# someone-in-somewhere/multimodal_rag

Measured on AMD Instinct MI355X. Metric: chunks embedded/sec + queries/sec top_k=5 over 1M×768 at 1/2/4/8 GPUs, higher is better.
Workload: dtype f16

## Files before the change

include/mmrag.h:

```cpp
#ifndef MMRAG_H
#define MMRAG_H

#include <stddef.h>
#include <stdint.h>

#ifdef __cplusplus
extern "C" {
#endif

#define MMRAG_OK 0
#define MMRAG_EINVAL 1
#define MMRAG_EWORKSPACE 2
#define MMRAG_EHIP 3
#define MMRAG_EUNSUPPORTED 4

#define MMRAG_F32 0
#define MMRAG_F16 1
#define MMRAG_BF16 2
#define MMRAG_F8E4M3 3

#define MMRAG_MAX_K 20

int mmrag_abi_version(void);
const char *mmrag_last_error(void);

int64_t mmrag_padded_dim(int d, int dtype);

size_t mmrag_cosine_topk_workspace_bytes(int B, int64_t n, int k);

int mmrag_cosine_topk(const void *q, const void *corpus, int B, int64_t n, int d, int64_t ld,
                      int dtype, int k, int64_t row_offset, const uint32_t *alive_bits,
                      float *out_scores, int64_t *out_rows, void *workspace,
                      size_t workspace_bytes, void *stream);

int mmrag_cosine_topk_lists(const void *q, const void *corpus, int B, int64_t n, int d, int64_t ld,
                            int dtype, int k, const uint32_t *alive_bits, void *workspace,
                            size_t workspace_bytes, void *stream);
int mmrag_cosine_topk_select(int B, int64_t n, int k, int64_t row_offset, const void *workspace,
                             float *out_scores, int64_t *out_rows, void *stream);

#define MMRAG_MAX_K_DEEP 4096
size_t mmrag_cosine_topk_deep_workspace_bytes(int B, int64_t n, int k);
int mmrag_cosine_topk_deep(const void *q, const void *corpus, int B, int64_t n, int d, int64_t ld,
                           int dtype, int k, int64_t row_offset, const uint32_t *alive_bits,
                           float *out_scores, int64_t *out_rows, void *workspace,
                           size_t workspace_bytes, void *stream);

#define MMRAG_MAX_RESCORE_CANDIDATES 4096
int mmrag_rescore_topk(const void *q, const void *plane, int64_t ld, int dtype, int d, const int64_t *cand_rows,
                       int B, int C, int k, float *out_scores, int64_t *out_rows, void *stream);

int mmrag_merge_topk(const float *scores, const int64_t *rows, int G, int B, int k_in, int k,
                     float *out_scores, int64_t *out_rows, void *stream);
int mmrag_merge_topk_host(const float *scores, const int64_t *rows, int G, int B, int k_in,
                          int k, float *out_scores, int64_t *out_rows);
int mmrag_merge_topk_host_packed(const void *blocks, int G, int B, int k_in, int k,
                                 float *out_scores, int64_t *out_rows);

int mmrag_append_rows(void *corpus, int64_t capacity, int64_t ld, int dtype, int64_t n_used,
                      const float *new_rows, int64_t m, int d, void *stream);

int mmrag_gather_rows(void *dst, const void *src, int64_t ld, int dtype,
                      const int64_t *keep_rows, int64_t m, void *stream);

int mmrag_fetch_rows_f32(const void *corpus, int64_t ld, int dtype, const int64_t *rows,
                         int64_t m, int d, float *out, void *stream);

int mmrag_copy_to_host_async(void *dst_host, const void *src_dev, size_t bytes, void *stream);


#define MMRAG_ACT_NONE 0
#define MMRAG_ACT_GELU 1
#define MMRAG_ACT_QUICK_GELU 2

#define MMRAG_ARCH_BERT 0
#define MMRAG_ARCH_PRELN 1

#define MMRAG_POOL_MEAN 0
#define MMRAG_POOL_FIRST 1
#define MMRAG_POOL_SELECT 2

typedef struct mmrag_encoder_desc {
    int32_t arch;
    int32_t n_layers, hidden, n_heads, intermediate, vocab, max_pos;
    int32_t pool, act, causal, normalize;
    int32_t out_dim;
    float ln_eps;
    int32_t image, patch;
} mmrag_encoder_desc;

size_t mmrag_encoder_workspace_bytes(const mmrag_encoder_desc *desc, int64_t T, int B);
int mmrag_encoder_forward(const mmrag_encoder_desc *desc, const void *const *w, const int32_t *ids,
                          const int32_t *pos_ids, const int32_t *cu_seqlens, const int32_t *sel,
                          int64_t T, int B, int max_len, float *out, void *workspace,
                          size_t workspace_bytes, void *stream);

size_t mmrag_encoder_f32_workspace_bytes(const mmrag_encoder_desc *desc, int64_t T, int B);
int mmrag_encoder_forward_f32(const mmrag_encoder_desc *desc, const void *const *w, const int32_t *ids,
                              const int32_t *pos_ids, const int32_t *cu_seqlens, const int32_t *sel, int64_t T, int B,
                              int max_len, float *out, void *workspace, size_t workspace_bytes, void *stream);
int mmrag_linear_f32(const float *x, int64_t M, int K, const float *wt, int N, const float *bias, int act,
                     const float *resid, float *out, void *stream);

size_t mmrag_cross_encoder_workspace_bytes(const mmrag_encoder_desc *desc, int64_t T, int B);
int mmrag_cross_encoder_forward(const mmrag_encoder_desc *desc, const void *const *w, int n_labels, const int32_t *ids,
                                const int32_t *type_ids, const int32_t *pos_ids, const int32_t *cu_seqlens, int64_t T,
                                int B, int max_len, float *out_logits, void *workspace, size_t workspace_bytes,
                                void *stream);
size_t mmrag_cross_encoder_f32_workspace_bytes(const mmrag_encoder_desc *desc, int64_t T, int B);
int mmrag_cross_encoder_forward_f32(const mmrag_encoder_desc *desc, const void *const *w, int n_labels,
                                    const int32_t *ids, const int32_t *type_ids, const int32_t *pos_ids,
                                    const int32_t *cu_seqlens, int64_t T, int B, int max_len, float *out_logits,
                                    void *workspace, size_t workspace_bytes, void *stream);

#define MMRAG_MAX_READER_TOKENS 512
#define MMRAG_MAX_ANSWER_TOKENS 64
#define MMRAG_MAX_READER_SPANS 8
int mmrag_span_select(const void *hidden, int ld, int hidden_dim, const float *qa_w, const float *qa_b,
                      const int32_t *cu_seqlens, const int32_t *ctx_start, const int32_t *ctx_len, int64_t T, int B,
                      int max_answer_tokens, int n_best, int32_t *out_span, float *out_score, float *out_null,
                      float *out_lse, float *out_logits, void *stream);
size_t mmrag_reader_workspace_bytes(const mmrag_encoder_desc *desc, int64_t T, int B);
int mmrag_reader_forward(const mmrag_encoder_desc *desc, const void *const *w, const int32_t *ids,
                         const int32_t *type_ids, const int32_t *pos_ids, const int32_t *cu_seqlens,
                         const int32_t *ctx_start, const int32_t *ctx_len, int64_t T, int B, int max_len,
                         int max_answer_tokens, int n_best, int32_t *out_span, float *out_score, float *out_null,
                         float *out_lse, float *out_logits, void *workspace, size_t workspace_bytes, void *stream);

#define MMRAG_PIXELS_F16_CHW 0
#define MMRAG_PIXELS_U8_HWC 1
int mmrag_vit_forward(const mmrag_encoder_desc *desc, const void *const *w, const void *pixels, int pixel_kind,
                      const int32_t *cu_seqlens, int B, float *out, void *workspace, size_t workspace_bytes,
                      void *stream);

void *mmrag_wordpiece_create(const uint32_t *cps, const int64_t *offsets, int n_tokens, int lower);
void mmrag_wordpiece_destroy(void *tokenizer);
int mmrag_wordpiece_encode_batch(const void *tokenizer, const uint32_t *cps, const int64_t *offsets, int n,
                                 int max_length, int32_t *ids, int32_t *lens, int n_threads);

int mmrag_wordpiece_encode_pairs(const void *tokenizer, const uint32_t *cps_a, const int64_t *offsets_a,
                                 const uint32_t *cps_b, const int64_t *offsets_b, int n, int max_length, int32_t *ids,
                                 int32_t *type_ids, int32_t *lens, int n_threads);

#define MMRAG_LEX_DOCUMENTS 0
#define MMRAG_LEX_QUERIES 1
void *mmrag_lexicon_create(void);
void mmrag_lexicon_destroy(void *lexicon);
int64_t mmrag_lexicon_size(const void *lexicon);
int mmrag_lexicon_analyze_batch(void *lexicon, const uint32_t *cps, const int64_t *offsets, int n, int mode,
                                int64_t *out_offsets, int32_t *term_ids, int32_t *tfs, int32_t *dl, int64_t capacity,
                                int n_threads);

int mmrag_lexical_df_update(const int64_t *fwd_off, const int32_t *fwd_term, const int64_t *rows, int64_t row0,
                            int64_t n_rows, int sign, int32_t *df, void *stream);
size_t mmrag_lexical_csr_build_workspace_bytes(int64_t n, int n_terms);
int mmrag_lexical_csr_build(const int64_t *fwd_off, const int32_t *fwd_term, const int32_t *fwd_tf, int64_t n,
                            int64_t n_postings, int n_terms, int64_t *term_off, int32_t *post_row, int32_t *post_tf,
                            void *workspace, size_t workspace_bytes, void *stream);
size_t mmrag_bm25_topk_workspace_bytes(int B, int64_t n, int k);
int mmrag_bm25_topk(const int64_t *term_off, const int32_t *post_row, const int32_t *post_tf, const int32_t *dl,
                    const int32_t *df, int n_terms, int64_t n, const int32_t *q_off, const int32_t *q_terms, int B,
                    int64_t n_live, int64_t sum_dl, float k1, float b, int k, const uint32_t *alive_bits,
                    float *out_scores, int64_t *out_rows, void *workspace, size_t workspace_bytes, void *stream);
int mmrag_rows_dot(const void *q, const void *corpus, int64_t ld, int dtype, int d, const int32_t *qi,
                   const int64_t *rows, int64_t m, float *out, void *stream);

#define MMRAG_MAX_MMR_CANDIDATES 1024
size_t mmrag_mmr_select_workspace_bytes(int B, int C, int d, int dtype);
int mmrag_mmr_select(const void *corpus, int64_t ld, int dtype, int d, const float *cand_scores,
                     const int64_t *cand_rows, int B, int C, int k, float lambda, float *out_scores, int64_t *out_rows,
                     int32_t *out_pos, float *out_mmr, void *workspace, size_t workspace_bytes, void *stream);

#define MMRAG_MAX_GROUP_CANDIDATES 4096
#define MMRAG_MAX_GROUPS 256
#define MMRAG_MAX_GROUP_SIZE 16
int mmrag_group_select(const float *scores, const int64_t *rows, int B, int C, const int32_t *group_of_row,
                       int64_t n_rows, int n_groups, int group_size, float *out_scores, int64_t *out_rows,
                       int32_t *out_pos, int32_t *out_group, int32_t *out_info, void *stream);

#define MMRAG_MAX_FUSE_LISTS 16
#define MMRAG_MAX_FUSE_CANDIDATES 256
#define MMRAG_MAX_FUSE_RESULTS 4096
#define MMRAG_FUSE_RRF 0
#define MMRAG_FUSE_MAX 1
int mmrag_fuse_select(const float *scores, const int64_t *rows, int L, int C, const int32_t *list_off, int G,
                      const float *weights, int method, int rrf_k, int n, float *out_fused, int64_t *out_rows,
                      float *out_best, int32_t *out_best_list, int32_t *out_count, int32_t *out_info, void *stream);

#define MMRAG_MAX_JOIN_PAIRS (1 << 26)
int mmrag_sim_join(const void *rows, int64_t n, int64_t ld, int dtype, int d, const uint32_t *alive, float threshold,
                   int64_t *out_pairs, float *out_scores, int64_t capacity, unsigned long long *count, void *stream);

#define MMRAG_MAX_CLUSTERS 4096
int mmrag_kmeans_assign(const void *rows, int64_t n, int64_t ld, int dtype, int d, const void *centroids, int k,
                        const uint32_t *alive, int32_t *out_assign, float *out_score, void *stream);
int mmrag_cluster_sums(const void *rows, int64_t ld, int dtype, int d, const int32_t *order, const int64_t *seg_off,
                       int k, float *out_sums, void *stream);

#define MMRAG_MAX_SCOPE_GROUPS 64
size_t mmrag_scoped_topk_workspace_bytes(int B, int64_t n, int k, int n_groups);
int mmrag_scoped_topk(const void *q, const void *rows, int B, int64_t n, int d, int64_t ld, int dtype, int k,
                      int64_t row_offset, const uint32_t *alive_bits, const int32_t *group_of_row, int n_groups,
                      const int32_t *scope_of_query, int S, const int32_t *scope_off, const int32_t *scope_groups,
                      int64_t max_candidates, float *out_scores, int64_t *out_rows, void *workspace,
                      size_t workspace_bytes, void *stream);

size_t mmrag_boosted_topk_workspace_bytes(int B, int64_t n, int k);
int mmrag_boosted_topk(const void *q, const void *rows, int B, int64_t n, int d, int64_t ld, int dtype, int k,
                       int64_t row_offset, const uint32_t *alive_bits, const float *prior, const float *weight,
                       float *out_scores, int64_t *out_rows, float *out_boost, void *workspace, size_t workspace_bytes,
                       void *stream);

#define MMRAG_MAX_RECOMMEND_EXAMPLES 16
size_t mmrag_recommend_topk_workspace_bytes(int R, int64_t n, int k);
int mmrag_recommend_topk(const void *examples, const int8_t *sign, const float *neg_weight, const void *rows, int R,
                         int64_t n, int d, int64_t ld, int dtype, int k, int64_t row_offset, const uint32_t *alive_bits,
                         float *out_scores, int64_t *out_rows, float *out_pos, float *out_neg, int32_t *out_pos_arg,
                         int32_t *out_neg_arg, void *workspace, size_t workspace_bytes, void *stream);

#define MMRAG_MAX_RELATED_ROWS 8192
#define MMRAG_MAX_RELATED_SETS 64
size_t mmrag_related_groups_workspace_bytes(int M, int S, int64_t n, int n_groups, int k);
int mmrag_related_groups(const void *set_rows, int M, const int32_t *set_off, int S, const void *rows, int64_t n, int d,
                         int64_t ld, int dtype, const uint32_t *alive_bits, const int32_t *group_of_row, int n_groups,
                         const int32_t *exclude_group, float threshold, int k, float *out_similarity, int32_t *out_group,
                         int32_t *out_covered, float *out_best, int64_t *out_best_row, void *workspace,
                         size_t workspace_bytes, void *stream);

#define MMRAG_MAX_FILTER_OPS 32
#define MMRAG_MAX_FILTER_SET 64
#define MMRAG_MAX_FILTER_COLUMNS 16
#define MMRAG_FILTER_NUMBER 0
#define MMRAG_FILTER_STRING 1
enum {
    MMRAG_FILTER_TRUE = 0, MMRAG_FILTER_FALSE, MMRAG_FILTER_AND, MMRAG_FILTER_OR, MMRAG_FILTER_EQ, MMRAG_FILTER_NE,
    MMRAG_FILTER_GT, MMRAG_FILTER_GE, MMRAG_FILTER_LT, MMRAG_FILTER_LE, MMRAG_FILTER_IN, MMRAG_FILTER_NIN
};
typedef struct {
    int32_t code, column, set_off, set_len;
    double value;
} mmrag_filter_op;
int64_t mmrag_filter_words(int64_t n);
int mmrag_filter_eval(const mmrag_filter_op *ops, int n_ops, const int32_t *prog_off, int F, const double *set_values,
                      int n_set, const void *const *columns, const int32_t *kinds, int n_columns, int64_t n,
                      const uint32_t *alive_bits, uint32_t *out_bits, void *stream);
size_t mmrag_filtered_topk_workspace_bytes(int B, int64_t n, int k);
int mmrag_filtered_topk(const void *q, const void *rows, int B, int64_t n, int d, int64_t ld, int dtype, int k,
                        int64_t row_offset, const int32_t *filter_of_query, int F, const uint32_t *vis_bits,
                        float *out_scores, int64_t *out_rows, void *workspace, size_t workspace_bytes, void *stream);

#define MMRAG_MAX_FACET_COLUMNS 4
size_t mmrag_range_scan_workspace_bytes(int B, int64_t n, int limit, int facet_slots);
int mmrag_range_scan(const void *q, const void *rows, int B, int64_t n, int d, int64_t ld, int dtype,
                     const float *threshold, int limit, int64_t row_offset, const int32_t *filter_of_query, int F,
                     const uint32_t *vis_bits, const int32_t *const *facet_cols, const int32_t *facet_sizes, int n_facets,
                     uint32_t *out_count, uint32_t *out_facets, float *out_scores, int64_t *out_rows, void *workspace,
                     size_t workspace_bytes, void *stream);

#define MMRAG_MAX_LATE_QUERY_TOKENS 128
#define MMRAG_MAX_LATE_DOC_TOKENS 512
size_t mmrag_encoder_tokens_workspace_bytes(const mmrag_encoder_desc *desc, int64_t T, int B, int out_dim);
int mmrag_encoder_forward_tokens(const mmrag_encoder_desc *desc, const void *const *w, const int32_t *ids,
                                 const int32_t *pos_ids, const int32_t *cu_seqlens, int64_t T, int B, int max_len,
                                 const void *proj, int out_dim, void *out_tokens, void *workspace,
                                 size_t workspace_bytes, void *stream);
int mmrag_maxsim_scores(const void *q_tok, int64_t q_rows, int64_t q_ld, const void *d_tok, int64_t d_rows,
                        int64_t d_ld, int dim, const int32_t *q_start, const int32_t *q_len, int n_q,
                        const int32_t *d_start, const int32_t *d_len, int n_d, const int32_t *pair_q,
                        const int32_t *pair_d, int P, float *out_sum, float *out_best_sim, int32_t *out_best_idx,
                        void *stream);

#define MMRAG_MAX_LATE_QUESTIONS 4096
size_t mmrag_maxsim_topk_workspace_bytes(int Q, int64_t n_items, int k);
int mmrag_maxsim_topk(const void *q_tok, int64_t q_rows, int64_t q_ld, const int32_t *q_start, const int32_t *q_len,
                      int Q, const void *tok, int64_t T, int64_t ld, const int32_t *item_off, int64_t n_items,
                      const uint32_t *alive_bits, int dim, int k, float *out_scores, int64_t *out_items,
                      void *workspace, size_t workspace_bytes, void *stream);

int mmrag_f8_encode_rows(const void *src, int src_dtype, int64_t m, int d, int64_t src_ld, void *dst, int64_t dst_ld,
                         void *stream);
int mmrag_maxsim_scores_f8(const void *q_codes, int64_t q_rows, int64_t q_ld, const void *d_codes, int64_t d_rows,
                           int64_t d_ld, int dim, const int32_t *q_start, const int32_t *q_len, int n_q,
                           const int32_t *d_start, const int32_t *d_len, int n_d, const int32_t *pair_q,
                           const int32_t *pair_d, int P, float *out_sum, float *out_best_sim, int32_t *out_best_idx,
                           void *stream);
size_t mmrag_maxsim_topk_f8_workspace_bytes(int Q, int64_t n_items, int k);
int mmrag_maxsim_topk_f8(const void *q_codes, int64_t q_rows, int64_t q_ld, const int32_t *q_start,
                         const int32_t *q_len, int Q, const void *codes, int64_t T, int64_t ld,
                         const int32_t *item_off, int64_t n_items, const uint32_t *alive_bits, int dim, int k,
                         float *out_scores, int64_t *out_items, void *workspace, size_t workspace_bytes, void *stream);

#define MMRAG_LATE_WINDOW_TOKENS 16
#define MMRAG_MAX_LATE_WINDOWS 32
int mmrag_maxsim_windows(const void *q_tok, int64_t q_rows, int64_t q_ld, const void *d_tok, int64_t d_rows,
                         int64_t d_ld, int dim, const int32_t *q_start, const int32_t *q_len, int n_q,
                         const int32_t *d_start, const int32_t *d_len, int n_d, const int32_t *pair_q,
                         const int32_t *pair_d, int P, int window_blocks, float *out_sum, float *out_win,
                         int32_t *out_best, void *stream);
int mmrag_maxsim_windows_f8(const void *q_codes, int64_t q_rows, int64_t q_ld, const void *d_codes, int64_t d_rows,
                            int64_t d_ld, int dim, const int32_t *q_start, const int32_t *q_len, int n_q,
                            const int32_t *d_start, const int32_t *d_len, int n_d, const int32_t *pair_q,
                            const int32_t *pair_d, int P, int window_blocks, float *out_sum, float *out_win,
                            int32_t *out_best, void *stream);

void *mmrag_clip_bpe_create(const uint32_t *vocab_cps, const int64_t *vocab_offsets, const int32_t *vocab_ids,
                            int n_vocab, const uint32_t *merge_cps, const int64_t *merge_offsets, int n_merges);
void mmrag_clip_bpe_destroy(void *tokenizer);
int mmrag_clip_bpe_encode_batch(const void *tokenizer, const uint32_t *cps, const int64_t *offsets, int n,
                                int max_length, int32_t *ids, int32_t *lens, int n_threads);

int mmrag_resample_ksize(int in_size, int out_size);
int mmrag_resample_coeffs(int in_size, int out_size, int first, int count, int32_t *bounds, int32_t *taps);
int mmrag_resize_crop_u8(const uint8_t *src, int H, int W, int64_t src_row_bytes, const int32_t *bx,
                         const int32_t *kx, int ksx, const int32_t *by, const int32_t *ky, int ksy, int out_h,
                         int out_w, int y_lo, int y_hi, uint8_t *tmp, uint8_t *dst, void *stream);

#define MMRAG_MAX_SPARSE_CHUNK_TOKENS 512
#define MMRAG_MAX_SPARSE_CHUNKS 65536
#define MMRAG_MAX_SPARSE_VOCAB 65536
#define MMRAG_MAX_SPARSE_TERMS 256
#define MMRAG_MAX_SPARSE_QUERY_TERMS 64
size_t mmrag_sparse_expand_forward_workspace_bytes(const mmrag_encoder_desc *desc, int64_t T, int B);
int mmrag_sparse_expand_forward(const mmrag_encoder_desc *desc, const void *const *w, const int32_t *ids,
                                const int32_t *pos_ids, const int32_t *cu_seqlens, int64_t T, int B, int max_len,
                                const void *head_w, const float *head_b, const float *head_ln_g,
                                const float *head_ln_b, void *out_tokens, void *workspace, size_t workspace_bytes,
                                void *stream);
size_t mmrag_sparse_pool_workspace_bytes(int64_t T, int n_chunks, int V);
int mmrag_sparse_pool(const void *tok, int64_t T, int64_t tok_ld, const int32_t *cu, int n_chunks, const void *E, int V,
                      int64_t e_ld, int dim, float *pooled, void *workspace, size_t workspace_bytes, void *stream);
int mmrag_sparse_select(const float *pooled, const float *bias, const uint32_t *skip_bits, int n_chunks, int V,
                        float scale, int m, int32_t *out_cnt, int32_t *out_terms, int32_t *out_imp, void *stream);
size_t mmrag_impact_topk_workspace_bytes(int B, int64_t n, int k);
int mmrag_impact_topk(const int64_t *term_off, const int32_t *post_row, const int32_t *post_imp, int n_terms, int64_t n,
                      const int32_t *q_off, const int32_t *q_terms, const int32_t *q_imp, int B, int k,
                      const uint32_t *alive_bits, float *out_scores, int64_t *out_rows, void *workspace,
                      size_t workspace_bytes, void *stream);

#define MMRAG_MAX_SUMMARY_SENTENCES 128
#define MMRAG_MAX_SUMMARY_ITERATIONS 64
int mmrag_summary_select(const void *rows, int64_t ld, int dtype, int d, int64_t n_rows, const int32_t *unit_start,
                         const int32_t *unit_len, int n_units, const int32_t *cost, const int32_t *budget,
                         const void *bias_rows, int64_t n_bias, const int32_t *unit_bias, float edge_threshold,
                         float alpha, int iterations, float lambda, int k, int32_t *out_pos, float *out_val,
                         float *out_rel, int32_t *out_used, void *stream);

int mmrag_device_info(int *n_cus, int *max_clock_mhz, int64_t *hbm_bytes);
int mmrag_bench_stream_copy(void *dst, const void *src, int64_t bytes, void *stream);
int mmrag_bench_stream_read(const void *src, int64_t bytes, float *out, void *stream);
int mmrag_bench_stream_write(void *dst, int64_t bytes, void *stream);
int mmrag_bench_mfma_f16(const void *seed, float *out, int iters, int64_t *flops, void *stream);
int mmrag_bench_mfma_f16_16x16x32(const void *seed, float *out, int iters, int64_t *flops, void *stream);

int mmrag_linear_f16(const void *x, int64_t M, int K, const void *wt, int N, const float *bias, int act,
                     const void *resid, void *out, void *stream);
int mmrag_layernorm_f16(const void *x, void *out, const float *gamma, const float *beta, int64_t T, int H,
                        float eps, void *stream);
int mmrag_embed_ln_f16(const int32_t *ids, const int32_t *pos_ids, const void *tok, const void *pos,
                       const void *type0, const float *gamma, const float *beta, void *out, int64_t T,
                       int H, int vocab, int max_pos, float eps, void *stream);
int mmrag_attention_f16(const void *qkv, const int32_t *cu_seqlens, void *ctx, int B, int max_len, int H,
                        int n_heads, int causal, void *stream);
int mmrag_pool_normalize_f16(const void *x, const int32_t *cu_seqlens, const int32_t *sel, float *out,
                             int B, int H, int pool, int normalize, void *stream);

#ifdef __cplusplus
}
#endif
#endif
```

multimodal_rag_amd/_native.py:

```python
from __future__ import annotations

import ctypes
import os
import threading
from ctypes import c_char_p, c_float, c_int, c_int32, c_int64, c_size_t, c_void_p
from typing import Optional, Tuple

import numpy as np
import torch

_PKG = os.path.dirname(os.path.abspath(__file__))
LIB_PATH = os.path.join(_PKG, "lib", "libmmrag.so")

F32, F16, BF16, F8E4M3 = 0, 1, 2, 3
MAX_K = 20
MAX_K_DEEP = 4096
MAX_MMR_CANDIDATES = 1024
MAX_RESCORE_CANDIDATES = 4096
MAX_GROUP_CANDIDATES, MAX_GROUPS, MAX_GROUP_SIZE = 4096, 256, 16
MAX_FUSE_LISTS, MAX_FUSE_CANDIDATES, MAX_FUSE_RESULTS = 16, 256, 4096
FUSE_METHODS = {"rrf": 0, "max": 1}
MAX_JOIN_PAIRS = 1 << 26
MAX_CLUSTERS = 4096
MAX_SCOPE_GROUPS = 64
MAX_FILTER_OPS, MAX_FILTER_SET, MAX_FILTER_COLUMNS = 32, 64, 16
MAX_FACET_COLUMNS = 4
MAX_RELATED_ROWS, MAX_RELATED_SETS = 8192, 64
MAX_RECOMMEND_EXAMPLES = 16
MAX_LATE_QUERY_TOKENS, MAX_LATE_DOC_TOKENS = 128, 512
MAX_LATE_PAIRS = 65535
MAX_LATE_QUESTIONS = 4096
LATE_WINDOW_TOKENS, MAX_LATE_WINDOWS = 16, 32
MAX_SUMMARY_SENTENCES, MAX_SUMMARY_ITERATIONS = 128, 64
MAX_READER_TOKENS, MAX_ANSWER_TOKENS, MAX_READER_SPANS = 512, 64, 8
_DT2TORCH = {F32: torch.float32, F16: torch.float16, BF16: torch.bfloat16, F8E4M3: torch.float8_e4m3fn}
_TORCH2DT = {v: k for k, v in _DT2TORCH.items()}

_lib = None
_lock = threading.Lock()


class MMRagNativeError(RuntimeError):
    pass


def _declare(lib):
    lib.mmrag_abi_version.restype = c_int
    lib.mmrag_last_error.restype = c_char_p
    lib.mmrag_padded_dim.restype = c_int64
    lib.mmrag_padded_dim.argtypes = [c_int, c_int]
    lib.mmrag_cosine_topk_workspace_bytes.restype = c_size_t
    lib.mmrag_cosine_topk_workspace_bytes.argtypes = [c_int, c_int64, c_int]
    lib.mmrag_cosine_topk.restype = c_int
    lib.mmrag_cosine_topk.argtypes = [c_void_p, c_void_p, c_int, c_int64, c_int, c_int64, c_int, c_int,
                                      c_int64, c_void_p, c_void_p, c_void_p, c_void_p, c_size_t, c_void_p]
    lib.mmrag_cosine_topk_lists.restype = c_int
    lib.mmrag_cosine_topk_lists.argtypes = [c_void_p, c_void_p, c_int, c_int64, c_int, c_int64, c_int, c_int,
                                            c_void_p, c_void_p, c_size_t, c_void_p]
    lib.mmrag_internal_search_uses_qs.restype = c_int
    lib.mmrag_internal_search_uses_qs.argtypes = [c_int, c_int64, c_int64, c_int, c_int]
    lib.mmrag_internal_cosine_topk_lists_ex.restype = c_int
    lib.mmrag_internal_cosine_topk_lists_ex.argtypes = [c_void_p, c_void_p, c_int, c_int64, c_int, c_int64, c_int,
                                                        c_int, c_void_p, c_void_p, c_size_t, c_void_p, ctypes.c_uint]
    lib.mmrag_cosine_topk_select.restype = c_int
    lib.mmrag_cosine_topk_select.argtypes = [c_int, c_int64, c_int, c_int64, c_void_p, c_void_p, c_void_p, c_void_p]
    lib.mmrag_cosine_topk_deep_workspace_bytes.restype = c_size_t
    lib.mmrag_cosine_topk_deep_workspace_bytes.argtypes = [c_int, c_int64, c_int]
    lib.mmrag_cosine_topk_deep.restype = c_int
    lib.mmrag_cosine_topk_deep.argtypes = lib.mmrag_cosine_topk.argtypes
    lib.mmrag_internal_cosine_topk_deep_ex.restype = c_int
    lib.mmrag_internal_cosine_topk_deep_ex.argtypes = lib.mmrag_cosine_topk.argtypes + [ctypes.c_uint, c_int64]
    lib.mmrag_rescore_topk.restype = c_int
    lib.mmrag_rescore_topk.argtypes = [c_void_p, c_void_p, c_int64, c_int, c_int, c_void_p, c_int, c_int, c_int,
                                       c_void_p, c_void_p, c_void_p]
    lib.mmrag_merge_topk.restype = c_int
    lib.mmrag_merge_topk.argtypes = [c_void_p, c_void_p, c_int, c_int, c_int, c_int, c_void_p, c_void_p, c_void_p]
    lib.mmrag_merge_topk_host.restype = c_int
    lib.mmrag_merge_topk_host.argtypes = [c_void_p, c_void_p, c_int, c_int, c_int, c_int, c_void_p, c_void_p]
    lib.mmrag_merge_topk_host_packed.restype = c_int
    lib.mmrag_merge_topk_host_packed.argtypes = [c_void_p, c_int, c_int, c_int, c_int, c_void_p, c_void_p]
    lib.mmrag_append_rows.restype = c_int
    lib.mmrag_append_rows.argtypes = [c_void_p, c_int64, c_int64, c_int, c_int64, c_void_p, c_int64, c_int, c_void_p]
    lib.mmrag_gather_rows.restype = c_int
    lib.mmrag_gather_rows.argtypes = [c_void_p, c_void_p, c_int64, c_int, c_void_p, c_int64, c_void_p]
    lib.mmrag_fetch_rows_f32.restype = c_int
    lib.mmrag_fetch_rows_f32.argtypes = [c_void_p, c_int64, c_int, c_void_p, c_int64, c_int, c_void_p, c_void_p]
    lib.mmrag_device_info.restype = c_int
    lib.mmrag_device_info.argtypes = [ctypes.POINTER(c_int), ctypes.POINTER(c_int), ctypes.POINTER(c_int64)]
    lib.mmrag_bench_stream_copy.restype = c_int
    lib.mmrag_bench_stream_copy.argtypes = [c_void_p, c_void_p, c_int64, c_void_p]
    lib.mmrag_bench_mfma_f16.restype = c_int
    lib.mmrag_bench_mfma_f16.argtypes = [c_void_p, c_void_p, c_int, ctypes.POINTER(c_int64), c_void_p]
    lib.mmrag_bench_mfma_f16_16x16x32.restype = c_int
    lib.mmrag_bench_mfma_f16_16x16x32.argtypes = [c_void_p, c_void_p, c_int, ctypes.POINTER(c_int64), c_void_p]
    lib.mmrag_bench_stream_read.restype = c_int
    lib.mmrag_bench_stream_read.argtypes = [c_void_p, c_int64, c_void_p, c_void_p]
    lib.mmrag_bench_stream_write.restype = c_int
    lib.mmrag_bench_stream_write.argtypes = [c_void_p, c_int64, c_void_p]
    lib.mmrag_copy_to_host_async.restype = c_int
    lib.mmrag_copy_to_host_async.argtypes = [c_void_p, c_void_p, c_size_t, c_void_p]
    lib.mmrag_encoder_workspace_bytes.restype = c_size_t
    lib.mmrag_encoder_workspace_bytes.argtypes = [c_void_p, c_int64, c_int]
    lib.mmrag_encoder_forward.restype = c_int
    lib.mmrag_encoder_forward.argtypes = [c_void_p, c_void_p, c_void_p, c_void_p, c_void_p, c_void_p, c_int64, c_int,
                                          c_int, c_void_p, c_void_p, c_size_t, c_void_p]
    lib.mmrag_encoder_f32_workspace_bytes.restype = c_size_t
    lib.mmrag_encoder_f32_workspace_bytes.argtypes = [c_void_p, c_int64, c_int]
    lib.mmrag_encoder_forward_f32.restype = c_int
    lib.mmrag_encoder_forward_f32.argtypes = lib.mmrag_encoder_forward.argtypes
    lib.mmrag_linear_f32.restype = c_int
    lib.mmrag_linear_f32.argtypes = [c_void_p, c_int64, c_int, c_void_p, c_int, c_void_p, c_int, c_void_p, c_void_p, c_void_p]
    lib.mmrag_vit_forward.restype = c_int
    lib.mmrag_vit_forward.argtypes = [c_void_p, c_void_p, c_void_p, c_int, c_void_p, c_int, c_void_p, c_void_p, c_size_t,
                                      c_void_p]
    lib.mmrag_wordpiece_create.restype = c_void_p
    lib.mmrag_wordpiece_create.argtypes = [c_void_p, c_void_p, c_int, c_int]
    lib.mmrag_wordpiece_destroy.restype = None
    lib.mmrag_wordpiece_destroy.argtypes = [c_void_p]
    lib.mmrag_wordpiece_encode_batch.restype = c_int
    lib.mmrag_wordpiece_encode_batch.argtypes = [c_void_p, c_void_p, c_void_p, c_int, c_int, c_void_p, c_void_p, c_int]
    lib.mmrag_clip_bpe_create.restype = c_void_p
    lib.mmrag_clip_bpe_create.argtypes = [c_void_p, c_void_p, c_void_p, c_int, c_void_p, c_void_p, c_int]
    lib.mmrag_clip_bpe_destroy.restype = None
    lib.mmrag_clip_bpe_destroy.argtypes = [c_void_p]
    lib.mmrag_clip_bpe_encode_batch.restype = c_int
    lib.mmrag_clip_bpe_encode_batch.argtypes = [c_void_p, c_void_p, c_void_p, c_int, c_int, c_void_p, c_void_p, c_int]
    lib.mmrag_resample_ksize.restype = c_int
    lib.mmrag_resample_ksize.argtypes = [c_int, c_int]
    lib.mmrag_resample_coeffs.restype = c_int
    lib.mmrag_resample_coeffs.argtypes = [c_int, c_int, c_int, c_int, c_void_p, c_void_p]
    lib.mmrag_resize_crop_u8.restype = c_int
    lib.mmrag_resize_crop_u8.argtypes = [c_void_p, c_int, c_int, c_int64, c_void_p, c_void_p, c_int, c_void_p, c_void_p,
                                         c_int, c_int, c_int, c_int, c_int, c_void_p, c_void_p, c_void_p]
    lib.mmrag_linear_f16.restype = c_int
    lib.mmrag_linear_f16.argtypes = [c_void_p, c_int64, c_int, c_void_p, c_int, c_void_p, c_int, c_void_p, c_void_p,
                                     c_void_p]
    lib.mmrag_layernorm_f16.restype = c_int
    lib.mmrag_layernorm_f16.argtypes = [c_void_p, c_void_p, c_void_p, c_void_p, c_int64, c_int, c_float, c_void_p]
    lib.mmrag_embed_ln_f16.restype = c_int
    lib.mmrag_embed_ln_f16.argtypes = [c_void_p, c_void_p, c_void_p, c_void_p, c_void_p, c_void_p, c_void_p, c_void_p,
                                       c_int64, c_int, c_int, c_int, c_float, c_void_p]
    lib.mmrag_attention_f16.restype = c_int
    lib.mmrag_attention_f16.argtypes = [c_void_p, c_void_p, c_void_p, c_int, c_int, c_int, c_int, c_int, c_void_p]
    lib.mmrag_pool_normalize_f16.restype = c_int
    lib.mmrag_pool_normalize_f16.argtypes = [c_void_p, c_void_p, c_void_p, c_void_p, c_int, c_int, c_int, c_int,
                                             c_void_p]
    lib.mmrag_internal_linear_f16_norms.restype = c_int
    lib.mmrag_internal_linear_f16_norms.argtypes = [c_void_p, c_int64, c_int, c_void_p, c_int, c_void_p, c_int, c_void_p,
                                                    c_void_p, c_void_p, c_void_p, c_float, c_void_p, c_void_p, c_void_p,
                                                    c_void_p, c_void_p]
    lib.mmrag_internal_attention_f32.restype = c_int
    lib.mmrag_internal_attention_f32.argtypes = [c_void_p, c_void_p, c_void_p, c_int, c_int, c_int, c_int, c_void_p]
    lib.mmrag_internal_layernorm_f32.restype = c_int
    lib.mmrag_internal_layernorm_f32.argtypes = [c_void_p, c_void_p, c_void_p, c_void_p, c_int64, c_int, c_float, c_void_p]
    lib.mmrag_internal_pool_norm_f32.restype = c_int
    lib.mmrag_internal_pool_norm_f32.argtypes = [c_void_p, c_void_p, c_void_p, c_void_p, c_int, c_int, c_int, c_int,
                                                 c_void_p]
    lib.mmrag_internal_patchify.restype = c_int
    lib.mmrag_internal_patchify.argtypes = [c_void_p, c_int, c_void_p, c_int, c_int, c_int, c_void_p]
    lib.mmrag_internal_vit_assemble_ln.restype = c_int
    lib.mmrag_internal_vit_assemble_ln.argtypes = [c_void_p] * 6 + [c_int, c_int, c_int, c_float, c_void_p]
    lib.mmrag_internal_normalize_rows.restype = c_int
    lib.mmrag_internal_normalize_rows.argtypes = [c_void_p, c_void_p, c_int, c_int, c_void_p]
    lib.mmrag_internal_pool_f16.restype = c_int
    lib.mmrag_internal_pool_f16.argtypes = [c_void_p, c_void_p, c_void_p, c_void_p, c_int, c_int, c_int, c_void_p]
    lib.mmrag_cross_encoder_workspace_bytes.restype = c_size_t
    lib.mmrag_cross_encoder_workspace_bytes.argtypes = [c_void_p, c_int64, c_int]
    lib.mmrag_cross_encoder_f32_workspace_bytes.restype = c_size_t
    lib.mmrag_cross_encoder_f32_workspace_bytes.argtypes = [c_void_p, c_int64, c_int]
    lib.mmrag_cross_encoder_forward.restype = c_int
    lib.mmrag_cross_encoder_forward.argtypes = [c_void_p, c_void_p, c_int, c_void_p, c_void_p, c_void_p, c_void_p,
                                                c_int64, c_int, c_int, c_void_p, c_void_p, c_size_t, c_void_p]
    lib.mmrag_cross_encoder_forward_f32.restype = c_int
    lib.mmrag_cross_encoder_forward_f32.argtypes = lib.mmrag_cross_encoder_forward.argtypes
    lib.mmrag_span_select.restype = c_int
    lib.mmrag_span_select.argtypes = [c_void_p, c_int, c_int, c_void_p, c_void_p, c_void_p, c_void_p, c_void_p, c_int64,
                                      c_int, c_int, c_int, c_void_p, c_void_p, c_void_p, c_void_p, c_void_p, c_void_p]
    lib.mmrag_reader_workspace_bytes.restype = c_size_t
    lib.mmrag_reader_workspace_bytes.argtypes = [c_void_p, c_int64, c_int]
    lib.mmrag_reader_forward.restype = c_int
    lib.mmrag_reader_forward.argtypes = [c_void_p] * 8 + [c_int64, c_int, c_int, c_int, c_int] + [c_void_p] * 6 + \
        [c_size_t, c_void_p]
    lib.mmrag_wordpiece_encode_pairs.restype = c_int
    lib.mmrag_wordpiece_encode_pairs.argtypes = [c_void_p, c_void_p, c_void_p, c_void_p, c_void_p, c_int, c_int, c_void_p,
                                                 c_void_p, c_void_p, c_int]
    lib.mmrag_internal_embed_types_ln_f16.restype = c_int
    lib.mmrag_internal_embed_types_ln_f16.argtypes = [c_void_p] * 9 + [c_int64, c_int, c_int, c_int, c_int, c_float,
                                                                       c_void_p]
    lib.mmrag_internal_embed_types_ln_f32.restype = c_int
    lib.mmrag_internal_embed_types_ln_f32.argtypes = lib.mmrag_internal_embed_types_ln_f16.argtypes
    lib.mmrag_internal_cls_head_f32.restype = c_int
    lib.mmrag_internal_cls_head_f32.argtypes = [c_void_p] * 6 + [c_int, c_int, c_int, c_void_p, c_size_t, c_void_p]
    lib.mmrag_internal_cls_head_workspace_bytes.restype = c_size_t
    lib.mmrag_internal_cls_head_workspace_bytes.argtypes = [c_int, c_int, c_int]
    lib.mmrag_mmr_select_workspace_bytes.restype = c_size_t
    lib.mmrag_mmr_select_workspace_bytes.argtypes = [c_int, c_int, c_int, c_int]
    lib.mmrag_mmr_select.restype = c_int
    lib.mmrag_mmr_select.argtypes = [c_void_p, c_int64, c_int, c_int, c_void_p, c_void_p, c_int, c_int, c_int, c_float,
                                     c_void_p, c_void_p, c_void_p, c_void_p, c_void_p, c_size_t, c_void_p]
    lib.mmrag_internal_mmr_select_ex.restype = c_int
    lib.mmrag_internal_mmr_select_ex.argtypes = lib.mmrag_mmr_select.argtypes + [ctypes.c_uint]
    lib.mmrag_group_select.restype = c_int
    lib.mmrag_group_select.argtypes = [c_void_p, c_void_p, c_int, c_int, c_void_p, c_int64, c_int, c_int, c_void_p,
                                       c_void_p, c_void_p, c_void_p, c_void_p, c_void_p]
    lib.mmrag_fuse_select.restype = c_int
    lib.mmrag_fuse_select.argtypes = [c_void_p, c_void_p, c_int, c_int, c_void_p, c_int, c_void_p, c_int, c_int, c_int,
                                      c_void_p, c_void_p, c_void_p, c_void_p, c_void_p, c_void_p, c_void_p]
    lib.mmrag_sim_join.restype = c_int
    lib.mmrag_sim_join.argtypes = [c_void_p, c_int64, c_int64, c_int, c_int, c_void_p, c_float, c_void_p, c_void_p,
                                   c_int64, c_void_p, c_void_p]
    for name in ("mmrag_internal_join_tile", "mmrag_internal_join_slot_tile"):
        getattr(lib, name).restype = c_int
        getattr(lib, name).argtypes = [c_int64, c_int64, ctypes.POINTER(c_int64), ctypes.POINTER(c_int64)]
    lib.mmrag_kmeans_assign.restype = c_int
    lib.mmrag_kmeans_assign.argtypes = [c_void_p, c_int64, c_int64, c_int, c_int, c_void_p, c_int, c_void_p, c_void_p,
                                        c_void_p, c_void_p]
    lib.mmrag_cluster_sums.restype = c_int
    lib.mmrag_cluster_sums.argtypes = [c_void_p, c_int64, c_int, c_int, c_void_p, c_void_p, c_int, c_void_p, c_void_p]
    lib.mmrag_scoped_topk_workspace_bytes.restype = c_size_t
    lib.mmrag_scoped_topk_workspace_bytes.argtypes = [c_int, c_int64, c_int, c_int]
    lib.mmrag_scoped_topk.restype = c_int
    lib.mmrag_scoped_topk.argtypes = [c_void_p, c_void_p, c_int, c_int64, c_int, c_int64, c_int, c_int, c_int64,
                                      c_void_p, c_void_p, c_int, c_void_p, c_int, c_void_p, c_void_p, c_int64,
                                      c_void_p, c_void_p, c_void_p, c_size_t, c_void_p]
    lib.mmrag_internal_scoped_topk_ex.restype = c_int
    lib.mmrag_internal_scoped_topk_ex.argtypes = lib.mmrag_scoped_topk.argtypes + [c_int64]
    lib.mmrag_filter_words.restype = c_int64
    lib.mmrag_filter_words.argtypes = [c_int64]
    lib.mmrag_filter_eval.restype = c_int
    lib.mmrag_filter_eval.argtypes = [c_void_p, c_int, c_void_p, c_int, c_void_p, c_int, c_void_p, c_void_p, c_int,
                                      c_int64, c_void_p, c_void_p, c_void_p]
    lib.mmrag_filtered_topk_workspace_bytes.restype = c_size_t
    lib.mmrag_filtered_topk_workspace_bytes.argtypes = [c_int, c_int64, c_int]
    lib.mmrag_filtered_topk.restype = c_int
    lib.mmrag_filtered_topk.argtypes = [c_void_p, c_void_p, c_int, c_int64, c_int, c_int64, c_int, c_int, c_int64,
                                        c_void_p, c_int, c_void_p, c_void_p, c_void_p, c_void_p, c_size_t, c_void_p]
    lib.mmrag_internal_filtered_topk_ex.restype = c_int
    lib.mmrag_internal_filtered_topk_ex.argtypes = lib.mmrag_filtered_topk.argtypes + [c_int64, ctypes.c_uint, c_void_p]
    lib.mmrag_range_scan_workspace_bytes.restype = c_size_t
    lib.mmrag_range_scan_workspace_bytes.argtypes = [c_int, c_int64, c_int, c_int]
    lib.mmrag_range_scan.restype = c_int
    lib.mmrag_range_scan.argtypes = [c_void_p, c_void_p, c_int, c_int64, c_int, c_int64, c_int, c_void_p, c_int, c_int64,
                                     c_void_p, c_int, c_void_p, c_void_p, c_void_p, c_int, c_void_p, c_void_p, c_void_p,
                                     c_void_p, c_void_p, c_size_t, c_void_p]
    lib.mmrag_internal_range_scan_ex.restype = c_int
    lib.mmrag_internal_range_scan_ex.argtypes = lib.mmrag_range_scan.argtypes + [c_int64, ctypes.c_uint]
    lib.mmrag_related_groups_workspace_bytes.restype = c_size_t
    lib.mmrag_related_groups_workspace_bytes.argtypes = [c_int, c_int, c_int64, c_int, c_int]
    lib.mmrag_related_groups.restype = c_int
    lib.mmrag_related_groups.argtypes = [c_void_p, c_int, c_void_p, c_int, c_void_p, c_int64, c_int, c_int64, c_int,
                                         c_void_p, c_void_p, c_int, c_void_p, c_float, c_int, c_void_p, c_void_p,
                                         c_void_p, c_void_p, c_void_p, c_void_p, c_size_t, c_void_p]
    lib.mmrag_internal_related_groups_ex.restype = c_int
    lib.mmrag_internal_related_groups_ex.argtypes = lib.mmrag_related_groups.argtypes + [c_int64]
    lib.mmrag_internal_candidate_capacity.restype = c_int64
    lib.mmrag_internal_candidate_capacity.argtypes = [c_int]
    lib.mmrag_internal_bound_plan.restype = c_int
    lib.mmrag_internal_bound_plan.argtypes = [c_int64, c_int, c_int64, ctypes.c_uint, c_void_p, c_void_p]
    lib.mmrag_boosted_topk_workspace_bytes.restype = c_size_t
    lib.mmrag_boosted_topk_workspace_bytes.argtypes = [c_int, c_int64, c_int]
    lib.mmrag_boosted_topk.restype = c_int
    lib.mmrag_boosted_topk.argtypes = [c_void_p, c_void_p, c_int, c_int64, c_int, c_int64, c_int, c_int, c_int64,
                                       c_void_p, c_void_p, c_void_p, c_void_p, c_void_p, c_void_p, c_void_p, c_size_t,
                                       c_void_p]
    lib.mmrag_internal_boosted_topk_ex.restype = c_int
    lib.mmrag_internal_boosted_topk_ex.argtypes = lib.mmrag_boosted_topk.argtypes + [c_int64, ctypes.c_uint]
    lib.mmrag_recommend_topk_workspace_bytes.restype = c_size_t
    lib.mmrag_recommend_topk_workspace_bytes.argtypes = [c_int, c_int64, c_int]
    lib.mmrag_recommend_topk.restype = c_int
    lib.mmrag_recommend_topk.argtypes = [c_void_p, c_void_p, c_void_p, c_void_p, c_int, c_int64, c_int, c_int64, c_int,
                                         c_int, c_int64, c_void_p, c_void_p, c_void_p, c_void_p, c_void_p, c_void_p,
                                         c_void_p, c_void_p, c_size_t, c_void_p]
    lib.mmrag_internal_recommend_topk_ex.restype = c_int
    lib.mmrag_internal_recommend_topk_ex.argtypes = lib.mmrag_recommend_topk.argtypes + [c_int64, ctypes.c_uint]
    lib.mmrag_encoder_tokens_workspace_bytes.restype = c_size_t
    lib.mmrag_encoder_tokens_workspace_bytes.argtypes = [c_void_p, c_int64, c_int, c_int]
    lib.mmrag_encoder_forward_tokens.restype = c_int
    lib.mmrag_encoder_forward_tokens.argtypes = [c_void_p, c_void_p, c_void_p, c_void_p, c_void_p, c_int64, c_int, c_int,
                                                 c_void_p, c_int, c_void_p, c_void_p, c_size_t, c_void_p]
    lib.mmrag_maxsim_scores.restype = c_int
    lib.mmrag_maxsim_scores.argtypes = [c_void_p, c_int64, c_int64, c_void_p, c_int64, c_int64, c_int, c_void_p, c_void_p,
                                        c_int, c_void_p, c_void_p, c_int, c_void_p, c_void_p, c_int, c_void_p, c_void_p,
                                        c_void_p, c_void_p]
    lib.mmrag_maxsim_topk_workspace_bytes.restype = c_size_t
    lib.mmrag_maxsim_topk_workspace_bytes.argtypes = [c_int, c_int64, c_int]
    lib.mmrag_maxsim_topk.restype = c_int
    lib.mmrag_maxsim_topk.argtypes = [c_void_p, c_int64, c_int64, c_void_p, c_void_p, c_int, c_void_p, c_int64, c_int64,
                                      c_void_p, c_int64, c_void_p, c_int, c_int, c_void_p, c_void_p, c_void_p, c_size_t,
                                      c_void_p]
    lib.mmrag_internal_maxsim_topk_ex.restype = c_int
    lib.mmrag_internal_maxsim_topk_ex.argtypes = lib.mmrag_maxsim_topk.argtypes + [c_int, c_int64, ctypes.c_uint, c_int]
    lib.mmrag_internal_maxsim_topk_workspace_bytes_ex.restype = c_size_t
    lib.mmrag_internal_maxsim_topk_workspace_bytes_ex.argtypes = [c_int, c_int64, c_int, c_int, c_int]
    lib.mmrag_f8_encode_rows.restype = c_int
    lib.mmrag_f8_encode_rows.argtypes = [c_void_p, c_int, c_int64, c_int, c_int64, c_void_p, c_int64, c_void_p]
    lib.mmrag_maxsim_scores_f8.restype = c_int
    lib.mmrag_maxsim_scores_f8.argtypes = lib.mmrag_maxsim_scores.argtypes
    lib.mmrag_maxsim_topk_f8_workspace_bytes.restype = c_size_t
    lib.mmrag_maxsim_topk_f8_workspace_bytes.argtypes = [c_int, c_int64, c_int]
    lib.mmrag_maxsim_topk_f8.restype = c_int
    lib.mmrag_maxsim_topk_f8.argtypes = lib.mmrag_maxsim_topk.argtypes
    lib.mmrag_internal_maxsim_topk_f8_ex.restype = c_int
    lib.mmrag_internal_maxsim_topk_f8_ex.argtypes = lib.mmrag_internal_maxsim_topk_ex.argtypes
    lib.mmrag_internal_maxsim_topk_f8_workspace_bytes_ex.restype = c_size_t
    lib.mmrag_internal_maxsim_topk_f8_workspace_bytes_ex.argtypes = [c_int, c_int64, c_int, c_int, c_int]
    lib.mmrag_maxsim_windows.restype = c_int
    lib.mmrag_maxsim_windows.argtypes = lib.mmrag_maxsim_scores.argtypes[:16] + [c_int, c_void_p, c_void_p, c_void_p,
                                                                                 c_void_p]
    lib.mmrag_maxsim_windows_f8.restype = c_int
    lib.mmrag_maxsim_windows_f8.argtypes = lib.mmrag_maxsim_windows.argtypes
    lib.mmrag_sparse_expand_forward_workspace_bytes.restype = c_size_t
    lib.mmrag_sparse_expand_forward_workspace_bytes.argtypes = [c_void_p, c_int64, c_int]
    lib.mmrag_sparse_expand_forward.restype = c_int
    lib.mmrag_sparse_expand_forward.argtypes = [c_void_p, c_void_p, c_void_p, c_void_p, c_void_p, c_int64, c_int, c_int,
                                                c_void_p, c_void_p, c_void_p, c_void_p, c_void_p, c_void_p, c_size_t,
                                                c_void_p]
    lib.mmrag_sparse_pool_workspace_bytes.restype = c_size_t
    lib.mmrag_sparse_pool_workspace_bytes.argtypes = [c_int64, c_int, c_int]
    lib.mmrag_sparse_pool.restype = c_int
    lib.mmrag_sparse_pool.argtypes = [c_void_p, c_int64, c_int64, c_void_p, c_int, c_void_p, c_int, c_int64, c_int,
                                      c_void_p, c_void_p, c_size_t, c_void_p]
    lib.mmrag_internal_sparse_pool_ex.restype = c_int
    lib.mmrag_internal_sparse_pool_ex.argtypes = [c_void_p, c_int64, c_int64, c_void_p, c_int, c_void_p, c_int, c_int64,
                                                  c_int, c_void_p, c_void_p, c_int]
    lib.mmrag_sparse_select.restype = c_int
    lib.mmrag_sparse_select.argtypes = [c_void_p, c_void_p, c_void_p, c_int, c_int, c_float, c_int, c_void_p, c_void_p,
                                        c_void_p, c_void_p]
    lib.mmrag_impact_topk_workspace_bytes.restype = c_size_t
    lib.mmrag_impact_topk_workspace_bytes.argtypes = [c_int, c_int64, c_int]
    lib.mmrag_impact_topk.restype = c_int
    lib.mmrag_impact_topk.argtypes = [c_void_p, c_void_p, c_void_p, c_int, c_int64, c_void_p, c_void_p, c_void_p, c_int,
                                      c_int, c_void_p, c_void_p, c_void_p, c_void_p, c_size_t, c_void_p]
    lib.mmrag_internal_impact_topk_ex.restype = c_int
    lib.mmrag_internal_impact_topk_ex.argtypes = lib.mmrag_impact_topk.argtypes + [c_int64, ctypes.c_uint]
    lib.mmrag_internal_sparse_limits.restype = c_int
    lib.mmrag_internal_sparse_limits.argtypes = [c_void_p] * 5
    lib.mmrag_summary_select.restype = c_int
    lib.mmrag_summary_select.argtypes = [c_void_p, c_int64, c_int, c_int, c_int64, c_void_p, c_void_p, c_int, c_void_p,
                                         c_void_p, c_void_p, c_int64, c_void_p, c_float, c_float, c_int, c_float, c_int,
                                         c_void_p, c_void_p, c_void_p, c_void_p, c_void_p]
    from .lexical import declare as declare_lexical

    declare_lexical(lib)


def lib():
    global _lib
    if _lib is None:
        with _lock:
            if _lib is None:
                if not os.path.exists(LIB_PATH):
                    raise MMRagNativeError(
                        f"{LIB_PATH} is missing: build it with `python -m multimodal_rag_amd.build` "
                        "(hipcc, gfx950).  There is no CPU fallback.")
                handle = ctypes.CDLL(LIB_PATH, mode=ctypes.RTLD_GLOBAL)
                _declare(handle)
                _lib = handle
    return _lib


def _check(status: int, what: str):
    if status != 0:
        msg = lib().mmrag_last_error().decode("utf-8", "replace")
        raise MMRagNativeError(f"{what} failed (status {status}): {msg}")


def _stream_ptr(device) -> int:
    return torch.cuda.current_stream(device).cuda_stream


def _dev_check(*tensors):
    for t in tensors:
        if t is not None and not t.is_cuda:
            raise MMRagNativeError("libmmrag entry points take device (HIP) tensors only; got a CPU tensor")


def _nbytes(t: torch.Tensor) -> int:
    return t.numel() * t.element_size()


def _check_q_rows(who: str, q: torch.Tensor, rows: torch.Tensor, n: Optional[int] = None, other: str = "corpus"):
    if q.dim() != 2 or rows.dim() != 2 or not q.is_contiguous() or not rows.is_contiguous():
        raise MMRagNativeError(f"{who}: q and {other} must be contiguous 2-D tensors")
    if q.dtype != rows.dtype or q.shape[1] != rows.shape[1]:
        raise MMRagNativeError(f"{who}: q and {other} must share dtype and padded width")
    if n is not None and n > rows.shape[0]:
        raise MMRagNativeError(f"{who}: n={n} exceeds corpus capacity {rows.shape[0]}")


def _topk_out(B: int, k: int, device, packed: bool = False) -> Tuple[torch.Tensor, torch.Tensor]:
    if not packed:
        return (torch.empty((B, k), dtype=torch.float32, device=device),
                torch.empty((B, k), dtype=torch.int64, device=device))
    buf = torch.empty(B * k * 12, dtype=torch.uint8, device=device)
    return buf[B * k * 8:].view(torch.float32).view(B, k), buf[: B * k * 8].view(torch.int64).view(B, k)


def search_uses_query_stationary(B: int, n: int, d: int, k: int, dtype: torch.dtype) -> bool:
    return bool(lib().mmrag_internal_search_uses_qs(B, n, padded_dim(d, dtype), _TORCH2DT[dtype], k))


def search_kernel_name(B: int, n: int, d: int, k: int, dtype: torch.dtype) -> str:
    v = lib().mmrag_internal_search_uses_qs(B, n, padded_dim(d, dtype), _TORCH2DT[dtype], k)
    return {0: "cosine_topk_kernel (slab-ring)", 1: "cosine_topk_qs_kernel", 2: "cosine_topk_walk_kernel"}[v]


def padded_dim(d: int, dtype: torch.dtype) -> int:
    v = lib().mmrag_padded_dim(int(d), _TORCH2DT[dtype])
    if v < 0:
        raise MMRagNativeError(f"padded_dim: bad arguments d={d} dtype={dtype}")
    return int(v)


DBG_NO_PREPASS, DBG_8_WAVES, DBG_NO_QS, DBG_FORCE_QS = 1, 2, 4, 8
DBG_OLD_QS, DBG_MFMA32, DBG_MFMA16, DBG_NO_DYN, DBG_NO_SEED = 0x10000, 0x20000, 0x40000, 0x80000, 0x100000


def cosine_topk(q: torch.Tensor, corpus: torch.Tensor, n: int, d: int, k: int, row_offset: int = 0,
                alive_bits: Optional[torch.Tensor] = None,
                workspace: Optional[torch.Tensor] = None, dbg: int = 0,
                packed_out: bool = False) -> Tuple[torch.Tensor, torch.Tensor]:
    _dev_check(q, corpus, alive_bits)
    _check_q_rows("cosine_topk", q, corpus, n)
    B, ld = q.shape
    L = lib()
    need = L.mmrag_cosine_topk_workspace_bytes(B, n, k)
    if workspace is None or _nbytes(workspace) < need:
        workspace = torch.empty(max(need, 16), dtype=torch.uint8, device=q.device)
    out_s, out_r = _topk_out(B, k, q.device, packed_out)
    if dbg:
        cosine_topk_lists(q, corpus, n, d, k, workspace, alive_bits=alive_bits, dbg=dbg)
        return cosine_topk_select(B, n, k, row_offset, workspace, out_s, out_r)
    with torch.cuda.device(q.device):
        st = L.mmrag_cosine_topk(q.data_ptr(), corpus.data_ptr(), B, n, d, ld, _TORCH2DT[q.dtype], k, row_offset,
                                 alive_bits.data_ptr() if alive_bits is not None else None,
                                 out_s.data_ptr(), out_r.data_ptr(), workspace.data_ptr(), _nbytes(workspace),
                                 _stream_ptr(q.device))
    _check(st, "mmrag_cosine_topk")
    return out_s, out_r


DEEP_DBG_NO_BOUND = 1


def cosine_topk_deep(q: torch.Tensor, corpus: torch.Tensor, n: int, d: int, k: int, row_offset: int = 0,
                     alive_bits: Optional[torch.Tensor] = None, workspace: Optional[torch.Tensor] = None,
                     dbg: int = 0, cap: int = 0) -> Tuple[torch.Tensor, torch.Tensor]:
    _dev_check(q, corpus, alive_bits)
    _check_q_rows("cosine_topk_deep", q, corpus, n)
    B, ld = q.shape
    L = lib()
    need = cosine_topk_deep_workspace_bytes(B, n, k)
    if workspace is None or _nbytes(workspace) < need:
        workspace = torch.empty(max(need, 16), dtype=torch.uint8, device=q.device)
    out_s, out_r = _topk_out(B, k, q.device)
    with torch.cuda.device(q.device):
        st = L.mmrag_internal_cosine_topk_deep_ex(
            q.data_ptr(), corpus.data_ptr(), B, n, d, ld, _TORCH2DT[q.dtype], k, row_offset,
            alive_bits.data_ptr() if alive_bits is not None else None, out_s.data_ptr(), out_r.data_ptr(),
            workspace.data_ptr(), _nbytes(workspace), _stream_ptr(q.device), dbg, cap)
    _check(st, "mmrag_cosine_topk_deep")
    return out_s, out_r


def cosine_topk_deep_workspace_bytes(B: int, n: int, k: int) -> int:
    return int(lib().mmrag_cosine_topk_deep_workspace_bytes(B, n, k))


def rescore_topk(q: torch.Tensor, plane: torch.Tensor, d: int, cand_rows: torch.Tensor, k: int,
                 packed_out: bool = False) -> Tuple[torch.Tensor, torch.Tensor]:
    _dev_check(q, plane, cand_rows)
    _check_q_rows("rescore_topk", q, plane, other="plane")
    if cand_rows.dim() != 2 or cand_rows.dtype != torch.int64 or not cand_rows.is_contiguous() \
            or cand_rows.shape[0] != q.shape[0]:
        raise MMRagNativeError("rescore_topk: cand_rows must be a contiguous [B, C] int64 tensor")
    B, C = cand_rows.shape
    out_s, out_r = _topk_out(B, k, q.device, packed_out)
    with torch.cuda.device(q.device):
        st = lib().mmrag_rescore_topk(q.data_ptr(), plane.data_ptr(), plane.shape[1], _TORCH2DT[plane.dtype], d,
                                      cand_rows.data_ptr(), B, C, k, out_s.data_ptr(), out_r.data_ptr(),
                                      _stream_ptr(q.device))
    _check(st, "mmrag_rescore_topk")
    return out_s, out_r


MMR_DBG_STREAM = 1


def mmr_select_workspace_bytes(B: int, C: int, d: int, dtype: torch.dtype) -> int:
    return int(lib().mmrag_mmr_select_workspace_bytes(B, C, d, _TORCH2DT[dtype]))


def mmr_select(corpus: torch.Tensor, d: int, cand_scores: torch.Tensor, cand_rows: torch.Tensor, k: int,
               lambda_mult: float, dbg: int = 0):
    _dev_check(corpus, cand_scores, cand_rows)
    if corpus.dim() != 2 or not corpus.is_contiguous() or corpus.dtype not in _TORCH2DT:
        raise MMRagNativeError("mmr_select: corpus must be a contiguous 2-D tensor of a storage dtype")
    if (cand_scores.dim() != 2 or cand_scores.shape != cand_rows.shape or cand_scores.dtype != torch.float32
            or cand_rows.dtype != torch.int64 or not cand_scores.is_contiguous() or not cand_rows.is_contiguous()):
        raise MMRagNativeError("mmr_select: cand_scores [B, C] float32 and cand_rows [B, C] int64 must be contiguous "
                               "and of one shape")
    if cand_scores.device != corpus.device or cand_rows.device != corpus.device:
        raise MMRagNativeError("mmr_select: candidates and corpus must be on one device")
    B, C = cand_scores.shape
    dev = corpus.device
    out_s = torch.empty((B, k), dtype=torch.float32, device=dev)
    out_r = torch.empty((B, k), dtype=torch.int64, device=dev)
    out_p = torch.empty((B, k), dtype=torch.int32, device=dev)
    out_v = torch.empty((B, k), dtype=torch.float32, device=dev)
    with torch.cuda.device(dev):
        st = lib().mmrag_internal_mmr_select_ex(corpus.data_ptr(), corpus.shape[1], _TORCH2DT[corpus.dtype], d,
                                                cand_scores.data_ptr(), cand_rows.data_ptr(), B, C, k,
                                                float(lambda_mult), out_s.data_ptr(), out_r.data_ptr(),
                                                out_p.data_ptr(), out_v.data_ptr(), None, 0, _stream_ptr(dev), int(dbg))
    _check(st, "mmrag_mmr_select")
    return out_s, out_r, out_p, out_v


def group_select(scores: torch.Tensor, rows: torch.Tensor, group_of_row: torch.Tensor, n_rows: int, n_groups: int,
                 group_size: int):
    _dev_check(scores, rows, group_of_row)
    if (scores.dim() != 2 or scores.shape != rows.shape or scores.dtype != torch.float32 or rows.dtype != torch.int64
            or not scores.is_contiguous() or not rows.is_contiguous()):
        raise MMRagNativeError("group_select: scores [B, C] float32 and rows [B, C] int64 must be contiguous and of "
                               "one shape")
    if group_of_row.dim() != 1 or group_of_row.dtype != torch.int32 or not group_of_row.is_contiguous():
        raise MMRagNativeError("group_select: group_of_row must be a contiguous 1-D int32 tensor")
    if rows.device != scores.device or group_of_row.device != scores.device:
        raise MMRagNativeError("group_select: candidates and group_of_row must be on one device")
    n_rows, G, S = int(n_rows), int(n_groups), int(group_size)
    if n_rows > group_of_row.numel():
        raise MMRagNativeError(f"group_select: n_rows={n_rows} but group_of_row holds {group_of_row.numel()} entries")
    B, C = scores.shape
    dev = scores.device
    shape = (B, max(G, 0), max(S, 0))
    out_s = torch.empty(shape, dtype=torch.float32, device=dev)
    out_r = torch.empty(shape, dtype=torch.int64, device=dev)
    out_p = torch.empty(shape, dtype=torch.int32, device=dev)
    out_g = torch.empty(shape[:2], dtype=torch.int32, device=dev)
    out_i = torch.empty((B, 2), dtype=torch.int32, device=dev)
    with torch.cuda.device(dev):
        st = lib().mmrag_group_select(scores.data_ptr(), rows.data_ptr(), B, C, group_of_row.data_ptr(), n_rows, G, S,
                                      out_s.data_ptr(), out_r.data_ptr(), out_p.data_ptr(), out_g.data_ptr(),
                                      out_i.data_ptr(), _stream_ptr(dev))
    _check(st, "mmrag_group_select")
    return out_s, out_r, out_p, out_g, out_i


def _pinned_to_device(host: torch.Tensor, device) -> torch.Tensor:
    return host.contiguous().pin_memory().to(device, non_blocking=True)


def fuse_offsets(list_off, L: int, device) -> torch.Tensor:
    host = torch.as_tensor(list_off).to(torch.int64).reshape(-1)
    steps = host[1:] - host[:-1]
    if host.numel() < 2 or int(host[0]) != 0 or int(host[-1]) != L or bool((steps < 0).any()):
        raise MMRagNativeError(f"fuse_select: list_off must ascend from 0 to L={L} over at least one group")
    if int(steps.max()) > MAX_FUSE_LISTS:
        raise MMRagNativeError(f"fuse_select: a group owns {int(steps.max())} lists, at most {MAX_FUSE_LISTS} "
                               "are fused")
    return _pinned_to_device(host.to(torch.int32), device)


def fuse_select(scores: torch.Tensor, rows: torch.Tensor, list_off, n: int, weights: Optional[torch.Tensor] = None,
                method: str = "rrf", rrf_k: int = 60):
    _dev_check(scores, rows, weights)
    if (scores.dim() != 2 or scores.shape != rows.shape or scores.dtype != torch.float32 or rows.dtype != torch.int64
            or not scores.is_contiguous() or not rows.is_contiguous()):
        raise MMRagNativeError("fuse_select: scores [L, C] float32 and rows [L, C] int64 must be contiguous and of "
                               "one shape")
    L, C = scores.shape
    dev = scores.device
    if rows.device != dev:
        raise MMRagNativeError("fuse_select: scores and rows must be on one device")
    if weights is not None and (weights.dim() != 1 or weights.numel() != L or weights.dtype != torch.float32
                                or not weights.is_contiguous() or weights.device != dev):
        raise MMRagNativeError("fuse_select: weights must be a contiguous float32 tensor [L] on the lists' device")
    if method not in FUSE_METHODS:
        raise MMRagNativeError(f"fuse_select: unknown method {method!r} (one of {sorted(FUSE_METHODS)})")
    if isinstance(list_off, torch.Tensor) and list_off.is_cuda:
        if list_off.dim() != 1 or list_off.dtype != torch.int32 or not list_off.is_contiguous() or list_off.device != dev:
            raise MMRagNativeError("fuse_select: list_off must be a contiguous 1-D int32 tensor on the lists' device")
        off_dev = list_off
    else:
        off_dev = fuse_offsets(list_off, L, dev)
    G, n = off_dev.numel() - 1, int(n)
    shape = (max(G, 0), max(n, 0))
    out_f = torch.empty(shape, dtype=torch.float32, device=dev)
    out_r = torch.empty(shape, dtype=torch.int64, device=dev)
    out_b = torch.empty(shape, dtype=torch.float32, device=dev)
    out_l = torch.empty(shape, dtype=torch.int32, device=dev)
    out_c = torch.empty(shape, dtype=torch.int32, device=dev)
    out_i = torch.empty((shape[0], 2), dtype=torch.int32, device=dev)
    with torch.cuda.device(dev):
        st = lib().mmrag_fuse_select(scores.data_ptr(), rows.data_ptr(), L, C, off_dev.data_ptr(), G,
                                     weights.data_ptr() if weights is not None else None, FUSE_METHODS[method],
                                     int(rrf_k), n, out_f.data_ptr(), out_r.data_ptr(), out_b.data_ptr(),
                                     out_l.data_ptr(), out_c.data_ptr(), out_i.data_ptr(), _stream_ptr(dev))
    _check(st, "mmrag_fuse_select")
    return out_f, out_r, out_b, out_l, out_c, out_i


def _check_stored_rows(who: str, rows: torch.Tensor):
    if rows.dim() != 2 or not rows.is_contiguous() or rows.dtype not in _TORCH2DT:
        raise MMRagNativeError(f"{who}: rows must be a contiguous 2-D tensor of a storage dtype")


def _check_alive(who: str, alive: Optional[torch.Tensor], n: int, rows: torch.Tensor):
    if n > rows.shape[0]:
        raise MMRagNativeError(f"{who}: n={n} exceeds the {rows.shape[0]} rows given")
    if alive is not None and (alive.dim() != 1 or alive.dtype != torch.int32 or not alive.is_contiguous()
                              or alive.numel() * 32 < n or alive.device != rows.device):
        raise MMRagNativeError(f"{who}: alive must be a contiguous int32 bitmap of at least n bits on the rows' device")


def sim_join(rows: torch.Tensor, n: int, d: int, threshold: float, alive: Optional[torch.Tensor] = None,
             capacity: int = 1 << 20) -> Tuple[torch.Tensor, torch.Tensor, int]:
    _dev_check(rows, alive)
    _check_stored_rows("sim_join", rows)
    n, cap = int(n), int(capacity)
    _check_alive("sim_join", alive, n, rows)
    dev = rows.device
    pairs = torch.empty((max(cap, 1), 2), dtype=torch.int64, device=dev)
    scores = torch.empty(max(cap, 1), dtype=torch.float32, device=dev)
    count = torch.empty(1, dtype=torch.int64, device=dev)
    with torch.cuda.device(dev):
        st = lib().mmrag_sim_join(rows.data_ptr(), n, rows.shape[1], _TORCH2DT[rows.dtype], int(d),
                                  alive.data_ptr() if alive is not None else None, float(threshold), pairs.data_ptr(),
                                  scores.data_ptr(), cap, count.data_ptr(), _stream_ptr(dev))
    _check(st, "mmrag_sim_join")
    total = int(count.item())
    m = min(total, cap)
    pairs, scores = pairs[:m], scores[:m]
    if m > 1:
        order = torch.argsort(pairs[:, 0] * max(n, 1) + pairs[:, 1])
        pairs, scores = pairs[order], scores[order]
    return pairs, scores, total


def kmeans_assign(rows: torch.Tensor, n: int, d: int, centroids: torch.Tensor,
                  alive: Optional[torch.Tensor] = None) -> Tuple[torch.Tensor, torch.Tensor]:
    _dev_check(rows, centroids, alive)
    _check_stored_rows("kmeans_assign", rows)
    if (centroids.dim() != 2 or not centroids.is_contiguous() or centroids.dtype != rows.dtype
            or centroids.shape[1] != rows.shape[1] or centroids.device != rows.device):
        raise MMRagNativeError("kmeans_assign: centroids must be a contiguous [k, ld] tensor of the rows' dtype, padded "
                               "width and device")
    n = int(n)
    _check_alive("kmeans_assign", alive, n, rows)
    dev = rows.device
    assign = torch.empty(max(n, 1), dtype=torch.int32, device=dev)
    score = torch.empty(max(n, 1), dtype=torch.float32, device=dev)
    with torch.cuda.device(dev):
        st = lib().mmrag_kmeans_assign(rows.data_ptr(), n, rows.shape[1], _TORCH2DT[rows.dtype], int(d),
                                       centroids.data_ptr(), centroids.shape[0],
                                       alive.data_ptr() if alive is not None else None,
                                       assign.data_ptr(), score.data_ptr(), _stream_ptr(dev))
    _check(st, "mmrag_kmeans_assign")
    return assign[: max(n, 0)], score[: max(n, 0)]


def cluster_sums(rows: torch.Tensor, d: int, order: torch.Tensor, seg_off: torch.Tensor, k: int) -> torch.Tensor:
    _dev_check(rows, order, seg_off)
    _check_stored_rows("cluster_sums", rows)
    k = int(k)
    if order.dim() != 1 or order.dtype != torch.int32 or not order.is_contiguous() or order.device != rows.device:
        raise MMRagNativeError("cluster_sums: order must be a contiguous 1-D int32 tensor on the rows' device")
    if (seg_off.dim() != 1 or seg_off.dtype != torch.int64 or not seg_off.is_contiguous()
            or seg_off.numel() != k + 1 or seg_off.device != rows.device):
        raise MMRagNativeError("cluster_sums: seg_off must be a contiguous int64 tensor of k + 1 offsets on the rows' "
                               "device")
    dev = rows.device
    sums = torch.empty((max(k, 1), max(int(d), 1)), dtype=torch.float32, device=dev)
    order_ptr = order.data_ptr() if order.numel() else seg_off.data_ptr()
    with torch.cuda.device(dev):
        st = lib().mmrag_cluster_sums(rows.data_ptr(), rows.shape[1], _TORCH2DT[rows.dtype], int(d),
                                      order_ptr, seg_off.data_ptr(), k, sums.data_ptr(), _stream_ptr(dev))
    _check(st, "mmrag_cluster_sums")
    return sums


def scoped_topk_workspace_bytes(B: int, n: int, k: int, n_groups: int) -> int:
    return int(lib().mmrag_scoped_topk_workspace_bytes(int(B), int(n), int(k), int(n_groups)))


def candidate_capacity(k: int) -> int:
    return int(lib().mmrag_internal_candidate_capacity(int(k)))


def bound_plan(n: int, k: int, cap: int = 0, dbg: int = 0) -> Tuple[int, list]:
    slots = ctypes.c_int64(0)
    stages = (ctypes.c_int64 * 8)()
    m = int(lib().mmrag_internal_bound_plan(int(n), int(k), int(cap), int(dbg), ctypes.byref(slots), stages))
    if m < 0:
        raise MMRagNativeError(f"bound_plan: n={n}, k={k} outside the range of the scans")
    return int(slots.value), [int(stages[i]) for i in range(m)]


def check_scopes(B: int, n_groups: int, scope_of_query, scope_off, scope_groups) -> int:
    soq = [int(v) for v in scope_of_query]
    off = [int(v) for v in scope_off]
    grp = [int(v) for v in scope_groups]
    S = len(off) - 1
    if len(soq) != B:
        raise MMRagNativeError(f"scoped_topk: scope_of_query holds {len(soq)} entries for {B} queries")
    if S < 1 or off[0] != 0 or off[-1] != len(grp) or any(b < a for a, b in zip(off, off[1:])):
        raise MMRagNativeError("scoped_topk: scope_off must hold S + 1 >= 2 ascending offsets from 0 to "
                               "len(scope_groups)")
    for s in range(S):
        mine = grp[off[s]: off[s + 1]]
        if len(mine) > MAX_SCOPE_GROUPS:
            raise MMRagNativeError(f"scoped_topk: scope {s} holds {len(mine)} groups, at most {MAX_SCOPE_GROUPS}")
        if any(b <= a for a, b in zip(mine, mine[1:])) or (mine and (mine[0] < 0 or mine[-1] >= n_groups)):
            raise MMRagNativeError(f"scoped_topk: scope {s} must hold ascending ordinals in 0..{n_groups - 1}")
    bad = [v for v in soq if not 0 <= v < S]
    if bad:
        raise MMRagNativeError(f"scoped_topk: scope_of_query {bad[0]} outside 0..{S - 1}")
    return S


def scoped_topk(q: torch.Tensor, rows: torch.Tensor, n: int, d: int, k: int, group_col: torch.Tensor, n_groups: int,
                scope_of_query, scope_off, scope_groups, max_candidates: int,
                alive_bits: Optional[torch.Tensor] = None, workspace: Optional[torch.Tensor] = None,
                row_offset: int = 0, cap: int = 0) -> Tuple[torch.Tensor, torch.Tensor]:
    _dev_check(q, rows, alive_bits, group_col)
    _check_q_rows("scoped_topk", q, rows, n, other="rows")
    _check_stored_rows("scoped_topk", rows)
    B, ld = q.shape
    n, k, n_groups = int(n), int(k), int(n_groups)
    _check_alive("scoped_topk", alive_bits, n, rows)
    dev = q.device
    if (group_col.dim() != 1 or group_col.dtype != torch.int32 or not group_col.is_contiguous()
            or group_col.numel() < n or group_col.device != dev):
        raise MMRagNativeError("scoped_topk: group_col must be a contiguous int32 tensor of at least n ordinals on the "
                               "rows' device")
    tables = [torch.as_tensor(t, dtype=torch.int32).reshape(-1).cpu()
              for t in (scope_of_query, scope_off, scope_groups)]
    S = check_scopes(B, n_groups, *(t.tolist() for t in tables))
    at = [0, B, B + S + 1]
    packed = _pinned_to_device(torch.cat(tables + [torch.zeros(1, dtype=torch.int32)]), dev)
    soq, off, grp = (packed[lo:] for lo in at)
    need = scoped_topk_workspace_bytes(B, n, k, n_groups)
    if workspace is None or _nbytes(workspace) < need:
        workspace = torch.empty(max(need, 16), dtype=torch.uint8, device=dev)
    out_s, out_r = _topk_out(B, k, dev)
    with torch.cuda.device(dev):
        st = lib().mmrag_internal_scoped_topk_ex(
            q.data_ptr(), rows.data_ptr(), B, n, int(d), ld, _TORCH2DT[q.dtype], k, int(row_offset),
            alive_bits.data_ptr() if alive_bits is not None else None, group_col.data_ptr(), n_groups,
            soq.data_ptr(), S, off.data_ptr(), grp.data_ptr(), int(max_candidates), out_s.data_ptr(), out_r.data_ptr(),
            workspace.data_ptr(), _nbytes(workspace), _stream_ptr(dev), int(cap))
    _check(st, "mmrag_scoped_topk")
    return out_s, out_r


def filter_words(n: int) -> int:
    return int(lib().mmrag_filter_words(int(n)))


def filtered_topk_workspace_bytes(B: int, n: int, k: int) -> int:
    return int(lib().mmrag_filtered_topk_workspace_bytes(int(B), int(n), int(k)))


def check_filter_programs(ops: np.ndarray, prog_off, set_values, n_columns: int) -> int:
    off = [int(v) for v in np.asarray(prog_off).reshape(-1)]
    F, n_ops, n_set = len(off) - 1, len(ops), len(set_values)
    if F < 1 or off[0] != 0 or off[-1] != n_ops or any(b < a for a, b in zip(off, off[1:])):
        raise MMRagNativeError("filter_eval: prog_off must hold F + 1 >= 2 ascending offsets from 0 to len(ops)")
    if n_set and not np.isfinite(np.asarray(set_values, dtype=np.float64)).all():
        raise MMRagNativeError("filter_eval: set_values must be finite")
    for f in range(F):
        lo, hi = off[f], off[f + 1]
        if not 1 <= hi - lo <= MAX_FILTER_OPS:
            raise MMRagNativeError(f"filter_eval: program {f} holds {hi - lo} instructions, 1..{MAX_FILTER_OPS}")
        depth = 0
        for i in range(lo, hi):
            code, column, set_off, set_len, value = (ops[i][name].item() for name in
                                                     ("code", "column", "set_off", "set_len", "value"))
            if not 0 <= code <= 11:
                raise MMRagNativeError(f"filter_eval: instruction {i} has the unknown code {code}")
            if code in (2, 3):
                depth -= 1
                if depth < 1:
                    raise MMRagNativeError(f"filter_eval: program {f} pops an empty stack")
                continue
            depth += 1
            if code >= 4 and not 0 <= column < n_columns:
                raise MMRagNativeError(f"filter_eval: instruction {i} reads column {column} outside 0..{n_columns - 1}")
            if code >= 10 and not (0 <= set_len <= MAX_FILTER_SET and 0 <= set_off <= n_set - set_len):
                raise MMRagNativeError(f"filter_eval: instruction {i} reads a set outside set_values "
                                       f"(offset {set_off}, length {set_len}, at most {MAX_FILTER_SET})")
            if 4 <= code <= 9 and not np.isfinite(value):
                raise MMRagNativeError(f"filter_eval: instruction {i} compares with {value}")
        if depth != 1:
            raise MMRagNativeError(f"filter_eval: program {f} leaves {depth} values on the stack")
    return F


def filter_eval(ops: np.ndarray, prog_off, set_values, columns, n: int, alive_bits: Optional[torch.Tensor] = None,
                device=None, out: Optional[torch.Tensor] = None) -> torch.Tensor:
    columns = list(columns)
    n = int(n)
    if len(columns) > MAX_FILTER_COLUMNS:
        raise MMRagNativeError(f"filter_eval: {len(columns)} columns, at most {MAX_FILTER_COLUMNS}")
    _dev_check(alive_bits, *columns)
    dev = columns[0].device if columns else (alive_bits.device if alive_bits is not None else torch.device(device))
    for c in columns:
        if (c.dim() != 1 or c.dtype not in (torch.float64, torch.int32) or not c.is_contiguous() or c.numel() < n
                or c.device != dev):
            raise MMRagNativeError("filter_eval: a column must be a contiguous float64 or int32 tensor of at least n "
                                   "values on one device")
    if alive_bits is not None and (alive_bits.dim() != 1 or alive_bits.dtype != torch.int32
                                   or not alive_bits.is_contiguous() or alive_bits.numel() * 32 < n
                                   or alive_bits.device != dev):
        raise MMRagNativeError("filter_eval: alive must be a contiguous int32 bitmap of at least n bits on the columns' "
                               "device")
    ops = np.ascontiguousarray(ops)
    if ops.dtype.itemsize != 24:
        raise MMRagNativeError("filter_eval: ops must be an array of filters.OP_DTYPE (24-byte instructions)")
    off = np.ascontiguousarray(prog_off, dtype=np.int32).reshape(-1)
    sets = np.ascontiguousarray(set_values, dtype=np.float64).reshape(-1)
    F = check_filter_programs(ops, off, sets, len(columns))
    W = filter_words(n)
    if n < 0 or (W == 0 and n != 0):
        raise MMRagNativeError(f"filter_eval: n={n} outside 0..2^31-1")
    blob = np.concatenate([ops.view(np.uint8).reshape(-1), np.append(sets, 0.0).view(np.uint8), off.view(np.uint8)])
    packed = _pinned_to_device(torch.from_numpy(blob), dev)
    at_sets = ops.nbytes
    at_off = at_sets + (sets.size + 1) * 8
    if out is None:
        out = torch.empty((F, W), dtype=torch.int32, device=dev)
    elif (not out.is_cuda or out.dtype != torch.int32 or not out.is_contiguous() or tuple(out.shape) != (F, W)
          or out.device != dev):
        raise MMRagNativeError(f"filter_eval: out must be a contiguous int32 [{F}, {W}] tensor on the columns' device")
    if W == 0:
        return out
    ptrs = (c_void_p * MAX_FILTER_COLUMNS)(*[c.data_ptr() for c in columns])
    kinds = (c_int32 * MAX_FILTER_COLUMNS)(*[0 if c.dtype == torch.float64 else 1 for c in columns])
    with torch.cuda.device(dev):
        st = lib().mmrag_filter_eval(packed.data_ptr(), len(ops), packed.data_ptr() + at_off, F,
                                     packed.data_ptr() + at_sets, sets.size, ptrs, kinds, len(columns), n,
                                     alive_bits.data_ptr() if alive_bits is not None else None, out.data_ptr(),
                                     _stream_ptr(dev))
    _check(st, "mmrag_filter_eval")
    return out


def filtered_topk(q: torch.Tensor, rows: torch.Tensor, n: int, d: int, k: int, filter_of_query, vis_bits: torch.Tensor,
                  workspace: Optional[torch.Tensor] = None, row_offset: int = 0, cap: int = 0, dbg: int = 0,
                  count_items: bool = False):
    _dev_check(q, rows, vis_bits)
    _check_q_rows("filtered_topk", q, rows, n, other="rows")
    _check_stored_rows("filtered_topk", rows)
    B, ld = q.shape
    n, k = int(n), int(k)
    if not 1 <= k <= MAX_K_DEEP:
        raise ValueError(f"filtered_topk: k={k} outside 1..{MAX_K_DEEP}")
    dev = q.device
    W = filter_words(n)
    if (vis_bits.dim() != 2 or vis_bits.dtype != torch.int32 or not vis_bits.is_contiguous() or vis_bits.shape[0] < 1
            or vis_bits.shape[1] != W or vis_bits.device != dev):
        raise MMRagNativeError(f"filtered_topk: vis_bits must be a contiguous int32 [F, {W}] tensor on the rows' device")
    F = vis_bits.shape[0]
    foq = torch.as_tensor(filter_of_query, dtype=torch.int32).reshape(-1).cpu()
    if foq.numel() != B:
        raise MMRagNativeError(f"filtered_topk: filter_of_query holds {foq.numel()} entries for {B} queries")
    if B and (int(foq.min()) < 0 or int(foq.max()) >= F):
        raise MMRagNativeError(f"filtered_topk: filter_of_query outside 0..{F - 1}")
    foq_dev = _pinned_to_device(foq, dev)
    need = filtered_topk_workspace_bytes(B, n, k)
    if workspace is None or _nbytes(workspace) < need:
        workspace = torch.empty(max(need, 16), dtype=torch.uint8, device=dev)
    out_s, out_r = _topk_out(B, k, dev)
    items = torch.zeros(1, dtype=torch.int64, device=dev) if count_items else None
    with torch.cuda.device(dev):
        st = lib().mmrag_internal_filtered_topk_ex(
            q.data_ptr(), rows.data_ptr(), B, n, int(d), ld, _TORCH2DT[q.dtype], k, int(row_offset), foq_dev.data_ptr(),
            F, vis_bits.data_ptr() if vis_bits.numel() else None, out_s.data_ptr(), out_r.data_ptr(),
            workspace.data_ptr(), _nbytes(workspace), _stream_ptr(dev), int(cap), int(dbg),
            items.data_ptr() if items is not None else None)
    _check(st, "mmrag_filtered_topk")
    return (out_s, out_r, items) if count_items else (out_s, out_r)


def range_scan_workspace_bytes(B: int, n: int, limit: int, facet_slots: int = 0) -> int:
    return int(lib().mmrag_range_scan_workspace_bytes(int(B), int(n), int(limit), int(facet_slots)))


def range_scan(q: torch.Tensor, rows: torch.Tensor, n: int, d: int, threshold, limit: int, facet_cols=(),
               facet_sizes=(), filter_of_query=None, vis_bits: Optional[torch.Tensor] = None,
               workspace: Optional[torch.Tensor] = None, row_offset: int = 0, cap: int = 0, dbg: int = 0):
    n, limit = int(n), int(limit)
    facet_cols, facet_sizes = list(facet_cols), [int(g) for g in facet_sizes]
    if not 0 <= limit <= MAX_K_DEEP:
        raise ValueError(f"range_scan: limit={limit} outside 0..{MAX_K_DEEP}")
    if len(facet_cols) > MAX_FACET_COLUMNS:
        raise MMRagNativeError(f"range_scan: {len(facet_cols)} facet columns, at most {MAX_FACET_COLUMNS}")
    if len(facet_sizes) != len(facet_cols) or any(g < 0 for g in facet_sizes):
        raise MMRagNativeError("range_scan: facet_sizes must hold one G >= 0 per facet column")
    _dev_check(q, rows, vis_bits, *facet_cols)
    _check_q_rows("range_scan", q, rows, n, other="rows")
    _check_stored_rows("range_scan", rows)
    B, ld = q.shape
    dev = q.device
    for c in facet_cols:
        if c.dim() != 1 or c.dtype != torch.int32 or not c.is_contiguous() or c.numel() < n or c.device != dev:
            raise MMRagNativeError("range_scan: a facet column must be a contiguous int32 tensor of at least n codes on "
                                   "the rows' device")
    if isinstance(threshold, torch.Tensor) and threshold.is_cuda:
        thr = threshold
        if thr.dtype != torch.float32 or thr.dim() != 1 or thr.numel() != B or not thr.is_contiguous() or thr.device != dev:
            raise MMRagNativeError(f"range_scan: a device threshold must be a contiguous float32 [{B}] tensor")
    else:
        host = torch.as_tensor(threshold, dtype=torch.float32).reshape(-1)
        if host.numel() == 1:
            host = host.expand(B)
        if host.numel() != B:
            raise MMRagNativeError(f"range_scan: threshold holds {host.numel()} entries for {B} queries")
        if not bool(torch.isfinite(host).all()):
            raise ValueError("range_scan: thresholds must be finite")
        thr = _pinned_to_device(host, dev)
    foq_dev, F = None, 0
    if vis_bits is not None:
        W = filter_words(n)
        if (vis_bits.dim() != 2 or vis_bits.dtype != torch.int32 or not vis_bits.is_contiguous()
                or vis_bits.shape[0] < 1 or vis_bits.shape[1] != W or vis_bits.device != dev):
            raise MMRagNativeError(f"range_scan: vis_bits must be a contiguous int32 [F, {W}] tensor on the rows' device")
        F = vis_bits.shape[0]
        if filter_of_query is None:
            raise MMRagNativeError("range_scan: vis_bits needs filter_of_query")
        foq = torch.as_tensor(filter_of_query, dtype=torch.int32).reshape(-1).cpu()
        if foq.numel() != B:
            raise MMRagNativeError(f"range_scan: filter_of_query holds {foq.numel()} entries for {B} queries")
        foq_dev = _pinned_to_device(foq, dev)
    slots = sum(g + 1 for g in facet_sizes)
    need = range_scan_workspace_bytes(B, n, limit, slots)
    if workspace is None or _nbytes(workspace) < need:
        workspace = torch.empty(max(need, 16), dtype=torch.uint8, device=dev)
    counts = torch.empty(B, dtype=torch.int32, device=dev)
    facets = torch.empty((B, slots), dtype=torch.int32, device=dev) if facet_cols else None
    out_s, out_r = _topk_out(B, limit, dev) if limit else (None, None)
    ptrs = (c_void_p * MAX_FACET_COLUMNS)(*[c.data_ptr() for c in facet_cols])
    sizes = (c_int32 * MAX_FACET_COLUMNS)(*facet_sizes)
    with torch.cuda.device(dev):
        st = lib().mmrag_internal_range_scan_ex(
            q.data_ptr(), rows.data_ptr(), B, n, int(d), ld, _TORCH2DT[q.dtype], thr.data_ptr(), limit, int(row_offset),
            foq_dev.data_ptr() if foq_dev is not None else None, F,
            vis_bits.data_ptr() if vis_bits is not None and vis_bits.numel() else None, ptrs, sizes, len(facet_cols),
            counts.data_ptr(), facets.data_ptr() if facets is not None else None,
            out_s.data_ptr() if limit else None, out_r.data_ptr() if limit else None, workspace.data_ptr(),
            _nbytes(workspace), _stream_ptr(dev), int(cap), int(dbg))
    _check(st, "mmrag_range_scan")
    return counts, facets, out_s, out_r


def related_groups_workspace_bytes(M: int, S: int, n: int, n_groups: int, k: int) -> int:
    return int(lib().mmrag_related_groups_workspace_bytes(int(M), int(S), int(n), int(n_groups), int(k)))


def related_groups(sets: torch.Tensor, set_off, rows: torch.Tensor, n: int, d: int, k: int, group_col: torch.Tensor,
                   n_groups: int, threshold: float, exclude=None, alive_bits: Optional[torch.Tensor] = None,
                   table_bytes: Optional[int] = None, grid: int = 0):
    _dev_check(sets, rows, alive_bits, group_col)
    _check_q_rows("related_groups", sets, rows, n, other="rows")
    _check_stored_rows("related_groups", rows)
    M, ld = sets.shape
    n, k, n_groups = int(n), int(k), int(n_groups)
    _check_alive("related_groups", alive_bits, n, rows)
    dev = rows.device
    if (group_col.dim() != 1 or group_col.dtype != torch.int32 or not group_col.is_contiguous()
            or group_col.numel() < n or group_col.device != dev):
        raise MMRagNativeError("related_groups: group_col must be a contiguous int32 tensor of at least n ordinals on "
                               "the rows' device")
    off = [int(v) for v in set_off]
    S = len(off) - 1
    if S < 1 or off[0] != 0 or off[-1] != M or any(b < a for a, b in zip(off, off[1:])):
        raise ValueError(f"related_groups: set_off must hold S + 1 >= 2 ascending offsets from 0 to M={M}")
    if S > MAX_RELATED_SETS or M > MAX_RELATED_ROWS:
        raise ValueError(f"related_groups: at most {MAX_RELATED_SETS} sets and {MAX_RELATED_ROWS} vectors per call "
                         f"(S={S}, M={M})")
    if not 1 <= k <= MAX_K_DEEP:
        raise ValueError(f"related_groups: k={k} outside 1..{MAX_K_DEEP}")
    excl = [-1] * S if exclude is None else [-1 if v is None else int(v) for v in exclude]
    if len(excl) != S:
        raise ValueError(f"related_groups: exclude holds {len(excl)} entries for {S} sets")
    if table_bytes is None:
        from .config import settings

        table_bytes = int(settings.MMRAG_RELATED_TABLE_BYTES)
    cell = 8 * max(n_groups, 0)
    parts, s0 = [], 0
    for s in range(S):
        if (off[s + 1] - off[s]) * cell > table_bytes:
            raise ValueError(f"related_groups: set {s} alone needs a table of {(off[s + 1] - off[s]) * cell} bytes, "
                             f"above MMRAG_RELATED_TABLE_BYTES={table_bytes}")
        if (off[s + 1] - off[s0]) * cell > table_bytes:
            parts.append((s0, s))
            s0 = s
    parts.append((s0, S))
    host = []
    for a, b in parts:
        host += [v - off[a] for v in off[a: b + 1]] + excl[a:b]
    packed = _pinned_to_device(torch.tensor(host, dtype=torch.int32), dev)
    out_sim = torch.empty((S, k), dtype=torch.float32, device=dev)
    out_grp = torch.empty((S, k), dtype=torch.int32, device=dev)
    out_cov = torch.empty((S, k), dtype=torch.int32, device=dev)
    out_best = torch.empty((M + 1, k), dtype=torch.float32, device=dev)
    out_row = torch.empty((M + 1, k), dtype=torch.int64, device=dev)
    need = max(related_groups_workspace_bytes(off[b] - off[a], b - a, n, n_groups, k) for a, b in parts)
    workspace = torch.empty(max(need, 16), dtype=torch.uint8, device=dev)
    sets_ptr = sets.data_ptr() if M else workspace.data_ptr()
    at = 0
    with torch.cuda.device(dev):
        for a, b in parts:
            Sp, c0, Mp = b - a, off[a], off[b] - off[a]
            st = lib().mmrag_internal_related_groups_ex(
                sets_ptr + c0 * ld * sets.element_size(), Mp, packed[at:].data_ptr(), Sp, rows.data_ptr(), n, int(d),
                ld, _TORCH2DT[rows.dtype], alive_bits.data_ptr() if alive_bits is not None else None,
                group_col.data_ptr(), n_groups, packed[at + Sp + 1:].data_ptr(), float(threshold), k,
                out_sim[a:].data_ptr(), out_grp[a:].data_ptr(), out_cov[a:].data_ptr(), out_best[c0:].data_ptr(),
                out_row[c0:].data_ptr(), workspace.data_ptr(), _nbytes(workspace), _stream_ptr(dev), int(grid))
            _check(st, "mmrag_related_groups")
            at += 2 * Sp + 1
    return out_sim, out_grp, out_cov, out_best[:M], out_row[:M]


def boosted_topk_workspace_bytes(B: int, n: int, k: int) -> int:
    return int(lib().mmrag_boosted_topk_workspace_bytes(int(B), int(n), int(k)))


def _boost_operand(who: str, what: str, t, count: int, exact: bool, device) -> torch.Tensor:
    if isinstance(t, torch.Tensor) and t.is_cuda:
        if (t.dim() != 1 or t.dtype != torch.float32 or not t.is_contiguous() or t.device != device
                or (t.numel() != count if exact else t.numel() < count)):
            raise ValueError(f"{who}: {what} must be a contiguous float32 tensor of {count} entries on the rows' device")
        return t
    host = torch.as_tensor(t, dtype=torch.float64).reshape(-1).to(torch.float32)
    if host.numel() != count:
        raise ValueError(f"{who}: {what} holds {host.numel()} entries, expected {count}")
    if not bool(torch.isfinite(host).all()):
        raise ValueError(f"{who}: {what} must be finite")
    if host.numel() == 0:
        host = torch.zeros(1, dtype=torch.float32)
    return _pinned_to_device(host, device)


def boosted_topk(q: torch.Tensor, rows: torch.Tensor, n: int, d: int, k: int, prior, weight,
                 alive_bits: Optional[torch.Tensor] = None, workspace: Optional[torch.Tensor] = None,
                 row_offset: int = 0, cap: int = 0, dbg: int = 0,
                 want_boost: bool = True) -> Tuple[torch.Tensor, torch.Tensor, Optional[torch.Tensor]]:
    _dev_check(q, rows, alive_bits)
    _check_q_rows("boosted_topk", q, rows, n, other="rows")
    _check_stored_rows("boosted_topk", rows)
    B, ld = q.shape
    n, k = int(n), int(k)
    if not 1 <= k <= MAX_K_DEEP:
        raise ValueError(f"boosted_topk: k={k} outside 1..{MAX_K_DEEP}")
    _check_alive("boosted_topk", alive_bits, n, rows)
    dev = q.device
    if not isinstance(weight, torch.Tensor) and not hasattr(weight, "__len__"):
        weight = [float(weight)] * B
    prior_dev = _boost_operand("boosted_topk", "prior", prior, n, False, dev)
    weight_dev = _boost_operand("boosted_topk", "weight", weight, B, True, dev)
    need = boosted_topk_workspace_bytes(B, n, k)
    if workspace is None or _nbytes(workspace) < need:
        workspace = torch.empty(max(need, 16), dtype=torch.uint8, device=dev)
    out_s, out_r = _topk_out(B, k, dev)
    out_b = torch.empty((B, k), dtype=torch.float32, device=dev) if want_boost else None
    with torch.cuda.device(dev):
        st = lib().mmrag_internal_boosted_topk_ex(
            q.data_ptr(), rows.data_ptr(), B, n, int(d), ld, _TORCH2DT[q.dtype], k, int(row_offset),
            alive_bits.data_ptr() if alive_bits is not None else None, prior_dev.data_ptr(), weight_dev.data_ptr(),
            out_s.data_ptr(), out_r.data_ptr(), out_b.data_ptr() if out_b is not None else None,
            workspace.data_ptr(), _nbytes(workspace), _stream_ptr(dev), int(cap), int(dbg))
    _check(st, "mmrag_boosted_topk")
    return out_s, out_r, out_b


def recommend_topk_workspace_bytes(R: int, n: int, k: int) -> int:
    return int(lib().mmrag_recommend_topk_workspace_bytes(int(R), int(n), int(k)))


def pack_examples(positives, negatives, dim: int, dtype: torch.dtype, device,
                  rows: Optional[torch.Tensor] = None) -> Tuple[torch.Tensor, torch.Tensor]:
    E = MAX_RECOMMEND_EXAMPLES
    positives = list(positives)
    R = len(positives)
    if R == 0:
        raise ValueError("pack_examples: no request")
    negatives = [None] * R if negatives is None else list(negatives)
    if len(negatives) != R:
        raise ValueError(f"pack_examples: {len(negatives)} negative lists for {R} requests")
    ld = int(rows.shape[1]) if rows is not None else padded_dim(dim, dtype)
    host = np.zeros((E * R, dim), dtype=np.float32)
    sign = np.zeros(E * R, dtype=np.int8)
    slots, gathered = [], []
    for g in range(R):
        pos = list(positives[g]) if positives[g] is not None else []
        neg = list(negatives[g]) if negatives[g] is not None else []
        if not pos:
            raise ValueError(f"pack_examples: request {g} has no positive example")
        if len(pos) + len(neg) > E:
            raise ValueError(f"pack_examples: request {g} has {len(pos) + len(neg)} examples, at most {E}")
        for j, e in enumerate(pos + neg):
            at = E * g + j
            sign[at] = 1 if j < len(pos) else -1
            if rows is not None and isinstance(e, (int, np.integer)) and not isinstance(e, bool):
                if not 0 <= int(e) < rows.shape[0]:
                    raise ValueError(f"pack_examples: request {g}: stored row {int(e)} out of range")
                slots.append(at)
                gathered.append(int(e))
                continue
            v = np.asarray(e.detach().cpu() if isinstance(e, torch.Tensor) else e, dtype=np.float32).reshape(-1)
            if v.size != dim:
                raise ValueError(f"pack_examples: request {g}: an example holds {v.size} numbers, expected {dim}")
            nrm = float(np.sqrt(np.dot(v.astype(np.float64), v.astype(np.float64))))
            if not abs(nrm - 1.0) <= 1e-2:
                raise ValueError(f"pack_examples: request {g}: example {j} has norm {nrm:.4f}; examples are unit "
                                 f"vectors, as queries are -- L2-normalise them first")
            host[at] = v
    packed = torch.zeros((E * R, ld), dtype=dtype)
    packed[:, :dim] = torch.from_numpy(host).to(dtype)
    dev = torch.device(device)
    if dev.type == "cpu":
        if gathered:
            packed[slots] = rows[gathered].to(dtype)
        return packed, torch.from_numpy(sign)
    examples = _pinned_to_device(packed, dev)
    if gathered:
        examples[_pinned_to_device(torch.tensor(slots, dtype=torch.int64), dev)] = \
            rows[_pinned_to_device(torch.tensor(gathered, dtype=torch.int64), dev)]
    return examples, _pinned_to_device(torch.from_numpy(sign), dev)


def check_recommend_request(who: str, sign, neg_weight, R: int):
    E = MAX_RECOMMEND_EXAMPLES
    s = w = None
    if sign is not None:
        s = np.asarray(sign.cpu() if isinstance(sign, torch.Tensor) else sign).reshape(-1)
        if s.size != E * R:
            raise ValueError(f"{who}: sign holds {s.size} entries, expected {E} per request = {E * R}")
        if not np.isin(s, (-1, 0, 1)).all():
            raise ValueError(f"{who}: a sign must be -1, 0 or 1")
        s = s.astype(np.int8)
        lacking = np.nonzero(~(s.reshape(R, E) > 0).any(axis=1))[0]
        if lacking.size:
            raise ValueError(f"{who}: request {int(lacking[0])} has no positive example")
    if neg_weight is not None:
        w = np.asarray(neg_weight.cpu() if isinstance(neg_weight, torch.Tensor) else neg_weight,
                       dtype=np.float64).reshape(-1)
        if np.ndim(neg_weight) == 0:
            w = np.full(R, w[0])
        if w.size != R:
            raise ValueError(f"{who}: neg_weight holds {w.size} entries, expected {R}")
        if not (np.isfinite(w).all() and (w >= 0).all()):
            raise ValueError(f"{who}: neg_weight must be finite and >= 0")
        w = w.astype(np.float32)
    return s, w


def recommend_topk(examples: torch.Tensor, sign, neg_weight, rows: torch.Tensor, n: int, d: int, k: int,
                   alive_bits: Optional[torch.Tensor] = None, workspace: Optional[torch.Tensor] = None,
                   row_offset: int = 0, cap: int = 0, dbg: int = 0, want_explain: bool = True, checked: bool = False):
    E = MAX_RECOMMEND_EXAMPLES
    _dev_check(examples, rows, alive_bits)
    _check_q_rows("recommend_topk", examples, rows, n, other="rows")
    _check_stored_rows("recommend_topk", rows)
    n, k = int(n), int(k)
    if examples.shape[0] == 0 or examples.shape[0] % E:
        raise ValueError(f"recommend_topk: examples hold {examples.shape[0]} rows, expected {E} per request")
    R, ld = examples.shape[0] // E, examples.shape[1]
    if not 1 <= k <= MAX_K_DEEP:
        raise ValueError(f"recommend_topk: k={k} outside 1..{MAX_K_DEEP}")
    _check_alive("recommend_topk", alive_bits, n, rows)
    dev = examples.device
    sign_dev = sign if isinstance(sign, torch.Tensor) and sign.is_cuda else None
    w_dev = neg_weight if isinstance(neg_weight, torch.Tensor) and neg_weight.is_cuda else None
    if sign_dev is not None and (sign_dev.dtype != torch.int8 or sign_dev.numel() != E * R
                                 or not sign_dev.is_contiguous() or sign_dev.device != dev):
        raise ValueError(f"recommend_topk: sign must be a contiguous int8 tensor of {E * R} entries on the rows' device")
    if w_dev is not None and (w_dev.dtype != torch.float32 or w_dev.numel() != R or not w_dev.is_contiguous()
                              or w_dev.device != dev):
        raise ValueError(f"recommend_topk: neg_weight must be a contiguous float32 tensor of {R} entries on the rows' "
                         f"device")
    s_host, w_host = check_recommend_request("recommend_topk", None if checked and sign_dev is not None else sign,
                                             None if checked and w_dev is not None else neg_weight, R)
    if sign_dev is None:
        sign_dev = _pinned_to_device(torch.from_numpy(s_host), dev)
    if w_dev is None:
        w_dev = _pinned_to_device(torch.from_numpy(w_host), dev)
    need = recommend_topk_workspace_bytes(R, n, k)
    if workspace is None or _nbytes(workspace) < need:
        workspace = torch.empty(max(need, 16), dtype=torch.uint8, device=dev)
    out_s, out_r = _topk_out(R, k, dev)
    expl = [None] * 4
    if want_explain:
        expl = [torch.empty((R, k), dtype=t, device=dev)
                for t in (torch.float32, torch.float32, torch.int32, torch.int32)]
    with torch.cuda.device(dev):
        st = lib().mmrag_internal_recommend_topk_ex(
            examples.data_ptr(), sign_dev.data_ptr(), w_dev.data_ptr(), rows.data_ptr(), R, n, int(d), ld,
            _TORCH2DT[examples.dtype], k, int(row_offset), alive_bits.data_ptr() if alive_bits is not None else None,
            out_s.data_ptr(), out_r.data_ptr(), *[t.data_ptr() if t is not None else None for t in expl],
            workspace.data_ptr(), _nbytes(workspace), _stream_ptr(dev), int(cap), int(dbg))
    _check(st, "mmrag_recommend_topk")
    return (out_s, out_r, *expl)


_DT_NAME = {torch.float16: "float16", torch.uint8: "uint8"}


def check_late_tables(q_rows: int, d_rows: int, q_start, q_len, d_start, d_len, pair_q, pair_d) -> Tuple[int, int, int]:
    qs, ql, ds, dl = ([int(v) for v in t] for t in (q_start, q_len, d_start, d_len))
    pq, pd = [int(v) for v in pair_q], [int(v) for v in pair_d]
    if len(qs) != len(ql) or len(ds) != len(dl) or not qs or not ds:
        raise MMRagNativeError("maxsim_scores: start and len tables must have one entry per sequence, at least one "
                               "sequence on each side")
    if len(pq) != len(pd) or not 1 <= len(pq) <= MAX_LATE_PAIRS:
        raise MMRagNativeError(f"maxsim_scores: pair_q and pair_d must hold the same 1..{MAX_LATE_PAIRS} pairs "
                               f"(got {len(pq)} and {len(pd)})")
    for side, starts, lens, rows, most in (("query", qs, ql, int(q_rows), MAX_LATE_QUERY_TOKENS),
                                           ("passage", ds, dl, int(d_rows), MAX_LATE_DOC_TOKENS)):
        for s, (a, n) in enumerate(zip(starts, lens)):
            if not 1 <= n <= most:
                raise MMRagNativeError(f"maxsim_scores: {side} {s} has {n} tokens, outside 1..{most}")
            if a < 0 or a + n > rows:
                raise MMRagNativeError(f"maxsim_scores: {side} {s} (rows {a}..{a + n}) is outside the {rows} rows given")
    for name, idx, n in (("pair_q", pq, len(qs)), ("pair_d", pd, len(ds))):
        bad = [v for v in idx if not 0 <= v < n]
        if bad:
            raise MMRagNativeError(f"maxsim_scores: {name} {bad[0]} outside 0..{n - 1}")
    return len(qs), len(ds), len(pq)


def maxsim_scores(q_tok: torch.Tensor, d_tok: torch.Tensor, dim: int, q_start, q_len, d_start, d_len, pair_q, pair_d,
                  want_best: bool = True, _f8: bool = False):
    who, row_dtype = ("maxsim_scores_f8", torch.uint8) if _f8 else ("maxsim_scores", torch.float16)
    _dev_check(q_tok, d_tok)
    for name, t in (("q_tok", q_tok), ("d_tok", d_tok)):
        if t.dim() != 2 or not t.is_contiguous() or t.dtype != row_dtype:
            raise MMRagNativeError(f"{who}: {name} must be a contiguous 2-D {_DT_NAME[row_dtype]} tensor")
    if q_tok.device != d_tok.device:
        raise MMRagNativeError(f"{who}: q_tok and d_tok must be on one device")
    tables = [torch.as_tensor(t, dtype=torch.int32).reshape(-1).cpu()
              for t in (q_start, q_len, d_start, d_len, pair_q, pair_d)]
    n_q, n_d, P = check_late_tables(q_tok.shape[0], d_tok.shape[0], *(t.tolist() for t in tables))
    dev = q_tok.device
    packed = _pinned_to_device(torch.cat(tables), dev)
    at = [0, n_q, 2 * n_q, 2 * n_q + n_d, 2 * n_q + 2 * n_d, 2 * n_q + 2 * n_d + P]
    qs, ql, ds, dl, pq, pd = (packed[lo:] for lo in at)
    sums = torch.empty(P, dtype=torch.float32, device=dev)
    best_sim = torch.empty((P, MAX_LATE_QUERY_TOKENS), dtype=torch.float32, device=dev) if want_best else None
    best_idx = torch.empty((P, MAX_LATE_QUERY_TOKENS), dtype=torch.int32, device=dev) if want_best else None
    with torch.cuda.device(dev):
        fn = lib().mmrag_maxsim_scores_f8 if _f8 else lib().mmrag_maxsim_scores
        st = fn(q_tok.data_ptr(), q_tok.shape[0], q_tok.shape[1], d_tok.data_ptr(), d_tok.shape[0], d_tok.shape[1],
                int(dim), qs.data_ptr(), ql.data_ptr(), n_q, ds.data_ptr(), dl.data_ptr(), n_d, pq.data_ptr(),
                pd.data_ptr(), P, sums.data_ptr(), _ptr(best_sim), _ptr(best_idx), _stream_ptr(dev))
    _check(st, "mmrag_" + who)
    return sums, best_sim, best_idx


def maxsim_scores_f8(q_codes: torch.Tensor, d_codes: torch.Tensor, dim: int, q_start, q_len, d_start, d_len, pair_q,
                     pair_d, want_best: bool = True):
    return maxsim_scores(q_codes, d_codes, dim, q_start, q_len, d_start, d_len, pair_q, pair_d, want_best, _f8=True)


def maxsim_windows(q_tok: torch.Tensor, d_tok: torch.Tensor, dim: int, q_start, q_len, d_start, d_len, pair_q, pair_d,
                   window_blocks: int, _f8: bool = False):
    who, row_dtype = ("maxsim_windows_f8", torch.uint8) if _f8 else ("maxsim_windows", torch.float16)
    _dev_check(q_tok, d_tok)
    for name, t in (("q_tok", q_tok), ("d_tok", d_tok)):
        if t.dim() != 2 or not t.is_contiguous() or t.dtype != row_dtype:
            raise MMRagNativeError(f"{who}: {name} must be a contiguous 2-D {_DT_NAME[row_dtype]} tensor")
    if q_tok.device != d_tok.device:
        raise MMRagNativeError(f"{who}: q_tok and d_tok must be on one device")
    if not 1 <= int(window_blocks) <= MAX_LATE_WINDOWS:
        raise MMRagNativeError(f"{who}: window_blocks={window_blocks} outside 1..{MAX_LATE_WINDOWS}")
    tables = [torch.as_tensor(t, dtype=torch.int32).reshape(-1).cpu()
              for t in (q_start, q_len, d_start, d_len, pair_q, pair_d)]
    n_q, n_d, P = check_late_tables(q_tok.shape[0], d_tok.shape[0], *(t.tolist() for t in tables))
    dev = q_tok.device
    packed = _pinned_to_device(torch.cat(tables), dev)
    at = [0, n_q, 2 * n_q, 2 * n_q + n_d, 2 * n_q + 2 * n_d, 2 * n_q + 2 * n_d + P]
    qs, ql, ds, dl, pq, pd = (packed[lo:] for lo in at)
    sums = torch.empty(P, dtype=torch.float32, device=dev)
    win = torch.empty((P, MAX_LATE_WINDOWS), dtype=torch.float32, device=dev)
    best = torch.empty((P, 3), dtype=torch.int32, device=dev)
    with torch.cuda.device(dev):
        fn = lib().mmrag_maxsim_windows_f8 if _f8 else lib().mmrag_maxsim_windows
        st = fn(q_tok.data_ptr(), q_tok.shape[0], q_tok.shape[1], d_tok.data_ptr(), d_tok.shape[0], d_tok.shape[1],
                int(dim), qs.data_ptr(), ql.data_ptr(), n_q, ds.data_ptr(), dl.data_ptr(), n_d, pq.data_ptr(),
                pd.data_ptr(), P, int(window_blocks), sums.data_ptr(), win.data_ptr(), best.data_ptr(),
                _stream_ptr(dev))
    _check(st, "mmrag_" + who)
    return sums, win, best


def maxsim_windows_f8(q_codes: torch.Tensor, d_codes: torch.Tensor, dim: int, q_start, q_len, d_start, d_len, pair_q,
                      pair_d, window_blocks: int):
    return maxsim_windows(q_codes, d_codes, dim, q_start, q_len, d_start, d_len, pair_q, pair_d, window_blocks,
                          _f8=True)


def summary_select(rows: torch.Tensor, d: int, unit_start: torch.Tensor, unit_len: torch.Tensor, cost: torch.Tensor,
                   budget: torch.Tensor, k: int, edge_threshold: float, alpha: float, iterations: int, lam: float,
                   bias_rows: Optional[torch.Tensor] = None, unit_bias: Optional[torch.Tensor] = None,
                   want_rel: bool = True, out=None):
    who = "summary_select"
    tables = (unit_start, unit_len, cost, budget)
    _dev_check(rows, bias_rows, unit_bias, *tables)
    _check_stored_rows(who, rows)
    for t in tables + ((unit_bias,) if unit_bias is not None else ()):
        if t.dtype != torch.int32 or t.dim() != 1 or not t.is_contiguous() or t.device != rows.device:
            raise MMRagNativeError(f"{who}: the tables must be contiguous 1-D int32 tensors on the rows' device")
    n_rows, n_units = int(rows.shape[0]), int(unit_start.shape[0])
    if unit_len.shape[0] != n_units or budget.shape[0] != n_units or cost.shape[0] != n_rows:
        raise MMRagNativeError(f"{who}: unit_start, unit_len and budget need one entry per unit, cost one per row")
    if (bias_rows is None) != (unit_bias is None):
        raise MMRagNativeError(f"{who}: bias_rows and unit_bias go together")
    if bias_rows is not None:
        _check_q_rows(who, bias_rows, rows, other="rows")
        if unit_bias.shape[0] != n_units or bias_rows.device != rows.device:
            raise MMRagNativeError(f"{who}: unit_bias needs one entry per unit, bias_rows the rows' device")
    dev = rows.device
    if out is None:
        k_alloc = max(int(k), 1)
        out = (torch.empty((n_units, k_alloc), dtype=torch.int32, device=dev),
               torch.empty((n_units, k_alloc), dtype=torch.float32, device=dev),
               torch.empty(n_rows, dtype=torch.float32, device=dev) if want_rel else None,
               torch.empty(n_units, dtype=torch.int32, device=dev))
    pos, val, rel, used = out
    with torch.cuda.device(dev):
        st = lib().mmrag_summary_select(rows.data_ptr(), rows.shape[1], _TORCH2DT[rows.dtype], int(d), n_rows,
                                        unit_start.data_ptr(), unit_len.data_ptr(), n_units, cost.data_ptr(),
                                        budget.data_ptr(), _ptr(bias_rows),
                                        int(bias_rows.shape[0]) if bias_rows is not None else 0, _ptr(unit_bias),
                                        float(edge_threshold), float(alpha), int(iterations), float(lam), int(k),
                                        pos.data_ptr(), val.data_ptr(), _ptr(rel), used.data_ptr(), _stream_ptr(dev))
    _check(st, "mmrag_summary_select")
    return pos, val, rel, used


def f8_encode_rows(src: torch.Tensor, d: Optional[int] = None, out: Optional[torch.Tensor] = None) -> torch.Tensor:
    _dev_check(src)
    if (src.dim() != 2 or src.dtype not in (torch.float16, torch.float32) or src.stride(1) != 1
            or (src.shape[0] > 1 and src.stride(0) < src.shape[1])):
        raise MMRagNativeError("f8_encode_rows: src must be a 2-D float16 or float32 tensor with contiguous rows")
    m, d = int(src.shape[0]), int(src.shape[1] if d is None else d)
    if not 0 < d <= src.shape[1]:
        raise MMRagNativeError(f"f8_encode_rows: d={d} outside 1..{src.shape[1]}")
    ld = padded_dim(d, torch.float8_e4m3fn)
    if out is None:
        out = torch.empty((m, ld), dtype=torch.uint8, device=src.device)
    elif (out.dim() != 2 or out.dtype != torch.uint8 or not out.is_contiguous() or out.shape[0] < m
          or out.shape[1] < ld or out.device != src.device):
        raise MMRagNativeError(f"f8_encode_rows: out must be a contiguous uint8 tensor of at least [{m}, {ld}] on "
                               f"src's device")
    src_ld = int(src.stride(0)) if m > 1 else int(src.shape[1])
    with torch.cuda.device(src.device):
        st = lib().mmrag_f8_encode_rows(src.data_ptr(), _TORCH2DT[src.dtype], m, d, src_ld, out.data_ptr(),
                                        out.shape[1], _stream_ptr(src.device))
    _check(st, "mmrag_f8_encode_rows")
    return out[:m]


def maxsim_topk_workspace_bytes(Q: int, n_items: int, k: int, dim: int = 0, max_tiles: int = 0,
                                dtype: torch.dtype = torch.float16) -> int:
    if dtype not in (torch.float16, torch.float8_e4m3fn):
        raise ValueError(f"maxsim_topk_workspace_bytes: dtype must be float16 or float8_e4m3fn (got {dtype})")
    L, f8 = lib(), dtype == torch.float8_e4m3fn
    if not dim:
        fn = L.mmrag_maxsim_topk_f8_workspace_bytes if f8 else L.mmrag_maxsim_topk_workspace_bytes
        return int(fn(int(Q), int(n_items), int(k)))
    fn = L.mmrag_internal_maxsim_topk_f8_workspace_bytes_ex if f8 else L.mmrag_internal_maxsim_topk_workspace_bytes_ex
    return int(fn(int(Q), int(n_items), int(k), int(dim), int(max_tiles)))


def late_question_tiles(q_start, q_len, q_rows: int) -> int:
    tiles, used = 0, MAX_LATE_QUERY_TOKENS + 1
    for a, n in zip(q_start, q_len):
        if not 1 <= n <= MAX_LATE_QUERY_TOKENS or a < 0 or a + n > q_rows:
            continue
        if used + n > MAX_LATE_QUERY_TOKENS:
            tiles, used = tiles + 1, 0
        used += n
    return max(tiles, 1)


def maxsim_topk(q_tok: torch.Tensor, q_start, q_len, tok: torch.Tensor, n_rows: int, item_off: torch.Tensor,
                n_items: int, dim: int, k: int, alive_bits: Optional[torch.Tensor] = None,
                workspace: Optional[torch.Tensor] = None, chunk_rows: int = 0, cap: int = 0, dbg: int = 0,
                check_tables: bool = True, _f8: bool = False):
    who, row_dtype = ("maxsim_topk_f8", torch.uint8) if _f8 else ("maxsim_topk", torch.float16)
    _dev_check(q_tok, tok, item_off)
    for name, t in (("q_tok", q_tok), ("tok", tok)):
        if t.dim() != 2 or not t.is_contiguous() or t.dtype != row_dtype:
            raise MMRagNativeError(f"{who}: {name} must be a contiguous 2-D {_DT_NAME[row_dtype]} tensor")
    dev = q_tok.device
    n_rows, n_items, k = int(n_rows), int(n_items), int(k)
    if not 1 <= k <= MAX_K_DEEP:
        raise ValueError(f"{who}: k={k} outside 1..{MAX_K_DEEP}")
    if tok.device != dev or item_off.device != dev or (alive_bits is not None and alive_bits.device != dev):
        raise MMRagNativeError(f"{who}: q_tok, tok, item_off and alive_bits must be on one device")
    if not 0 <= n_rows <= tok.shape[0]:
        raise MMRagNativeError(f"{who}: n_rows={n_rows} outside the {tok.shape[0]} rows of tok")
    if (item_off.dim() != 1 or item_off.dtype != torch.int32 or not item_off.is_contiguous() or n_items < 0
            or item_off.numel() < n_items + 1):
        raise MMRagNativeError(f"{who}: item_off must be a contiguous int32 tensor of at least n_items + 1 = "
                               f"{n_items + 1} offsets")
    if alive_bits is not None and (alive_bits.dtype != torch.int32 or not alive_bits.is_contiguous()
                                   or alive_bits.numel() * 32 < n_items):
        raise MMRagNativeError(f"{who}: alive_bits must be a contiguous int32 bitmap over {n_items} items")
    tables = [torch.as_tensor(t, dtype=torch.int32).reshape(-1).cpu() for t in (q_start, q_len)]
    Q = tables[0].numel()
    if tables[1].numel() != Q or not 1 <= Q <= MAX_LATE_QUESTIONS:
        raise MMRagNativeError(f"{who}: q_start and q_len must hold the same 1..{MAX_LATE_QUESTIONS} questions "
                               f"(got {Q} and {tables[1].numel()})")
    if check_tables:
        for s, (a, n) in enumerate(zip(tables[0].tolist(), tables[1].tolist())):
            if not 1 <= n <= MAX_LATE_QUERY_TOKENS:
                raise MMRagNativeError(f"{who}: question {s} has {n} tokens, outside 1..{MAX_LATE_QUERY_TOKENS}")
            if a < 0 or a + n > q_tok.shape[0]:
                raise MMRagNativeError(f"{who}: question {s} (rows {a}..{a + n}) is outside the "
                                       f"{q_tok.shape[0]} rows given")
    packed = _pinned_to_device(torch.cat(tables), dev)
    tiles = late_question_tiles(tables[0].tolist(), tables[1].tolist(), q_tok.shape[0])
    need = maxsim_topk_workspace_bytes(Q, n_items, k, int(dim), tiles, torch.float8_e4m3fn if _f8 else torch.float16)
    if need == 0:
        raise MMRagNativeError(f"{who}: dim must be a multiple of 64, at most 1024 (dim={dim})")
    if workspace is None or _nbytes(workspace) < need:
        workspace = torch.empty(max(need, 16), dtype=torch.uint8, device=dev)
    out_s, out_r = _topk_out(Q, k, dev)
    with torch.cuda.device(dev):
        fn = lib().mmrag_internal_maxsim_topk_f8_ex if _f8 else lib().mmrag_internal_maxsim_topk_ex
        st = fn(
            q_tok.data_ptr(), q_tok.shape[0], q_tok.shape[1], packed.data_ptr(), packed[Q:].data_ptr(), Q,
            tok.data_ptr(), n_rows, tok.shape[1], item_off.data_ptr(), n_items, _ptr(alive_bits), int(dim), k,
            out_s.data_ptr(), out_r.data_ptr(), workspace.data_ptr(), _nbytes(workspace), _stream_ptr(dev),
            int(chunk_rows), int(cap), int(dbg), tiles)
    _check(st, "mmrag_" + who)
    return out_s, out_r


def maxsim_topk_f8(q_codes: torch.Tensor, q_start, q_len, codes: torch.Tensor, n_rows: int, item_off: torch.Tensor,
                   n_items: int, dim: int, k: int, alive_bits: Optional[torch.Tensor] = None,
                   workspace: Optional[torch.Tensor] = None, chunk_rows: int = 0, cap: int = 0, dbg: int = 0,
                   check_tables: bool = True):
    return maxsim_topk(q_codes, q_start, q_len, codes, n_rows, item_off, n_items, dim, k, alive_bits, workspace,
                       chunk_rows, cap, dbg, check_tables, _f8=True)


def join_tile(T: int, at: int, slot_order: bool = False) -> Tuple[int, int]:
    ti, tj = c_int64(0), c_int64(0)
    fn = lib().mmrag_internal_join_slot_tile if slot_order else lib().mmrag_internal_join_tile
    _check(fn(int(T), int(at), ctypes.byref(ti), ctypes.byref(tj)), "mmrag_internal_join_tile")
    return ti.value, tj.value


def device_info() -> dict:
    cus, mhz, mem = c_int(0), c_int(0), c_int64(0)
    _check(lib().mmrag_device_info(ctypes.byref(cus), ctypes.byref(mhz), ctypes.byref(mem)), "mmrag_device_info")
    return {"compute_units": cus.value, "max_clock_mhz": mhz.value, "hbm_bytes": mem.value}


def measure_peaks(device: torch.device, seconds: float = 0.4) -> dict:
    L = lib()
    out = {}
    with torch.cuda.device(device):
        stream = _stream_ptr(device)
        nbytes = 1 << 30
        src = torch.empty(nbytes, dtype=torch.uint8, device=device)
        dst = torch.empty(nbytes, dtype=torch.uint8, device=device)
        src.zero_()
        e0, e1 = torch.cuda.Event(enable_timing=True), torch.cuda.Event(enable_timing=True)

        def timed(fn, min_s):
            import time
            fn(); torch.cuda.synchronize(device)
            t_end = time.time() + min_s / 2
            while time.time() < t_end:
                for _ in range(4): fn()
                torch.cuda.synchronize(device)
            n = 0
            e0.record()
            t_end = time.time() + min_s / 2
            while time.time() < t_end:
                for _ in range(4): fn()
                n += 4
                torch.cuda.synchronize(device)
            e1.record(); torch.cuda.synchronize(device)
            return e0.elapsed_time(e1) * 1e-3 / n

        t = timed(lambda: _check(L.mmrag_bench_stream_copy(dst.data_ptr(), src.data_ptr(), nbytes, stream), "copy"), seconds)
        out["stream_copy_GBps"] = round(2 * nbytes / t / 1e9, 1)
        sink = torch.empty(256 * 8 * 256, dtype=torch.float32, device=device)
        t = timed(lambda: _check(L.mmrag_bench_stream_read(src.data_ptr(), nbytes, sink.data_ptr(), stream), "read"), seconds)
        out["stream_read_GBps"] = round(nbytes / t / 1e9, 1)
        t = timed(lambda: _check(L.mmrag_bench_stream_write(dst.data_ptr(), nbytes, stream), "write"), seconds)
        out["stream_write_GBps"] = round(nbytes / t / 1e9, 1)
        del src, dst, sink
        seed = (torch.randn(256 * 8, device=device) * 0.5).to(torch.float16)
        res = torch.empty(256 * 1024, dtype=torch.float32, device=device)
        flops = c_int64(0)
        iters = 20000
        t = timed(lambda: _check(L.mmrag_bench_mfma_f16(seed.data_ptr(), res.data_ptr(), iters, ctypes.byref(flops), stream),
                                 "mfma"), seconds)
        out["mfma_f16_TFLOPs"] = round(flops.value / t / 1e12, 1)
        iters = 5000
        t = timed(lambda: _check(L.mmrag_bench_mfma_f16_16x16x32(seed.data_ptr(), res.data_ptr(), iters,
                                                                 ctypes.byref(flops), stream), "mfma16"), seconds)
        out["mfma_f16_16x16x32_TFLOPs"] = round(flops.value / t / 1e12, 1)
    return out


def cosine_topk_workspace_bytes(B: int, n: int, k: int) -> int:
    return int(lib().mmrag_cosine_topk_workspace_bytes(B, n, k))


def merge_topk(scores: torch.Tensor, rows: torch.Tensor, k: int) -> Tuple[torch.Tensor, torch.Tensor]:
    _dev_check(scores, rows)
    G, B, k_in = scores.shape
    scores = scores.contiguous()
    rows = rows.contiguous()
    out_s, out_r = _topk_out(B, k, scores.device)
    with torch.cuda.device(scores.device):
        st = lib().mmrag_merge_topk(scores.data_ptr(), rows.data_ptr(), G, B, k_in, k, out_s.data_ptr(),
                                    out_r.data_ptr(), _stream_ptr(scores.device))
    _check(st, "mmrag_merge_topk")
    return out_s, out_r


def merge_topk_host(scores: torch.Tensor, rows: torch.Tensor, k: int) -> Tuple[torch.Tensor, torch.Tensor]:
    if scores.is_cuda or rows.is_cuda:
        raise MMRagNativeError("merge_topk_host takes CPU tensors")
    G, B, k_in = scores.shape
    scores = scores.contiguous().to(torch.float32)
    rows = rows.contiguous().to(torch.int64)
    out_s = torch.empty((B, k), dtype=torch.float32)
    out_r = torch.empty((B, k), dtype=torch.int64)
    st = lib().mmrag_merge_topk_host(scores.data_ptr(), rows.data_ptr(), G, B, k_in, k, out_s.data_ptr(),
                                     out_r.data_ptr())
    _check(st, "mmrag_merge_topk_host")
    return out_s, out_r


def packed_block_bytes(B: int, k: int) -> int:
    return (B * k * 12 + 7) // 8 * 8


def merge_topk_host_packed(blocks: torch.Tensor, G: int, B: int, k_in: int, k: int) -> Tuple[torch.Tensor, torch.Tensor]:
    if blocks.is_cuda or blocks.dtype != torch.uint8 or blocks.numel() != G * packed_block_bytes(B, k_in):
        raise MMRagNativeError("merge_topk_host_packed takes a CPU uint8 tensor of G * packed_block_bytes(B, k_in) bytes")
    out_s = torch.empty((B, k), dtype=torch.float32)
    out_r = torch.empty((B, k), dtype=torch.int64)
    st = lib().mmrag_merge_topk_host_packed(blocks.data_ptr(), G, B, k_in, k, out_s.data_ptr(), out_r.data_ptr())
    _check(st, "mmrag_merge_topk_host_packed")
    return out_s, out_r


def append_rows(corpus: torch.Tensor, n_used: int, new_rows: torch.Tensor, d: int) -> None:
    _dev_check(corpus, new_rows)
    new_rows = new_rows.to(torch.float32).contiguous()
    m = new_rows.shape[0]
    with torch.cuda.device(corpus.device):
        st = lib().mmrag_append_rows(corpus.data_ptr(), corpus.shape[0], corpus.shape[1], _TORCH2DT[corpus.dtype],
                                     n_used, new_rows.data_ptr(), m, d, _stream_ptr(corpus.device))
    _check(st, "mmrag_append_rows")


def gather_rows(dst: torch.Tensor, src: torch.Tensor, keep_rows: torch.Tensor) -> None:
    _dev_check(dst, src, keep_rows)
    keep_rows = keep_rows.to(torch.int64).contiguous()
    with torch.cuda.device(src.device):
        st = lib().mmrag_gather_rows(dst.data_ptr(), src.data_ptr(), src.shape[1], _TORCH2DT[src.dtype],
                                     keep_rows.data_ptr(), keep_rows.numel(), _stream_ptr(src.device))
    _check(st, "mmrag_gather_rows")


def fetch_rows_f32(corpus: torch.Tensor, rows: torch.Tensor, d: int) -> torch.Tensor:
    _dev_check(corpus, rows)
    rows = rows.to(torch.int64).contiguous()
    out = torch.empty((rows.numel(), d), dtype=torch.float32, device=corpus.device)
    with torch.cuda.device(corpus.device):
        st = lib().mmrag_fetch_rows_f32(corpus.data_ptr(), corpus.shape[1], _TORCH2DT[corpus.dtype], rows.data_ptr(),
                                        rows.numel(), d, out.data_ptr(), _stream_ptr(corpus.device))
    _check(st, "mmrag_fetch_rows_f32")
    return out


def cosine_topk_lists(q: torch.Tensor, corpus: torch.Tensor, n: int, d: int, k: int, workspace: torch.Tensor,
                      alive_bits: Optional[torch.Tensor] = None, dbg: int = 0) -> None:
    _dev_check(q, corpus, workspace, alive_bits)
    if q.dtype != corpus.dtype or q.shape[1] != corpus.shape[1] or not q.is_contiguous() or not corpus.is_contiguous():
        raise MMRagNativeError("cosine_topk_lists: q and corpus must be contiguous and share dtype and padded width")
    if n > corpus.shape[0]:
        raise MMRagNativeError(f"cosine_topk_lists: n={n} exceeds corpus capacity {corpus.shape[0]}")
    B, ld = q.shape
    with torch.cuda.device(q.device):
        st = lib().mmrag_internal_cosine_topk_lists_ex(
            q.data_ptr(), corpus.data_ptr(), B, n, d, ld, _TORCH2DT[q.dtype], k,
            alive_bits.data_ptr() if alive_bits is not None else None, workspace.data_ptr(),
            _nbytes(workspace), _stream_ptr(q.device), int(dbg))
    _check(st, "mmrag_cosine_topk_lists")


def cosine_topk_select(B: int, n: int, k: int, row_offset: int, workspace: torch.Tensor,
                       out_scores: Optional[torch.Tensor] = None,
                       out_rows: Optional[torch.Tensor] = None) -> Tuple[torch.Tensor, torch.Tensor]:
    _dev_check(workspace)
    dev = workspace.device
    if out_scores is None:
        out_scores = torch.empty((B, k), dtype=torch.float32, device=dev)
    if out_rows is None:
        out_rows = torch.empty((B, k), dtype=torch.int64, device=dev)
    with torch.cuda.device(dev):
        st = lib().mmrag_cosine_topk_select(B, n, k, row_offset, workspace.data_ptr(), out_scores.data_ptr(),
                                            out_rows.data_ptr(), _stream_ptr(dev))
    _check(st, "mmrag_cosine_topk_select")
    return out_scores, out_rows


ACT_NONE, ACT_GELU, ACT_QUICK_GELU = 0, 1, 2
ARCH_BERT, ARCH_PRELN = 0, 1
POOL_MEAN, POOL_FIRST, POOL_SELECT = 0, 1, 2


class EncoderDesc(ctypes.Structure):
    _fields_ = [("arch", c_int32), ("n_layers", c_int32), ("hidden", c_int32), ("n_heads", c_int32),
                ("intermediate", c_int32), ("vocab", c_int32), ("max_pos", c_int32), ("pool", c_int32),
                ("act", c_int32), ("causal", c_int32), ("normalize", c_int32), ("out_dim", c_int32),
                ("ln_eps", c_float), ("image", c_int32), ("patch", c_int32)]


def _ptr(t: Optional[torch.Tensor]):
    return t.data_ptr() if t is not None else None


def linear_f16(x: torch.Tensor, wt: torch.Tensor, bias: Optional[torch.Tensor] = None, act: int = ACT_NONE,
               resid: Optional[torch.Tensor] = None, out: Optional[torch.Tensor] = None) -> torch.Tensor:
    _dev_check(x, wt, bias, resid, out)
    M, K = x.shape
    Nf = wt.shape[0]
    if x.dtype != torch.float16 or wt.dtype != torch.float16 or wt.shape[1] != K:
        raise MMRagNativeError("linear_f16: x [M,K] and wt [N,K] must be fp16 with matching K")
    if out is None:
        out = torch.empty((M, Nf), dtype=torch.float16, device=x.device)
    with torch.cuda.device(x.device):
        st = lib().mmrag_linear_f16(x.data_ptr(), M, K, wt.data_ptr(), Nf, _ptr(bias), act, _ptr(resid),
                                    out.data_ptr(), _stream_ptr(x.device))
    _check(st, "mmrag_linear_f16")
    return out


def layernorm_f16(x: torch.Tensor, gamma: torch.Tensor, beta: torch.Tensor, eps: float) -> torch.Tensor:
    _dev_check(x, gamma, beta)
    out = torch.empty_like(x)
    with torch.cuda.device(x.device):
        st = lib().mmrag_layernorm_f16(x.data_ptr(), out.data_ptr(), gamma.data_ptr(), beta.data_ptr(), x.shape[0],
                                       x.shape[1], eps, _stream_ptr(x.device))
    _check(st, "mmrag_layernorm_f16")
    return out


def embed_ln_f16(ids, pos_ids, tok, pos, type0, gamma, beta, eps: float) -> torch.Tensor:
    _dev_check(ids, pos_ids, tok, pos, type0, gamma, beta)
    T, H = ids.numel(), tok.shape[1]
    out = torch.empty((T, H), dtype=torch.float16, device=tok.device)
    with torch.cuda.device(tok.device):
        st = lib().mmrag_embed_ln_f16(ids.data_ptr(), pos_ids.data_ptr(), tok.data_ptr(), pos.data_ptr(), _ptr(type0),
                                      _ptr(gamma), _ptr(beta), out.data_ptr(), T, H, tok.shape[0], pos.shape[0], eps,
                                      _stream_ptr(tok.device))
    _check(st, "mmrag_embed_ln_f16")
    return out


def attention_f16(qkv: torch.Tensor, cu_seqlens: torch.Tensor, max_len: int, n_heads: int,
                  causal: bool = False) -> torch.Tensor:
    _dev_check(qkv, cu_seqlens)
    T, H3 = qkv.shape
    H = H3 // 3
    ctx = torch.empty((T, H), dtype=torch.float16, device=qkv.device)
    with torch.cuda.device(qkv.device):
        st = lib().mmrag_attention_f16(qkv.data_ptr(), cu_seqlens.data_ptr(), ctx.data_ptr(), cu_seqlens.numel() - 1,
                                       max_len, H, n_heads, int(causal), _stream_ptr(qkv.device))
    _check(st, "mmrag_attention_f16")
    return ctx


def pool_normalize_f16(x: torch.Tensor, cu_seqlens: torch.Tensor, pool: int, normalize: bool = True,
                       sel: Optional[torch.Tensor] = None) -> torch.Tensor:
    _dev_check(x, cu_seqlens, sel)
    B, H = cu_seqlens.numel() - 1, x.shape[1]
    out = torch.empty((B, H), dtype=torch.float32, device=x.device)
    with torch.cuda.device(x.device):
        st = lib().mmrag_pool_normalize_f16(x.data_ptr(), cu_seqlens.data_ptr(), _ptr(sel), out.data_ptr(), B, H, pool,
                                            int(normalize), _stream_ptr(x.device))
    _check(st, "mmrag_pool_normalize_f16")
    return out


def linear_f16_norms(x: torch.Tensor, wt: torch.Tensor, bias: Optional[torch.Tensor] = None, act: int = ACT_NONE,
                     resid: Optional[torch.Tensor] = None, ln_gamma: Optional[torch.Tensor] = None,
                     ln_beta: Optional[torch.Tensor] = None, ln_eps: float = 1e-12,
                     ln_stats_out: Optional[torch.Tensor] = None, res_stats: Optional[torch.Tensor] = None,
                     res_gamma: Optional[torch.Tensor] = None, res_beta: Optional[torch.Tensor] = None) -> torch.Tensor:
    _dev_check(x, wt, bias, resid, ln_gamma, ln_beta, ln_stats_out, res_stats, res_gamma, res_beta)
    M, K = x.shape
    Nf = wt.shape[0]
    out = torch.empty((M, Nf), dtype=torch.float16, device=x.device)
    with torch.cuda.device(x.device):
        st = lib().mmrag_internal_linear_f16_norms(x.data_ptr(), M, K, wt.data_ptr(), Nf, _ptr(bias), act, _ptr(resid),
                                                   out.data_ptr(), _ptr(ln_gamma), _ptr(ln_beta), ln_eps,
                                                   _ptr(ln_stats_out), _ptr(res_stats), _ptr(res_gamma), _ptr(res_beta),
                                                   _stream_ptr(x.device))
    _check(st, "mmrag_internal_linear_f16_norms")
    return out


def attention_f32(qkv: torch.Tensor, cu_seqlens: torch.Tensor, max_len: int, n_heads: int) -> torch.Tensor:
    _dev_check(qkv, cu_seqlens)
    T, H3 = qkv.shape
    ctx = torch.empty((T, H3 // 3), dtype=torch.float32, device=qkv.device)
    with torch.cuda.device(qkv.device):
        st = lib().mmrag_internal_attention_f32(qkv.data_ptr(), cu_seqlens.data_ptr(), ctx.data_ptr(),
                                                cu_seqlens.numel() - 1, max_len, H3 // 3, n_heads,
                                                _stream_ptr(qkv.device))
    _check(st, "mmrag_internal_attention_f32")
    return ctx


def layernorm_f32(x: torch.Tensor, gamma: torch.Tensor, beta: torch.Tensor, eps: float) -> torch.Tensor:
    _dev_check(x, gamma, beta)
    out = torch.empty_like(x)
    with torch.cuda.device(x.device):
        st = lib().mmrag_internal_layernorm_f32(x.data_ptr(), out.data_ptr(), gamma.data_ptr(), beta.data_ptr(),
                                                x.shape[0], x.shape[1], eps, _stream_ptr(x.device))
    _check(st, "mmrag_internal_layernorm_f32")
    return out


def pool_norm_f32(x: torch.Tensor, cu_seqlens: torch.Tensor, pool: int, normalize: bool = True,
                  sel: Optional[torch.Tensor] = None) -> torch.Tensor:
    _dev_check(x, cu_seqlens, sel)
    B, H = cu_seqlens.numel() - 1, x.shape[1]
    out = torch.empty((B, H), dtype=torch.float32, device=x.device)
    with torch.cuda.device(x.device):
        st = lib().mmrag_internal_pool_norm_f32(x.data_ptr(), cu_seqlens.data_ptr(), _ptr(sel), out.data_ptr(), B, H,
                                                pool, int(normalize), _stream_ptr(x.device))
    _check(st, "mmrag_internal_pool_norm_f32")
    return out


def encoder_workspace_bytes(desc: EncoderDesc, T: int, B: int, f32: bool = False) -> int:
    if f32:
        return int(lib().mmrag_encoder_f32_workspace_bytes(ctypes.byref(desc), T, B))
    return int(lib().mmrag_encoder_workspace_bytes(ctypes.byref(desc), T, B))


def linear_f32(x: torch.Tensor, wt: torch.Tensor, bias: Optional[torch.Tensor] = None, act: int = ACT_NONE,
               resid: Optional[torch.Tensor] = None) -> torch.Tensor:
    _dev_check(x, wt, bias, resid)
    M, K = x.shape
    N = wt.shape[0]
    out = torch.empty((M, N), dtype=torch.float32, device=x.device)
    with torch.cuda.device(x.device):
        st = lib().mmrag_linear_f32(x.data_ptr(), M, K, wt.data_ptr(), N, _ptr(bias), act, _ptr(resid), out.data_ptr(),
                                    _stream_ptr(x.device))
    _check(st, "mmrag_linear_f32")
    return out


def encoder_forward(desc: EncoderDesc, weight_ptrs, ids: torch.Tensor, pos_ids: torch.Tensor,
                    cu_seqlens: torch.Tensor, max_len: int, sel: Optional[torch.Tensor] = None,
                    workspace: Optional[torch.Tensor] = None, out: Optional[torch.Tensor] = None,
                    f32: bool = False) -> torch.Tensor:
    _dev_check(ids, pos_ids, cu_seqlens, sel, workspace, out)
    T, B = ids.numel(), cu_seqlens.numel() - 1
    need = encoder_workspace_bytes(desc, T, B, f32)
    if workspace is None or _nbytes(workspace) < need:
        workspace = torch.empty(need, dtype=torch.uint8, device=ids.device)
    if out is None:
        out = torch.empty((B, desc.out_dim), dtype=torch.float32, device=ids.device)
    fn = lib().mmrag_encoder_forward_f32 if f32 else lib().mmrag_encoder_forward
    with torch.cuda.device(ids.device):
        st = fn(ctypes.byref(desc), weight_ptrs, ids.data_ptr(), pos_ids.data_ptr(),
                                         cu_seqlens.data_ptr(), _ptr(sel), T, B, max_len, out.data_ptr(),
                                         workspace.data_ptr(), _nbytes(workspace),
                                         _stream_ptr(ids.device))
    _check(st, "mmrag_encoder_forward")
    return out


def encoder_tokens_workspace_bytes(desc: EncoderDesc, T: int, B: int, out_dim: int) -> int:
    return int(lib().mmrag_encoder_tokens_workspace_bytes(ctypes.byref(desc), T, B, int(out_dim)))


def encoder_forward_tokens(desc: EncoderDesc, weight_ptrs, ids: torch.Tensor, pos_ids: torch.Tensor,
                           cu_seqlens: torch.Tensor, max_len: int, proj: Optional[torch.Tensor] = None,
                           workspace: Optional[torch.Tensor] = None, out: Optional[torch.Tensor] = None) -> torch.Tensor:
    _dev_check(ids, pos_ids, cu_seqlens, proj, workspace, out)
    T, B = ids.numel(), cu_seqlens.numel() - 1
    out_dim = desc.hidden
    if proj is not None:
        if proj.dim() != 2 or proj.dtype != torch.float16 or not proj.is_contiguous() or proj.shape[1] != desc.hidden:
            raise MMRagNativeError("encoder_forward_tokens: proj must be a contiguous [out_dim, hidden] float16 tensor")
        out_dim = int(proj.shape[0])
    need = encoder_tokens_workspace_bytes(desc, T, B, out_dim)
    if workspace is None or _nbytes(workspace) < need:
        workspace = torch.empty(max(need, 16), dtype=torch.uint8, device=ids.device)
    if out is None:
        out = torch.empty((max(T, 1), max(out_dim, 1)), dtype=torch.float16, device=ids.device)
    with torch.cuda.device(ids.device):
        st = lib().mmrag_encoder_forward_tokens(ctypes.byref(desc), weight_ptrs, ids.data_ptr(), pos_ids.data_ptr(),
                                                cu_seqlens.data_ptr(), T, B, max_len, _ptr(proj), out_dim,
                                                out.data_ptr(), workspace.data_ptr(), _nbytes(workspace),
                                                _stream_ptr(ids.device))
    _check(st, "mmrag_encoder_forward_tokens")
    return out


MAX_SPARSE_CHUNK_TOKENS, MAX_SPARSE_CHUNKS, MAX_SPARSE_VOCAB = 512, 65536, 65536
MAX_SPARSE_TERMS, MAX_SPARSE_QUERY_TERMS = 256, 64


def sparse_limits() -> dict:
    v = [ctypes.c_int(0) for _ in range(5)]
    _check(lib().mmrag_internal_sparse_limits(*[ctypes.byref(x) for x in v]), "mmrag_internal_sparse_limits")
    return dict(zip(("impact_rows", "pool_batch", "pool_vrun", "select_terms", "tile_rows"), (int(x.value) for x in v)))


def sparse_expand_forward_workspace_bytes(desc: EncoderDesc, T: int, B: int) -> int:
    return int(lib().mmrag_sparse_expand_forward_workspace_bytes(ctypes.byref(desc), T, B))


def sparse_expand_forward(desc: EncoderDesc, weight_ptrs, ids: torch.Tensor, pos_ids: torch.Tensor,
                          cu_seqlens: torch.Tensor, max_len: int, head_w: torch.Tensor, head_b: torch.Tensor,
                          head_ln_g: torch.Tensor, head_ln_b: torch.Tensor, workspace: Optional[torch.Tensor] = None,
                          out: Optional[torch.Tensor] = None) -> torch.Tensor:
    _dev_check(ids, pos_ids, cu_seqlens, head_w, head_b, head_ln_g, head_ln_b, workspace, out)
    T, B, H = ids.numel(), cu_seqlens.numel() - 1, desc.hidden
    if head_w.dtype != torch.float16 or tuple(head_w.shape) != (H, H) or not head_w.is_contiguous():
        raise MMRagNativeError("sparse_expand_forward: head_w must be a contiguous [hidden, hidden] float16 tensor")
    for t in (head_b, head_ln_g, head_ln_b):
        if t.dtype != torch.float32 or t.numel() != H or not t.is_contiguous():
            raise MMRagNativeError("sparse_expand_forward: head bias / LayerNorm vectors must be [hidden] float32")
    need = sparse_expand_forward_workspace_bytes(desc, T, B)
    if workspace is None or _nbytes(workspace) < need:
        workspace = torch.empty(max(need, 16), dtype=torch.uint8, device=ids.device)
    if out is None:
        out = torch.empty((max(T, 1), H), dtype=torch.float16, device=ids.device)
    with torch.cuda.device(ids.device):
        st = lib().mmrag_sparse_expand_forward(ctypes.byref(desc), weight_ptrs, ids.data_ptr(), pos_ids.data_ptr(),
                                               cu_seqlens.data_ptr(), T, B, max_len, head_w.data_ptr(),
                                               head_b.data_ptr(), head_ln_g.data_ptr(), head_ln_b.data_ptr(),
                                               out.data_ptr(), workspace.data_ptr(), _nbytes(workspace),
                                               _stream_ptr(ids.device))
    _check(st, "mmrag_sparse_expand_forward")
    return out


def sparse_pool(tok: torch.Tensor, cu: torch.Tensor, E: torch.Tensor, dim: int, n_rows: Optional[int] = None,
                V: Optional[int] = None, vrun: int = 0) -> torch.Tensor:
    _dev_check(tok, cu, E)
    for name, t in (("tok", tok), ("E", E)):
        if t.dim() != 2 or t.dtype != torch.float16 or not t.is_contiguous():
            raise MMRagNativeError(f"sparse_pool: {name} must be a contiguous 2-D float16 tensor")
    if cu.dtype != torch.int32 or cu.dim() != 1 or not cu.is_contiguous() or cu.numel() < 2:
        raise MMRagNativeError("sparse_pool: cu must be a contiguous int32 vector of n_chunks + 1 offsets")
    T = tok.shape[0] if n_rows is None else int(n_rows)
    V = E.shape[0] if V is None else int(V)
    if T > tok.shape[0] or V > E.shape[0]:
        raise MMRagNativeError("sparse_pool: n_rows / V exceed the tensors")
    n_chunks = cu.numel() - 1
    pooled = torch.empty((max(n_chunks, 1), max(V, 1)), dtype=torch.float32, device=tok.device)
    with torch.cuda.device(tok.device):
        args = (tok.data_ptr(), T, tok.shape[1], cu.data_ptr(), n_chunks, E.data_ptr(), V, E.shape[1], int(dim),
                pooled.data_ptr())
        if vrun:
            st = lib().mmrag_internal_sparse_pool_ex(*args, _stream_ptr(tok.device), int(vrun))
        else:
            st = lib().mmrag_sparse_pool(*args, None, 0, _stream_ptr(tok.device))
    _check(st, "mmrag_sparse_pool")
    return pooled


def sparse_select(pooled: torch.Tensor, bias: torch.Tensor, scale: float, m: int,
                  skip_bits: Optional[torch.Tensor] = None) -> Tuple[torch.Tensor, torch.Tensor, torch.Tensor]:
    _dev_check(pooled, bias, skip_bits)
    if pooled.dim() != 2 or pooled.dtype != torch.float32 or not pooled.is_contiguous():
        raise MMRagNativeError("sparse_select: pooled must be a contiguous [n_chunks, V] float32 tensor")
    n_chunks, V = pooled.shape
    if bias.dtype != torch.float32 or bias.numel() != V or not bias.is_contiguous():
        raise MMRagNativeError("sparse_select: bias must be a contiguous [V] float32 tensor")
    if skip_bits is not None and (skip_bits.dtype != torch.int32 or skip_bits.numel() < (V + 31) // 32
                                  or not skip_bits.is_contiguous()):
        raise MMRagNativeError("sparse_select: skip_bits must be ceil(V / 32) int32 words")
    dev = pooled.device
    cnt = torch.empty(max(n_chunks, 1), dtype=torch.int32, device=dev)
    terms = torch.empty((max(n_chunks, 1), max(int(m), 1)), dtype=torch.int32, device=dev)
    imps = torch.empty_like(terms)
    with torch.cuda.device(dev):
        st = lib().mmrag_sparse_select(pooled.data_ptr(), bias.data_ptr(), _ptr(skip_bits), n_chunks, V, float(scale),
                                       int(m), cnt.data_ptr(), terms.data_ptr(), imps.data_ptr(), _stream_ptr(dev))
    _check(st, "mmrag_sparse_select")
    return cnt, terms, imps


def impact_topk_workspace_bytes(B: int, n: int, k: int) -> int:
    return int(lib().mmrag_impact_topk_workspace_bytes(B, n, k))


def impact_topk(term_off: torch.Tensor, post_row: torch.Tensor, post_imp: torch.Tensor, n_terms: int, n: int,
                q_off: torch.Tensor, q_terms: torch.Tensor, q_imp: torch.Tensor, k: int,
                alive_bits: Optional[torch.Tensor] = None, workspace: Optional[torch.Tensor] = None,
                cap: int = 0, dbg: int = 0) -> Tuple[torch.Tensor, torch.Tensor]:
    _dev_check(term_off, post_row, post_imp, q_off, q_terms, q_imp, alive_bits, workspace)
    B = q_off.numel() - 1
    dev = q_off.device
    need = impact_topk_workspace_bytes(B, n, k)
    if workspace is None or _nbytes(workspace) < need:
        workspace = torch.empty(max(need, 16), dtype=torch.uint8, device=dev)
    out_s, out_r = _topk_out(max(B, 1), max(k, 1), dev)
    args = (term_off.data_ptr(), post_row.data_ptr(), post_imp.data_ptr(), int(n_terms), int(n), q_off.data_ptr(),
            q_terms.data_ptr(), q_imp.data_ptr(), B, int(k), _ptr(alive_bits), out_s.data_ptr(), out_r.data_ptr(),
            workspace.data_ptr(), _nbytes(workspace), _stream_ptr(dev))
    with torch.cuda.device(dev):
        if cap or dbg:
            st = lib().mmrag_internal_impact_topk_ex(*args, int(cap), int(dbg))
        else:
            st = lib().mmrag_impact_topk(*args)
    _check(st, "mmrag_impact_topk")
    return out_s, out_r


def cross_encoder_workspace_bytes(desc: EncoderDesc, T: int, B: int, f32: bool = False) -> int:
    fn = lib().mmrag_cross_encoder_f32_workspace_bytes if f32 else lib().mmrag_cross_encoder_workspace_bytes
    return int(fn(ctypes.byref(desc), T, B))


def cross_encoder_forward(desc: EncoderDesc, weight_ptrs, n_labels: int, ids: torch.Tensor, type_ids: torch.Tensor,
                          pos_ids: torch.Tensor, cu_seqlens: torch.Tensor, max_len: int,
                          workspace: Optional[torch.Tensor] = None, out: Optional[torch.Tensor] = None,
                          f32: bool = False) -> torch.Tensor:
    _dev_check(ids, type_ids, pos_ids, cu_seqlens, workspace, out)
    T, B = ids.numel(), cu_seqlens.numel() - 1
    need = cross_encoder_workspace_bytes(desc, T, B, f32)
    if workspace is None or _nbytes(workspace) < need:
        workspace = torch.empty(need, dtype=torch.uint8, device=ids.device)
    if out is None:
        out = torch.empty((B, n_labels), dtype=torch.float32, device=ids.device)
    fn = lib().mmrag_cross_encoder_forward_f32 if f32 else lib().mmrag_cross_encoder_forward
    with torch.cuda.device(ids.device):
        st = fn(ctypes.byref(desc), weight_ptrs, n_labels, ids.data_ptr(), type_ids.data_ptr(), pos_ids.data_ptr(),
                cu_seqlens.data_ptr(), T, B, max_len, out.data_ptr(), workspace.data_ptr(),
                _nbytes(workspace), _stream_ptr(ids.device))
    _check(st, "mmrag_cross_encoder_forward")
    return out


def _reader_outs(B: int, T: int, n_best: int, logits: bool, dev):
    n = max(int(n_best), 1)
    return (torch.empty((B, n, 2), dtype=torch.int32, device=dev), torch.empty((B, n), dtype=torch.float32, device=dev),
            torch.empty(B, dtype=torch.float32, device=dev), torch.empty((B, 2), dtype=torch.float32, device=dev),
            torch.empty((T, 2), dtype=torch.float32, device=dev) if logits else None)


def _reader_tables(cu_seqlens, ctx_start, ctx_len):
    B = cu_seqlens.numel() - 1
    for t in (cu_seqlens, ctx_start, ctx_len):
        if t.dtype != torch.int32 or t.dim() != 1 or not t.is_contiguous():
            raise MMRagNativeError("reader: cu_seqlens / ctx_start / ctx_len must be contiguous int32 vectors")
    if B < 1 or ctx_start.numel() != B or ctx_len.numel() != B:
        raise MMRagNativeError("reader: ctx_start / ctx_len need one entry per sequence")
    return B


def span_select(hidden: torch.Tensor, qa_w: torch.Tensor, qa_b: torch.Tensor, cu_seqlens: torch.Tensor,
                ctx_start: torch.Tensor, ctx_len: torch.Tensor, max_answer_tokens: int, n_best: int,
                logits: bool = False, hidden_dim: Optional[int] = None):
    _dev_check(hidden, qa_w, qa_b, cu_seqlens, ctx_start, ctx_len)
    if hidden.dim() != 2 or hidden.dtype != torch.float16 or not hidden.is_contiguous():
        raise MMRagNativeError("span_select: hidden must be a contiguous [T, ld] float16 tensor")
    T, ld = hidden.shape
    H = ld if hidden_dim is None else int(hidden_dim)
    if qa_w.dtype != torch.float32 or tuple(qa_w.shape) != (2, H) or not qa_w.is_contiguous() \
            or qa_b.dtype != torch.float32 or qa_b.numel() != 2 or not qa_b.is_contiguous():
        raise MMRagNativeError("span_select: qa_w must be [2, hidden] and qa_b [2], contiguous float32")
    B = _reader_tables(cu_seqlens, ctx_start, ctx_len)
    span, score, null, lse, lg = _reader_outs(B, T, n_best, logits, hidden.device)
    with torch.cuda.device(hidden.device):
        st = lib().mmrag_span_select(hidden.data_ptr(), ld, H, qa_w.data_ptr(), qa_b.data_ptr(), cu_seqlens.data_ptr(),
                                     ctx_start.data_ptr(), ctx_len.data_ptr(), T, B, int(max_answer_tokens),
                                     int(n_best), span.data_ptr(), score.data_ptr(), null.data_ptr(), lse.data_ptr(),
                                     _ptr(lg), _stream_ptr(hidden.device))
    _check(st, "mmrag_span_select")
    return span, score, null, lse, lg


def reader_workspace_bytes(desc: EncoderDesc, T: int, B: int) -> int:
    return int(lib().mmrag_reader_workspace_bytes(ctypes.byref(desc), T, B))


def reader_forward(desc: EncoderDesc, weight_ptrs, ids: torch.Tensor, type_ids: torch.Tensor, pos_ids: torch.Tensor,
                   cu_seqlens: torch.Tensor, ctx_start: torch.Tensor, ctx_len: torch.Tensor, max_len: int,
                   max_answer_tokens: int, n_best: int, logits: bool = False,
                   workspace: Optional[torch.Tensor] = None):
    _dev_check(ids, type_ids, pos_ids, cu_seqlens, ctx_start, ctx_len, workspace)
    T = ids.numel()
    B = _reader_tables(cu_seqlens, ctx_start, ctx_len)
    need = reader_workspace_bytes(desc, T, B)
    if workspace is None or _nbytes(workspace) < need:
        workspace = torch.empty(max(need, 16), dtype=torch.uint8, device=ids.device)
    span, score, null, lse, lg = _reader_outs(B, T, n_best, logits, ids.device)
    with torch.cuda.device(ids.device):
        st = lib().mmrag_reader_forward(ctypes.byref(desc), weight_ptrs, ids.data_ptr(), type_ids.data_ptr(),
                                        pos_ids.data_ptr(), cu_seqlens.data_ptr(), ctx_start.data_ptr(),
                                        ctx_len.data_ptr(), T, B, int(max_len), int(max_answer_tokens), int(n_best),
                                        span.data_ptr(), score.data_ptr(), null.data_ptr(), lse.data_ptr(), _ptr(lg),
                                        workspace.data_ptr(), _nbytes(workspace), _stream_ptr(ids.device))
    _check(st, "mmrag_reader_forward")
    return span, score, null, lse, lg


def embed_types_ln(ids, type_ids, pos_ids, tok, pos, type_tab, gamma, beta, eps: float) -> torch.Tensor:
    _dev_check(ids, type_ids, pos_ids, tok, pos, type_tab, gamma, beta)
    T, H = ids.numel(), tok.shape[1]
    f32 = tok.dtype == torch.float32
    out = torch.empty((T, H), dtype=tok.dtype, device=tok.device)
    fn = lib().mmrag_internal_embed_types_ln_f32 if f32 else lib().mmrag_internal_embed_types_ln_f16
    with torch.cuda.device(tok.device):
        st = fn(ids.data_ptr(), type_ids.data_ptr(), pos_ids.data_ptr(), tok.data_ptr(), pos.data_ptr(),
                type_tab.data_ptr(), gamma.data_ptr(), beta.data_ptr(), out.data_ptr(), T, H, tok.shape[0], pos.shape[0],
                type_tab.shape[0], eps, _stream_ptr(tok.device))
    _check(st, "mmrag_internal_embed_types_ln")
    return out


def cls_head_f32(cls: torch.Tensor, wp, bp, wc, bc) -> torch.Tensor:
    _dev_check(cls, wp, bp, wc, bc)
    B, H = cls.shape
    NL = wc.shape[0]
    ws = torch.empty(int(lib().mmrag_internal_cls_head_workspace_bytes(B, H, NL)) + 256, dtype=torch.uint8,
                     device=cls.device)
    off = (-ws.data_ptr()) % 256
    out = torch.empty((B, NL), dtype=torch.float32, device=cls.device)
    with torch.cuda.device(cls.device):
        st = lib().mmrag_internal_cls_head_f32(cls.data_ptr(), wp.data_ptr(), bp.data_ptr(), wc.data_ptr(), bc.data_ptr(),
                                               out.data_ptr(), B, H, NL, ws.data_ptr() + off, ws.numel() - off,
                                               _stream_ptr(cls.device))
    _check(st, "mmrag_internal_cls_head_f32")
    return out


PIXELS_F16_CHW, PIXELS_U8_HWC = 0, 1


def vit_forward(desc: EncoderDesc, weight_ptrs, pixels: torch.Tensor, pixel_kind: int, cu_seqlens: torch.Tensor,
                workspace: Optional[torch.Tensor] = None, out: Optional[torch.Tensor] = None) -> torch.Tensor:
    _dev_check(pixels, cu_seqlens, workspace, out)
    B = pixels.shape[0]
    S = (desc.image // desc.patch) ** 2 + 1
    need = encoder_workspace_bytes(desc, B * S, B)
    if workspace is None or _nbytes(workspace) < need:
        workspace = torch.empty(need, dtype=torch.uint8, device=pixels.device)
    if out is None:
        out = torch.empty((B, desc.out_dim), dtype=torch.float32, device=pixels.device)
    with torch.cuda.device(pixels.device):
        st = lib().mmrag_vit_forward(ctypes.byref(desc), weight_ptrs, pixels.data_ptr(), pixel_kind,
                                     cu_seqlens.data_ptr(), B, out.data_ptr(), workspace.data_ptr(),
                                     _nbytes(workspace), _stream_ptr(pixels.device))
    _check(st, "mmrag_vit_forward")
    return out


def patchify(pixels: torch.Tensor, image: int, patch: int) -> torch.Tensor:
    _dev_check(pixels)
    kind = PIXELS_U8_HWC if pixels.dtype == torch.uint8 else PIXELS_F16_CHW
    want = (image, image, 3) if kind == PIXELS_U8_HWC else (3, image, image)
    if pixels.dtype not in (torch.uint8, torch.float16) or tuple(pixels.shape[1:]) != want or not pixels.is_contiguous():
        raise MMRagNativeError(f"patchify: bad pixel tensor {tuple(pixels.shape)} {pixels.dtype}")
    if patch <= 0 or image % patch != 0:
        raise MMRagNativeError(f"patchify: bad image/patch {image}/{patch}")
    B, G = pixels.shape[0], image // patch
    out = torch.empty((B, G * G, 3 * patch * patch), dtype=torch.float16, device=pixels.device)
    with torch.cuda.device(pixels.device):
        st = lib().mmrag_internal_patchify(pixels.data_ptr(), kind, out.data_ptr(), B, image, patch,
                                           _stream_ptr(pixels.device))
    _check(st, "mmrag_internal_patchify")
    return out


def vit_assemble_ln(emb: torch.Tensor, cls: torch.Tensor, pos: torch.Tensor, gamma: torch.Tensor, beta: torch.Tensor,
                    eps: float) -> torch.Tensor:
    _dev_check(emb, cls, pos, gamma, beta)
    B, S, H = emb.shape[0], pos.shape[0], pos.shape[1]
    if tuple(emb.shape) != (B, S - 1, H) or cls.numel() != H or gamma.numel() != H or beta.numel() != H:
        raise MMRagNativeError("vit_assemble_ln: emb [B, S-1, H], cls [H], pos [S, H], gamma / beta [H]")
    if any(t.dtype != torch.float16 or not t.is_contiguous() for t in (emb, cls, pos)):
        raise MMRagNativeError("vit_assemble_ln: emb, cls, pos must be contiguous fp16")
    out = torch.empty((B * S, H), dtype=torch.float16, device=emb.device)
    with torch.cuda.device(emb.device):
        st = lib().mmrag_internal_vit_assemble_ln(emb.data_ptr(), cls.data_ptr(), pos.data_ptr(), gamma.data_ptr(),
                                                  beta.data_ptr(), out.data_ptr(), B, S, H, eps,
                                                  _stream_ptr(emb.device))
    _check(st, "mmrag_internal_vit_assemble_ln")
    return out


def normalize_rows(x: torch.Tensor) -> torch.Tensor:
    _dev_check(x)
    if x.dtype != torch.float16 or x.dim() != 2 or not x.is_contiguous():
        raise MMRagNativeError("normalize_rows: x must be contiguous fp16 [B, D]")
    out = torch.empty(x.shape, dtype=torch.float32, device=x.device)
    with torch.cuda.device(x.device):
        st = lib().mmrag_internal_normalize_rows(x.data_ptr(), out.data_ptr(), x.shape[0], x.shape[1],
                                                 _stream_ptr(x.device))
    _check(st, "mmrag_internal_normalize_rows")
    return out


def pool_f16(x: torch.Tensor, cu_seqlens: torch.Tensor, pool: int, sel: Optional[torch.Tensor] = None) -> torch.Tensor:
    _dev_check(x, cu_seqlens, sel)
    if x.dtype != torch.float16 or x.dim() != 2 or not x.is_contiguous():
        raise MMRagNativeError("pool_f16: x must be contiguous fp16 [T, H]")
    B, H = cu_seqlens.numel() - 1, x.shape[1]
    out = torch.empty((B, H), dtype=torch.float16, device=x.device)
    with torch.cuda.device(x.device):
        st = lib().mmrag_internal_pool_f16(x.data_ptr(), cu_seqlens.data_ptr(), _ptr(sel), out.data_ptr(), B, H, pool,
                                           _stream_ptr(x.device))
    _check(st, "mmrag_internal_pool_f16")
    return out


def resample_coeffs(in_size: int, out_size: int, first: int, count: int):
    import numpy as np

    ks = lib().mmrag_resample_ksize(in_size, out_size)
    bounds = np.zeros((count, 2), np.int32)
    taps = np.zeros((count, max(ks, 1)), np.int32)
    _check(lib().mmrag_resample_coeffs(in_size, out_size, first, count, bounds.ctypes.data, taps.ctypes.data),
           "mmrag_resample_coeffs")
    return bounds, taps


def resize_crop_u8(src: torch.Tensor, bx: torch.Tensor, kx: torch.Tensor, by: torch.Tensor, ky: torch.Tensor,
                   y_lo: int, y_hi: int, out: Optional[torch.Tensor] = None) -> torch.Tensor:
    _dev_check(src, bx, kx, by, ky, out)
    if src.dtype != torch.uint8 or src.dim() != 3 or src.shape[2] != 3 or src.stride(2) != 1 or src.stride(1) != 3:
        raise MMRagNativeError("resize_crop_u8: src must be [H, W, 3] uint8 with packed pixels")
    H, W = int(src.shape[0]), int(src.shape[1])
    out_h, out_w = int(by.shape[0]), int(bx.shape[0])
    if out is None:
        out = torch.empty((out_h, out_w, 3), dtype=torch.uint8, device=src.device)
    tmp = torch.empty(((y_hi - y_lo) * out_w * 3,), dtype=torch.uint8, device=src.device)
    with torch.cuda.device(src.device):
        st = lib().mmrag_resize_crop_u8(src.data_ptr(), H, W, src.stride(0), bx.data_ptr(), kx.data_ptr(),
                                        int(kx.shape[1]), by.data_ptr(), ky.data_ptr(), int(ky.shape[1]), out_h, out_w,
                                        y_lo, y_hi, tmp.data_ptr(), out.data_ptr(), _stream_ptr(src.device))
    _check(st, "mmrag_resize_crop_u8")
    return out


def copy_to_host_async(dst_host: torch.Tensor, src_dev: torch.Tensor, stream: int) -> None:
    nbytes = src_dev.numel() * src_dev.element_size()
    if dst_host.is_cuda or not src_dev.is_cuda or dst_host.numel() * dst_host.element_size() < nbytes:
        raise MMRagNativeError("copy_to_host_async: need a host destination at least as large as the device source")
    _check(lib().mmrag_copy_to_host_async(dst_host.data_ptr(), src_dev.data_ptr(), nbytes, stream),
           "mmrag_copy_to_host_async")


class SearchPlan:

    def __init__(self, q: torch.Tensor, corpus: torch.Tensor, n: int, d: int, k: int, workspace: torch.Tensor,
                 alive_bits: Optional[torch.Tensor] = None):
        _dev_check(q, corpus, workspace, alive_bits)
        if q.dtype != corpus.dtype or q.shape[1] != corpus.shape[1] or not q.is_contiguous() or not corpus.is_contiguous():
            raise MMRagNativeError("SearchPlan: q and corpus must be contiguous and share dtype and padded width")
        if n > corpus.shape[0]:
            raise MMRagNativeError(f"SearchPlan: n={n} exceeds corpus capacity {corpus.shape[0]}")
        need = lib().mmrag_cosine_topk_workspace_bytes(q.shape[0], n, k)
        if _nbytes(workspace) < need:
            raise MMRagNativeError("SearchPlan: workspace too small")
        self._keep = (q, corpus, workspace, alive_bits)
        self.B, self.n, self.k = q.shape[0], n, k
        self._scan_args = (q.data_ptr(), corpus.data_ptr(), q.shape[0], n, d, q.shape[1], _TORCH2DT[q.dtype], k,
                           alive_bits.data_ptr() if alive_bits is not None else None, workspace.data_ptr(),
                           _nbytes(workspace))
        self._ws = workspace.data_ptr()
        self._scan = lib().mmrag_cosine_topk_lists
        self._select = lib().mmrag_cosine_topk_select

    def scan(self, stream: int) -> None:
        st = self._scan(*self._scan_args, stream)
        if st:
            _check(st, "mmrag_cosine_topk_lists")

    def select(self, row_offset: int, out_scores_ptr: int, out_rows_ptr: int, stream: int) -> None:
        st = self._select(self.B, self.n, self.k, row_offset, self._ws, out_scores_ptr, out_rows_ptr, stream)
        if st:
            _check(st, "mmrag_cosine_topk_select")
```

multimodal_rag_amd/csrc/search.hip:

```cpp
#include "slab_ring.h"

#include <stdlib.h>

using namespace mmrag;

namespace mmrag_impl {

template <int DT, int WN, int K, int NSTAGE, int NW, bool SEEDED>
__global__ __launch_bounds__(64 * NW, NW / 4) void cosine_topk_kernel(const KParams p) {
#if defined(__HIP_DEVICE_COMPILE__)
#include "slab_ring_body.inc"
#endif
}

template <int K>
struct FullList {
    float v[K];
    long long r[K];
    __device__ inline void init() {
#pragma unroll
        for (int i = 0; i < K; ++i) {
            v[i] = NEG_INF;
            r[i] = LLONG_MAX;
        }
    }
    __device__ inline void insert(float x, long long xr) {
#pragma unroll
        for (int j = 0; j < K; ++j) {
            const bool b = better(x, xr, v[j], r[j]);
            const float nv = b ? x : v[j];
            const float nx = b ? v[j] : x;
            const long long nr = b ? xr : r[j];
            const long long nxr = b ? r[j] : xr;
            v[j] = nv;
            x = nx;
            r[j] = nr;
            xr = nxr;
        }
    }
    __device__ inline void pop() {
#pragma unroll
        for (int j = 0; j + 1 < K; ++j) {
            v[j] = v[j + 1];
            r[j] = r[j + 1];
        }
        v[K - 1] = NEG_INF;
        r[K - 1] = LLONG_MAX;
    }
};

template <int K>
__device__ inline void wave_extract(FullList<K> &l, float *out_v, long long *out_r) {
#pragma unroll
    for (int round = 0; round < K; ++round) {
        float s = l.v[0];
        long long r = l.r[0];
#pragma unroll
        for (int off = 32; off >= 1; off >>= 1) {
            const float os = __shfl_xor(s, off);
            const long long orr = __shfl_xor(r, off);
            if (better(os, orr, s, r)) {
                s = os;
                r = orr;
            }
        }
        out_v[round] = s;
        out_r[round] = r;
        if (l.v[0] == s && l.r[0] == r) l.pop();
    }
}

template <int K, typename RowT>
__global__ __launch_bounds__(256) void merge_topk_kernel(const float *__restrict__ cs,
                                                          const RowT *__restrict__ cr, long long n_cand,
                                                          long long inner, long long outer_stride,
                                                          long long q_stride, int k_out,
                                                          long long row_offset, float *__restrict__ out_s,
                                                          long long *__restrict__ out_r,
                                                          float *__restrict__ thr0, float *__restrict__ seed_s,
                                                          int *__restrict__ seed_r, long long seed_q_stride) {
    __shared__ float sh_v[4 * K];
    __shared__ long long sh_r[4 * K];
    const int q = blockIdx.x;
    const int lane = threadIdx.x & 63;
    const int wave = threadIdx.x >> 6;
    constexpr long long PAD = sizeof(RowT) == 4 ? (long long)INT_MAX : LLONG_MAX;

    FullList<K> l;
    l.init();
    for (long long c = threadIdx.x; c < n_cand; c += 256) {
        const long long a = (c / inner) * outer_stride + (long long)q * q_stride + (c % inner);
        const float s = cs[a];
        long long r = (long long)cr[a];
        if (r == PAD || r < 0) continue;
        if (better(s, r, l.v[K - 1], l.r[K - 1])) l.insert(s, r);
    }
    float ov[K];
    long long orr[K];
    wave_extract<K>(l, ov, orr);
    if (lane == 0) {
#pragma unroll
        for (int i = 0; i < K; ++i) {
            sh_v[wave * K + i] = ov[i];
            sh_r[wave * K + i] = orr[i];
        }
    }
    __syncthreads();
    if (wave == 0) {
        l.init();
        for (int i = lane; i < 4 * K; i += 64)
            if (sh_r[i] != LLONG_MAX) l.insert(sh_v[i], sh_r[i]);
        wave_extract<K>(l, ov, orr);
        if (lane == 0) {
#pragma unroll
            for (int i = 0; i < K; ++i) {
                if (i < k_out) {
                    const bool valid = orr[i] != LLONG_MAX && ov[i] > NEG_INF;
                    out_s[(size_t)q * k_out + i] = valid ? ov[i] : NEG_INF;
                    out_r[(size_t)q * k_out + i] = valid ? orr[i] + row_offset : -1;
                }
            }
            if (thr0 != nullptr) {
                const bool full = orr[K - 1] != LLONG_MAX && ov[K - 1] > NEG_INF;
                thr0[q] = full ? ov[K - 1] : NEG_INF;
#pragma unroll
                for (int i = 0; i < K; ++i) {
                    const bool valid = orr[i] != LLONG_MAX && ov[i] > NEG_INF;
                    seed_s[(size_t)q * seed_q_stride + i] = valid ? ov[i] : NEG_INF;
                    seed_r[(size_t)q * seed_q_stride + i] = valid ? (int)orr[i] : INT_MAX;
                }
            }
        }
    }
}

struct Plan {
    int K;
    int WN;
    int NW;
    int grid_x, grid_y;
    int n_tiles;
    int n_lists;
    int b_pad;
    int pre_tiles;
    bool qs_ok;
    bool qs_room;
};

constexpr unsigned DBG_NO_PREPASS = 1u, DBG_8_WAVES = 2u, DBG_NO_QS = 4u, DBG_FORCE_QS = 8u;
constexpr unsigned DBG_OLD_QS = 0x10000u, DBG_MFMA32 = 0x20000u, DBG_MFMA16 = 0x40000u, DBG_NO_DYN = 0x80000u,
                   DBG_NO_SEED = 0x100000u;

Plan make_plan(int B, long long n, int k, unsigned dbg = 0) {
    Plan pl;
    pl.K = k <= 5 ? 5 : (k <= 10 ? 10 : 20);
    pl.WN = plan_wn(B);
    const int qrows = 32 * pl.WN;
    pl.grid_y = (B + qrows - 1) / qrows;
    pl.n_tiles = (int)((n + TM - 1) / TM);
    const int cus = num_cus();
    pl.grid_x = plan_walkers(pl.n_tiles, pl.grid_y);
    pl.NW = (pl.K == 5 && pl.WN == 8 && !(dbg & DBG_8_WAVES)) ? 16 : 8;
    pl.pre_tiles = 0;
    const bool want_pre = (pl.WN == 8 || pl.K > 5) && pl.n_tiles >= 3 * cus;
    if (want_pre && !(dbg & DBG_NO_PREPASS)) pl.pre_tiles = cus;
    pl.n_lists = pl.grid_x + (want_pre ? 1 : 0);
    pl.b_pad = pl.grid_y * qrows;
    pl.qs_room = pl.WN == 8 && pl.n_tiles >= cus;
    const bool long_enough = pl.K <= 5 ? pl.n_tiles * 4 >= 15 * cus : pl.n_tiles >= 6 * cus;
    pl.qs_ok = pl.qs_room && !(dbg & DBG_NO_QS) && (long_enough || (dbg & DBG_FORCE_QS));
    return pl;
}

template <int DT, int WN, int K, int NSTAGE, int NW = 8, bool SEEDED = false>
void launch_main(const KParams &p, dim3 grid, hipStream_t s) {
    KParams kp = p;
    kp.walkers = (int)grid.x;
    kp.share_l2 = grid.y > 1;
    cosine_topk_kernel<DT, WN, K, NSTAGE, NW, SEEDED><<<grid.x * grid.y, 64 * NW, 0, s>>>(kp);
}

template <int DT, int K>
void dispatch_deep(const Plan &pl, const KParams &p, dim3 grid, hipStream_t s) {
    if (pl.WN == 2) launch_main<DT, 2, K, 3>(p, grid, s);
    else if (pl.WN == 4) launch_main<DT, 4, K, 3>(p, grid, s);
    else if (p.thr0) launch_main<DT, 8, K, 2, 8, true>(p, grid, s);
    else launch_main<DT, 8, K, 2>(p, grid, s);
}

template <int DT>
int dispatch_main(const Plan &pl, const KParams &p, hipStream_t s) {
    dim3 grid(pl.grid_x, pl.grid_y);
    if (pl.K == 5) {
        if (pl.WN == 2) launch_main<DT, 2, 5, 3>(p, grid, s);
        else if (pl.WN == 4) launch_main<DT, 4, 5, 3>(p, grid, s);
        else if (pl.NW == 16 && p.thr0) launch_main<DT, 8, 5, 2, 16, true>(p, grid, s);
        else if (pl.NW == 16) launch_main<DT, 8, 5, 2, 16>(p, grid, s);
        else if (p.thr0) launch_main<DT, 8, 5, 2, 8, true>(p, grid, s);
        else launch_main<DT, 8, 5, 2>(p, grid, s);
    } else if (pl.K == 10) {
        dispatch_deep<DT, 10>(pl, p, grid, s);
    } else {
        dispatch_deep<DT, 20>(pl, p, grid, s);
    }
    return MMRAG_OK;
}

template <int DT>
void launch_filter(int WN, const KParams &p, dim3 grid, hipStream_t s) {
    if (WN == 2) launch_main<DT, 2, 0, 3>(p, grid, s);
    else if (WN == 4) launch_main<DT, 4, 0, 3>(p, grid, s);
    else if constexpr (DT == MMRAG_F32) launch_main<DT, 8, 0, 2, 8>(p, grid, s);
    else launch_main<DT, 8, 0, 2, 16>(p, grid, s);
}

int deep_filter_launch(int dtype, int WN, const KParams &p, int grid_x, int grid_y, hipStream_t s) {
    if (dtype == MMRAG_F8E4M3) return f8_filter_launch(WN, p, grid_x, grid_y, s);
    const dim3 grid(grid_x, grid_y);
    with_elem_type(dtype, [&](auto tag) { launch_filter<decltype(tag)::value>(WN, p, grid, s); });
    MMRAG_CHECK_HIP(hipGetLastError());
    return MMRAG_OK;
}

template <typename RowT>
int launch_merge(int K, const float *cs, const RowT *cr, long long n_cand, long long inner,
                 long long outer_stride, long long q_stride, int B, int k_out, long long row_offset,
                 float *out_s, long long *out_r, hipStream_t s, float *thr0 = nullptr, float *seed_s = nullptr,
                 int *seed_r = nullptr, long long seed_q_stride = 0) {
    if (K == 5)
        merge_topk_kernel<5, RowT><<<B, 256, 0, s>>>(cs, cr, n_cand, inner, outer_stride, q_stride, k_out,
                                                     row_offset, out_s, out_r, thr0, seed_s, seed_r, seed_q_stride);
    else if (K == 10)
        merge_topk_kernel<10, RowT><<<B, 256, 0, s>>>(cs, cr, n_cand, inner, outer_stride, q_stride, k_out,
                                                      row_offset, out_s, out_r, thr0, seed_s, seed_r, seed_q_stride);
    else
        merge_topk_kernel<20, RowT><<<B, 256, 0, s>>>(cs, cr, n_cand, inner, outer_stride, q_stride, k_out,
                                                      row_offset, out_s, out_r, thr0, seed_s, seed_r, seed_q_stride);
    return MMRAG_OK;
}

__global__ void fill_empty_kernel(float *s, long long *r, long long total) {
    const long long i = (long long)blockIdx.x * blockDim.x + threadIdx.x;
    if (i < total) {
        s[i] = NEG_INF;
        r[i] = -1;
    }
}

__global__ void fill_seed_empty_kernel(float *s, int *r, long long q_stride, int K, long long n_queries) {
    const long long q = (long long)blockIdx.x * blockDim.x + threadIdx.x;
    if (q < n_queries)
        for (int i = 0; i < K; ++i) {
            s[q * q_stride + i] = NEG_INF;
            r[q * q_stride + i] = INT_MAX;
        }
}

int check_search_args(const char *name, int k_max, const void *q, const void *corpus, int B, int64_t n, int d, int64_t ld,
                      int dtype, int k) {
    MMRAG_CHECK_ARG(dtype >= 0 && dtype <= MMRAG_F8E4M3, "%s: bad dtype %d", name, dtype);
    MMRAG_CHECK_ARG(B > 0, "%s: B must be positive (got %d)", name, B);
    MMRAG_CHECK_ARG(k >= 1 && k <= k_max, "%s: k=%d outside 1..%d", name, k, k_max);
    MMRAG_CHECK_ARG(n >= 0 && n < (int64_t)INT_MAX - TM, "%s: n=%lld out of range", name, (long long)n);
    MMRAG_CHECK_ARG(d > 0 && ld >= d, "%s: need 0 < d <= ld (d=%d ld=%lld)", name, d, (long long)ld);
    const int64_t row_bytes = ld * esize(dtype);
    MMRAG_CHECK_ARG(row_bytes % SLAB == 0, "%s: row bytes %lld not a multiple of %d (use mmrag_padded_dim)", name,
                    (long long)row_bytes, SLAB);
    MMRAG_CHECK_ARG(row_bytes * TM < (int64_t)UINT_MAX, "%s: rows too long", name);
    MMRAG_CHECK_ARG(q, "%s: null q", name);
    MMRAG_CHECK_ARG(n == 0 || corpus, "%s: null corpus", name);
    MMRAG_CHECK_ARG(((uintptr_t)q % 16) == 0 && ((uintptr_t)corpus % 16) == 0, "%s: q/corpus must be 16-byte aligned",
                    name);
    return MMRAG_OK;
}

}
using namespace mmrag_impl;

extern "C" {

struct WsLayout {
    size_t entries, off_r, off_thr, off_ts, off_tr, off_cnt, cnt_bytes, off_pub, off_pthr, off_tk, xch_end, total;
};
static WsLayout ws_layout(const Plan &pl) {
    WsLayout w;
    w.entries = (size_t)pl.b_pad * pl.n_lists * pl.K;
    w.off_r = w.entries * sizeof(float);
    w.off_thr = w.off_r + w.entries * sizeof(int);
    w.off_ts = w.off_thr + (size_t)pl.b_pad * sizeof(float);
    w.off_tr = (w.off_ts + (size_t)pl.b_pad * pl.K * sizeof(float) + 15) / 16 * 16;
    w.off_cnt = (w.off_tr + (size_t)pl.b_pad * pl.K * sizeof(long long) + 63) / 64 * 64;
    w.cnt_bytes = 0;
    w.off_pub = w.off_cnt + w.cnt_bytes;
    w.off_pthr = w.off_pub + (pl.qs_room ? (size_t)pl.b_pad * pl.grid_x * sizeof(float) : 0);
    w.off_tk = w.off_pthr + (pl.qs_room ? (size_t)pl.b_pad * sizeof(float) : 0);
    w.xch_end = w.off_tk + (pl.qs_room ? ((size_t)pl.grid_y * sizeof(unsigned) + 63) / 64 * 64 : 0);
    w.total = w.xch_end;
    return w;
}

size_t mmrag_cosine_topk_workspace_bytes(int B, int64_t n, int k) {
    if (B <= 0 || n < 0 || k < 1 || k > MMRAG_MAX_K) return 0;
    return ws_layout(make_plan(B, n, k)).total + 256;
}

int mmrag_internal_cosine_topk_lists_ex(const void *q, const void *corpus, int B, int64_t n, int d, int64_t ld,
                                        int dtype, int k, const uint32_t *alive_bits, void *workspace,
                                        size_t workspace_bytes, void *stream, unsigned dbg) {
    if (int st = check_search_args("cosine_topk", MMRAG_MAX_K, q, corpus, B, n, d, ld, dtype, k)) return st;
    if (n == 0) return MMRAG_OK;
    const Plan pl = make_plan(B, n, k, dbg);
    const WsLayout wl = ws_layout(pl);
    if (!workspace || workspace_bytes < wl.total) {
        set_error("cosine_topk: workspace %zu bytes < required %zu", workspace_bytes, wl.total);
        return MMRAG_EWORKSPACE;
    }
    MMRAG_CHECK_ARG(((uintptr_t)workspace % 16) == 0, "cosine_topk: workspace must be 16-byte aligned");

    KParams p;
    p.q = (const char *)q;
    p.corpus = (const char *)corpus;
    p.alive_bits = alive_bits;
    p.cand_s = (float *)workspace;
    p.cand_r = (int *)((char *)workspace + wl.off_r);
    p.n = n;
    p.B = B;
    p.row_bytes = (unsigned)(ld * esize(dtype));
    p.n_tiles = pl.n_tiles;
    p.n_lists = pl.n_lists;
    p.tile0 = 0;
    p.thr0 = nullptr;
    p.dbg = dbg;
    p.stamps = ((dbg & DBG_QS_CLOCK) && workspace_bytes >= wl.total + 256 * (size_t)(pl.grid_x * pl.grid_y)) ? (unsigned long long *)((char *)workspace + wl.total) : nullptr;
    p.walkers = pl.grid_x;
    p.share_l2 = pl.grid_y > 1;
    p.sample_best = nullptr;
    p.pub_best = nullptr;
    p.pub_thr = nullptr;
    p.tickets = nullptr;
    p.p_static = INT_MAX / 2;
    hipStream_t s = (hipStream_t)stream;
    const size_t seed_off = (size_t)(pl.n_lists - 1) * pl.K;
    const int walk_mfma = (dbg & DBG_MFMA32) ? 32 : ((dbg & DBG_MFMA16) ? 16 : (pl.K == 5 ? QSW_DEFAULT_MFMA : 32));
    if (pl.qs_ok && !(dbg & DBG_OLD_QS) && qsw_supported(dtype, p.row_bytes, pl.K, walk_mfma)) {
        const int tiles = (int)((n + QS_TILE_ROWS - 1) / QS_TILE_ROWS);
        const int per = tiles / pl.grid_x;
        p.n_tiles = tiles;
        p.pub_best = nullptr;
        p.pub_thr = nullptr;
        p.tickets = nullptr;
        p.p_static = INT_MAX / 2;
        const bool seed = per >= 12 && !(dbg & DBG_NO_SEED);
        const bool dyn = pl.grid_y == 1 && per >= 24 && !(dbg & DBG_NO_DYN);
        if (seed || dyn) {
            MMRAG_CHECK_HIP(hipMemsetD32Async((hipDeviceptr_t)((char *)workspace + wl.off_pub), (int)TICKET0,
                                              (wl.xch_end - wl.off_pub) / 4, s));
            if (seed) {
                p.pub_best = (float *)((char *)workspace + wl.off_pub);
                p.pub_thr = (float *)((char *)workspace + wl.off_pthr);
            }
            if (dyn) {
                p.tickets = (unsigned *)((char *)workspace + wl.off_tk);
                const int tail = per / 10 > 3 ? per / 10 : 3;
                p.p_static = per - tail;
            }
        }
        if (int st = qsw_launch(dtype, pl.K, walk_mfma, p, pl.grid_x, pl.grid_y, s)) return st;
        MMRAG_CHECK_HIP(hipGetLastError());
        return MMRAG_OK;
    }
    if (pl.qs_ok && qs_supported(dtype, p.row_bytes, pl.K)) {
        const int tiles = (int)((n + QS_TILE_ROWS - 1) / QS_TILE_ROWS);
        float *thr0 = nullptr;
        if (pl.pre_tiles > 0) {
            KParams ks = p;
            ks.n_tiles = pl.pre_tiles * (TM / QS_TILE_ROWS);
            ks.sample_best = (float *)((char *)workspace + wl.off_pub);
            if (int st = qs_launch(dtype, pl.K, ks, pl.grid_x, pl.grid_y, s)) return st;
            thr0 = (float *)((char *)workspace + wl.off_thr);
            if (int st = qs_seed_thresholds(pl.K, ks.sample_best, pl.grid_x, pl.b_pad, thr0, s)) return st;
        }
        p.n_tiles = tiles;
        p.thr0 = thr0;
        if (int st = qs_launch(dtype, pl.K, p, pl.grid_x, pl.grid_y, s)) return st;
        MMRAG_CHECK_HIP(hipGetLastError());
        return MMRAG_OK;
    }
    auto run = [&](int tile0, int n_tiles, int grid_x, const float *thr0) -> int {
        KParams kp = p;
        kp.tile0 = tile0;
        kp.n_tiles = n_tiles;
        kp.thr0 = thr0;
        Plan lp = pl;
        lp.grid_x = grid_x;
        if (dtype == MMRAG_F8E4M3) return f8_lists_launch(lp.K, lp.WN, kp, lp.grid_x, lp.grid_y, s);
        return with_elem_type(dtype, [&](auto tag) { return dispatch_main<decltype(tag)::value>(lp, kp, s); });
    };
    if (pl.pre_tiles > 0) {
        float *thr0 = (float *)((char *)workspace + wl.off_thr);
        float *top_s = (float *)((char *)workspace + wl.off_ts);
        long long *top_r = (long long *)((char *)workspace + wl.off_tr);
        const int pre = pl.pre_tiles;
        const int pre_grid = pre < pl.grid_x ? pre : pl.grid_x;
        if (int st = run(0, pre, pre_grid, nullptr)) return st;
        MMRAG_CHECK_HIP(hipGetLastError());
        const long long n_cand = (long long)pre_grid * pl.K;
        launch_merge<int>(pl.K, p.cand_s, p.cand_r, n_cand, n_cand, 0, (long long)pl.n_lists * pl.K, B, pl.K, 0, top_s,
                          top_r, s, thr0, p.cand_s + seed_off, p.cand_r + seed_off, (long long)pl.n_lists * pl.K);
        MMRAG_CHECK_HIP(hipGetLastError());
        if (int st = run(pre, pl.n_tiles - pre, pl.grid_x, thr0)) return st;
    } else {
        if (pl.n_lists > pl.grid_x) {
            const long long total = (long long)pl.b_pad;
            fill_seed_empty_kernel<<<(unsigned)((total + 255) / 256), 256, 0, s>>>(
                p.cand_s + seed_off, p.cand_r + seed_off, (long long)pl.n_lists * pl.K, pl.K, total);
        }
        if (int st = run(0, pl.n_tiles, pl.grid_x, nullptr)) return st;
    }
    MMRAG_CHECK_HIP(hipGetLastError());
    return MMRAG_OK;
}

int mmrag_internal_search_uses_qs(int B, int64_t n, int64_t ld, int dtype, int k) {
    if (B <= 0 || n <= 0 || k <= 0 || k > MMRAG_MAX_K) return 0;
    const Plan pl = make_plan(B, n, k, 0u);
    const unsigned rb = (unsigned)(ld * esize(dtype));
    if (!pl.qs_ok) return 0;
    if (qsw_supported(dtype, rb, pl.K, QSW_DEFAULT_MFMA)) return 2;
    return qs_supported(dtype, rb, pl.K) ? 1 : 0;
}

int mmrag_cosine_topk_lists(const void *q, const void *corpus, int B, int64_t n, int d, int64_t ld, int dtype,
                            int k, const uint32_t *alive_bits, void *workspace, size_t workspace_bytes,
                            void *stream) {
    return mmrag_internal_cosine_topk_lists_ex(q, corpus, B, n, d, ld, dtype, k, alive_bits, workspace,
                                               workspace_bytes, stream, 0u);
}

int mmrag_cosine_topk_select(int B, int64_t n, int k, int64_t row_offset, const void *workspace,
                             float *out_scores, int64_t *out_rows, void *stream) {
    MMRAG_CHECK_ARG(B > 0 && n >= 0 && k >= 1 && k <= MMRAG_MAX_K, "cosine_topk_select: bad shape");
    MMRAG_CHECK_ARG(out_scores && out_rows, "cosine_topk_select: null output");
    hipStream_t s = (hipStream_t)stream;
    if (n == 0) {
        const long long total = (long long)B * k;
        fill_empty_kernel<<<(unsigned)((total + 255) / 256), 256, 0, s>>>(out_scores, (long long *)out_rows, total);
        MMRAG_CHECK_HIP(hipGetLastError());
        return MMRAG_OK;
    }
    MMRAG_CHECK_ARG(workspace, "cosine_topk_select: null workspace");
    const Plan pl = make_plan(B, n, k);
    const WsLayout wl = ws_layout(pl);
    const float *cand_s = (const float *)workspace;
    const int *cand_r = (const int *)((const char *)workspace + wl.off_r);
    const long long n_cand = (long long)pl.n_lists * pl.K;
    launch_merge<int>(pl.K, cand_s, cand_r, n_cand, n_cand, 0, n_cand, B, k, row_offset, out_scores,
                      (long long *)out_rows, s);
    MMRAG_CHECK_HIP(hipGetLastError());
    return MMRAG_OK;
}

int mmrag_cosine_topk(const void *q, const void *corpus, int B, int64_t n, int d, int64_t ld, int dtype,
                      int k, int64_t row_offset, const uint32_t *alive_bits, float *out_scores,
                      int64_t *out_rows, void *workspace, size_t workspace_bytes, void *stream) {
    if (int st = mmrag_cosine_topk_lists(q, corpus, B, n, d, ld, dtype, k, alive_bits, workspace, workspace_bytes,
                                         stream))
        return st;
    return mmrag_cosine_topk_select(B, n, k, row_offset, workspace, out_scores, out_rows, stream);
}

int mmrag_merge_topk(const float *scores, const int64_t *rows, int G, int B, int k_in, int k,
                     float *out_scores, int64_t *out_rows, void *stream) {
    MMRAG_CHECK_ARG(scores && rows && out_scores && out_rows, "merge_topk: null pointer");
    MMRAG_CHECK_ARG(G > 0 && B > 0 && k_in > 0, "merge_topk: bad shape G=%d B=%d k_in=%d", G, B, k_in);
    MMRAG_CHECK_ARG(k >= 1 && k <= MMRAG_MAX_K, "merge_topk: k=%d outside 1..%d", k, MMRAG_MAX_K);
    const int K = k <= 5 ? 5 : (k <= 10 ? 10 : 20);
    launch_merge<long long>(K, scores, (const long long *)rows, (long long)G * k_in, k_in, (long long)B * k_in,
                            k_in, B, k, 0, out_scores, (long long *)out_rows, (hipStream_t)stream);
    MMRAG_CHECK_HIP(hipGetLastError());
    return MMRAG_OK;
}

}
```

Baseline: 681,700.

## Add wave-parallel sorted-list select kernel that rearms exchange workspace for next scan

Adds a select kernel for K=5 with up to 320 lists per query. Each query is handled by one wavefront: it finds the K-th best list head through DPP reductions, filters candidates against that threshold, and extracts the final top-k. The same kernel also resets the scan's exchange/ticket region, so the next armed scan can skip its hipMemsetD32Async. The Python plan object tracks armed workspaces so the memset is only skipped when the previous select rearmed that buffer. This removes a memset launch and the generic merge from the query path, at the cost of cross-call state that must stay consistent.

```diff
diff --git a/include/mmrag.h b/include/mmrag.h
--- a/include/mmrag.h
+++ b/include/mmrag.h
@@ -38,6 +38,12 @@
                             size_t workspace_bytes, void *stream);
 int mmrag_cosine_topk_select(int B, int64_t n, int k, int64_t row_offset, const void *workspace,
                              float *out_scores, int64_t *out_rows, void *stream);
+
+int mmrag_cosine_topk_select_rearm(int B, int64_t n, int k, int64_t row_offset, void *workspace,
+                                   float *out_scores, int64_t *out_rows, void *stream);
+int mmrag_cosine_topk_lists_armed(const void *q, const void *corpus, int B, int64_t n, int d, int64_t ld,
+                                  int dtype, int k, const uint32_t *alive_bits, void *workspace,
+                                  size_t workspace_bytes, void *stream);
 
 #define MMRAG_MAX_K_DEEP 4096
 size_t mmrag_cosine_topk_deep_workspace_bytes(int B, int64_t n, int k);
diff --git a/multimodal_rag_amd/_native.py b/multimodal_rag_amd/_native.py
--- a/multimodal_rag_amd/_native.py
+++ b/multimodal_rag_amd/_native.py
@@ -3,6 +3,7 @@
 import ctypes
 import os
 import threading
+import weakref
 from ctypes import c_char_p, c_float, c_int, c_int32, c_int64, c_size_t, c_void_p
 from typing import Optional, Tuple
 
@@ -64,6 +65,12 @@
                                                         c_int, c_void_p, c_void_p, c_size_t, c_void_p, ctypes.c_uint]
     lib.mmrag_cosine_topk_select.restype = c_int
     lib.mmrag_cosine_topk_select.argtypes = [c_int, c_int64, c_int, c_int64, c_void_p, c_void_p, c_void_p, c_void_p]
+    lib.mmrag_cosine_topk_select_rearm.restype = c_int
+    lib.mmrag_cosine_topk_select_rearm.argtypes = lib.mmrag_cosine_topk_select.argtypes
+    lib.mmrag_cosine_topk_lists_armed.restype = c_int
+    lib.mmrag_cosine_topk_lists_armed.argtypes = lib.mmrag_cosine_topk_lists.argtypes
+    lib.mmrag_internal_select_layout.restype = c_int
+    lib.mmrag_internal_select_layout.argtypes = [c_int, c_int64, c_int] + [c_void_p] * 5
     lib.mmrag_cosine_topk_deep_workspace_bytes.restype = c_size_t
     lib.mmrag_cosine_topk_deep_workspace_bytes.argtypes = [c_int, c_int64, c_int]
     lib.mmrag_cosine_topk_deep.restype = c_int
@@ -379,6 +386,14 @@
     return t.numel() * t.element_size()
 
 
+_ARMED: dict = {}
+
+
+def _disarm(workspace: Optional[torch.Tensor]) -> None:
+    if workspace is not None and _ARMED:
+        _ARMED.pop(workspace.data_ptr(), None)
+
+
 def _check_q_rows(who: str, q: torch.Tensor, rows: torch.Tensor, n: Optional[int] = None, other: str = "corpus"):
     if q.dim() != 2 or rows.dim() != 2 or not q.is_contiguous() or not rows.is_contiguous():
         raise MMRagNativeError(f"{who}: q and {other} must be contiguous 2-D tensors")
@@ -425,6 +440,7 @@
     B, ld = q.shape
     L = lib()
     need = L.mmrag_cosine_topk_workspace_bytes(B, n, k)
+    _disarm(workspace)
     if workspace is None or _nbytes(workspace) < need:
         workspace = torch.empty(max(need, 16), dtype=torch.uint8, device=q.device)
     out_s, out_r = _topk_out(B, k, q.device, packed_out)
@@ -451,6 +467,7 @@
     B, ld = q.shape
     L = lib()
     need = cosine_topk_deep_workspace_bytes(B, n, k)
+    _disarm(workspace)
     if workspace is None or _nbytes(workspace) < need:
         workspace = torch.empty(max(need, 16), dtype=torch.uint8, device=q.device)
     out_s, out_r = _topk_out(B, k, q.device)
@@ -741,6 +758,7 @@
     packed = _pinned_to_device(torch.cat(tables + [torch.zeros(1, dtype=torch.int32)]), dev)
     soq, off, grp = (packed[lo:] for lo in at)
     need = scoped_topk_workspace_bytes(B, n, k, n_groups)
+    _disarm(workspace)
     if workspace is None or _nbytes(workspace) < need:
         workspace = torch.empty(max(need, 16), dtype=torch.uint8, device=dev)
     out_s, out_r = _topk_out(B, k, dev)
@@ -869,6 +887,7 @@
         raise MMRagNativeError(f"filtered_topk: filter_of_query outside 0..{F - 1}")
     foq_dev = _pinned_to_device(foq, dev)
     need = filtered_topk_workspace_bytes(B, n, k)
+    _disarm(workspace)
     if workspace is None or _nbytes(workspace) < need:
         workspace = torch.empty(max(need, 16), dtype=torch.uint8, device=dev)
     out_s, out_r = _topk_out(B, k, dev)
@@ -935,6 +954,7 @@
         foq_dev = _pinned_to_device(foq, dev)
     slots = sum(g + 1 for g in facet_sizes)
     need = range_scan_workspace_bytes(B, n, limit, slots)
+    _disarm(workspace)
     if workspace is None or _nbytes(workspace) < need:
         workspace = torch.empty(max(need, 16), dtype=torch.uint8, device=dev)
     counts = torch.empty(B, dtype=torch.int32, device=dev)
@@ -1063,6 +1083,7 @@
     prior_dev = _boost_operand("boosted_topk", "prior", prior, n, False, dev)
     weight_dev = _boost_operand("boosted_topk", "weight", weight, B, True, dev)
     need = boosted_topk_workspace_bytes(B, n, k)
+    _disarm(workspace)
     if workspace is None or _nbytes(workspace) < need:
         workspace = torch.empty(max(need, 16), dtype=torch.uint8, device=dev)
     out_s, out_r = _topk_out(B, k, dev)
@@ -1190,6 +1211,7 @@
     if w_dev is None:
         w_dev = _pinned_to_device(torch.from_numpy(w_host), dev)
     need = recommend_topk_workspace_bytes(R, n, k)
+    _disarm(workspace)
     if workspace is None or _nbytes(workspace) < need:
         workspace = torch.empty(max(need, 16), dtype=torch.uint8, device=dev)
     out_s, out_r = _topk_out(R, k, dev)
@@ -1429,6 +1451,7 @@
     need = maxsim_topk_workspace_bytes(Q, n_items, k, int(dim), tiles, torch.float8_e4m3fn if _f8 else torch.float16)
     if need == 0:
         raise MMRagNativeError(f"{who}: dim must be a multiple of 64, at most 1024 (dim={dim})")
+    _disarm(workspace)
     if workspace is None or _nbytes(workspace) < need:
         workspace = torch.empty(max(need, 16), dtype=torch.uint8, device=dev)
     out_s, out_r = _topk_out(Q, k, dev)
@@ -1597,6 +1620,7 @@
     if n > corpus.shape[0]:
         raise MMRagNativeError(f"cosine_topk_lists: n={n} exceeds corpus capacity {corpus.shape[0]}")
     B, ld = q.shape
+    _disarm(workspace)
     with torch.cuda.device(q.device):
         st = lib().mmrag_internal_cosine_topk_lists_ex(
             q.data_ptr(), corpus.data_ptr(), B, n, d, ld, _TORCH2DT[q.dtype], k,
@@ -1605,18 +1629,28 @@
     _check(st, "mmrag_cosine_topk_lists")
 
 
+def select_layout(B: int, n: int, k: int) -> dict:
+    n_lists, b_pad = c_int(), c_int()
+    off_r, off_pub, xch = c_size_t(), c_size_t(), c_size_t()
+    _check(lib().mmrag_internal_select_layout(B, n, k, ctypes.addressof(n_lists), ctypes.addressof(b_pad),
+                                              ctypes.addressof(off_r), ctypes.addressof(off_pub), ctypes.addressof(xch)),
+           "mmrag_internal_select_layout")
+    return {"n_lists": n_lists.value, "b_pad": b_pad.value, "K": 5 if k <= 5 else (10 if k <= 10 else 20),
+            "off_r": off_r.value, "off_pub": off_pub.value, "xch_bytes": xch.value}
+
+
 def cosine_topk_select(B: int, n: int, k: int, row_offset: int, workspace: torch.Tensor,
                        out_scores: Optional[torch.Tensor] = None,
-                       out_rows: Optional[torch.Tensor] = None) -> Tuple[torch.Tensor, torch.Tensor]:
+                       out_rows: Optional[torch.Tensor] = None, rearm: bool = False) -> Tuple[torch.Tensor, torch.Tensor]:
     _dev_check(workspace)
     dev = workspace.device
     if out_scores is None:
         out_scores = torch.empty((B, k), dtype=torch.float32, device=dev)
     if out_rows is None:
         out_rows = torch.empty((B, k), dtype=torch.int64, device=dev)
+    fn = lib().mmrag_cosine_topk_select_rearm if rearm else lib().mmrag_cosine_topk_select
     with torch.cuda.device(dev):
-        st = lib().mmrag_cosine_topk_select(B, n, k, row_offset, workspace.data_ptr(), out_scores.data_ptr(),
-                                            out_rows.data_ptr(), _stream_ptr(dev))
+        st = fn(B, n, k, row_offset, workspace.data_ptr(), out_scores.data_ptr(), out_rows.data_ptr(), _stream_ptr(dev))
     _check(st, "mmrag_cosine_topk_select")
     return out_scores, out_rows
 
@@ -1778,6 +1812,7 @@
     _dev_check(ids, pos_ids, cu_seqlens, sel, workspace, out)
     T, B = ids.numel(), cu_seqlens.numel() - 1
     need = encoder_workspace_bytes(desc, T, B, f32)
+    _disarm(workspace)
     if workspace is None or _nbytes(workspace) < need:
         workspace = torch.empty(need, dtype=torch.uint8, device=ids.device)
     if out is None:
@@ -1807,6 +1842,7 @@
             raise MMRagNativeError("encoder_forward_tokens: proj must be a contiguous [out_dim, hidden] float16 tensor")
         out_dim = int(proj.shape[0])
     need = encoder_tokens_workspace_bytes(desc, T, B, out_dim)
+    _disarm(workspace)
     if workspace is None or _nbytes(workspace) < need:
         workspace = torch.empty(max(need, 16), dtype=torch.uint8, device=ids.device)
     if out is None:
@@ -1846,6 +1882,7 @@
         if t.dtype != torch.float32 or t.numel() != H or not t.is_contiguous():
             raise MMRagNativeError("sparse_expand_forward: head bias / LayerNorm vectors must be [hidden] float32")
     need = sparse_expand_forward_workspace_bytes(desc, T, B)
+    _disarm(workspace)
     if workspace is None or _nbytes(workspace) < need:
         workspace = torch.empty(max(need, 16), dtype=torch.uint8, device=ids.device)
     if out is None:
@@ -1919,6 +1956,7 @@
     B = q_off.numel() - 1
     dev = q_off.device
     need = impact_topk_workspace_bytes(B, n, k)
+    _disarm(workspace)
     if workspace is None or _nbytes(workspace) < need:
         workspace = torch.empty(max(need, 16), dtype=torch.uint8, device=dev)
     out_s, out_r = _topk_out(max(B, 1), max(k, 1), dev)
@@ -1946,6 +1984,7 @@
     _dev_check(ids, type_ids, pos_ids, cu_seqlens, workspace, out)
     T, B = ids.numel(), cu_seqlens.numel() - 1
     need = cross_encoder_workspace_bytes(desc, T, B, f32)
+    _disarm(workspace)
     if workspace is None or _nbytes(workspace) < need:
         workspace = torch.empty(need, dtype=torch.uint8, device=ids.device)
     if out is None:
@@ -2010,6 +2049,7 @@
     T = ids.numel()
     B = _reader_tables(cu_seqlens, ctx_start, ctx_len)
     need = reader_workspace_bytes(desc, T, B)
+    _disarm(workspace)
     if workspace is None or _nbytes(workspace) < need:
         workspace = torch.empty(max(need, 16), dtype=torch.uint8, device=ids.device)
     span, score, null, lse, lg = _reader_outs(B, T, n_best, logits, ids.device)
@@ -2062,6 +2102,7 @@
     B = pixels.shape[0]
     S = (desc.image // desc.patch) ** 2 + 1
     need = encoder_workspace_bytes(desc, B * S, B)
+    _disarm(workspace)
     if workspace is None or _nbytes(workspace) < need:
         workspace = torch.empty(need, dtype=torch.uint8, device=pixels.device)
     if out is None:
@@ -2189,14 +2230,20 @@
                            _nbytes(workspace))
         self._ws = workspace.data_ptr()
         self._scan = lib().mmrag_cosine_topk_lists
-        self._select = lib().mmrag_cosine_topk_select
+        self._scan_armed = lib().mmrag_cosine_topk_lists_armed
+        self._select = lib().mmrag_cosine_topk_select_rearm
+        ws = self._ws
+        self._ref = weakref.ref(self, lambda r: _ARMED.pop(ws, None) if _ARMED.get(ws) is r else None)
 
     def scan(self, stream: int) -> None:
-        st = self._scan(*self._scan_args, stream)
+        armed = _ARMED.pop(self._ws, None) is self._ref
+        st = (self._scan_armed if armed else self._scan)(*self._scan_args, stream)
         if st:
             _check(st, "mmrag_cosine_topk_lists")
 
     def select(self, row_offset: int, out_scores_ptr: int, out_rows_ptr: int, stream: int) -> None:
+        _ARMED.pop(self._ws, None)
         st = self._select(self.B, self.n, self.k, row_offset, self._ws, out_scores_ptr, out_rows_ptr, stream)
         if st:
-            _check(st, "mmrag_cosine_topk_select")
+            _check(st, "mmrag_cosine_topk_select_rearm")
+        _ARMED[self._ws] = self._ref
diff --git a/multimodal_rag_amd/csrc/search.hip b/multimodal_rag_amd/csrc/search.hip
--- a/multimodal_rag_amd/csrc/search.hip
+++ b/multimodal_rag_amd/csrc/search.hip
@@ -132,6 +132,132 @@
             }
         }
     }
+}
+
+#ifndef MMRAG_SELECT_WAVES
+#define MMRAG_SELECT_WAVES 16
+#endif
+constexpr int SEL_WAVES = MMRAG_SELECT_WAVES;
+constexpr int SEL_JMAX = 5;
+
+constexpr int DPP_XOR1 = 0xb1, DPP_XOR2 = 0x4e;
+constexpr int DPP_HALF_MIRROR = 0x141;
+constexpr int DPP_ROR8 = 0x128;
+template <int CTRL>
+__device__ __forceinline__ int sel_dpp(int x) {
+    return __builtin_amdgcn_update_dpp(x, x, CTRL, 0xf, 0xf, false);
+}
+__device__ __forceinline__ float sel_wave_max(float v) {
+    v = fmaxf(v, __builtin_bit_cast(float, sel_dpp<DPP_XOR1>(__builtin_bit_cast(int, v))));
+    v = fmaxf(v, __builtin_bit_cast(float, sel_dpp<DPP_XOR2>(__builtin_bit_cast(int, v))));
+    v = fmaxf(v, __builtin_bit_cast(float, sel_dpp<DPP_HALF_MIRROR>(__builtin_bit_cast(int, v))));
+    v = fmaxf(v, __builtin_bit_cast(float, sel_dpp<DPP_ROR8>(__builtin_bit_cast(int, v))));
+    const int x = __builtin_bit_cast(int, v);
+    const float a = __builtin_bit_cast(float, __builtin_amdgcn_readlane(x, 0));
+    const float b = __builtin_bit_cast(float, __builtin_amdgcn_readlane(x, 16));
+    const float c = __builtin_bit_cast(float, __builtin_amdgcn_readlane(x, 32));
+    const float d = __builtin_bit_cast(float, __builtin_amdgcn_readlane(x, 48));
+    return fmaxf(fmaxf(a, b), fmaxf(c, d));
+}
+__device__ __forceinline__ int sel_wave_min(int v) {
+    v = min(v, sel_dpp<DPP_XOR1>(v));
+    v = min(v, sel_dpp<DPP_XOR2>(v));
+    v = min(v, sel_dpp<DPP_HALF_MIRROR>(v));
+    v = min(v, sel_dpp<DPP_ROR8>(v));
+    return min(min(__builtin_amdgcn_readlane(v, 0), __builtin_amdgcn_readlane(v, 16)),
+               min(__builtin_amdgcn_readlane(v, 32), __builtin_amdgcn_readlane(v, 48)));
+}
+
+template <int K>
+__global__ __launch_bounds__(64 * SEL_WAVES) void select_sorted_lists_kernel(
+    const float *__restrict__ cs, const int *__restrict__ cr, int n_lists, int B, int k_out, long long row_offset,
+    float *__restrict__ out_s, long long *__restrict__ out_r, uint4 *__restrict__ rearm, unsigned rearm_vec) {
+#if defined(__HIP_DEVICE_COMPILE__)
+    if (rearm != nullptr) {
+        const uint4 t = {TICKET0, TICKET0, TICKET0, TICKET0};
+        for (unsigned i = blockIdx.x * blockDim.x + threadIdx.x; i < rearm_vec; i += gridDim.x * blockDim.x) rearm[i] = t;
+    }
+    const int lane = threadIdx.x & 63;
+    const int q = blockIdx.x * SEL_WAVES + __builtin_amdgcn_readfirstlane(threadIdx.x >> 6);
+    if (q >= B) return;
+    const float *qs = cs + (size_t)q * n_lists * K;
+    const int *qr = cr + (size_t)q * n_lists * K;
+
+    float s[SEL_JMAX][K];
+    int r[SEL_JMAX][K];
+#pragma unroll
+    for (int j = 0; j < SEL_JMAX; ++j) {
+        const int list = lane + 64 * j;
+        const bool have = list < n_lists;
+#pragma unroll
+        for (int i = 0; i < K; ++i) {
+            s[j][i] = have ? qs[list * K + i] : NEG_INF;
+            r[j][i] = have ? qr[list * K + i] : INT_MAX;
+        }
+    }
+    float h[SEL_JMAX];
+#pragma unroll
+    for (int j = 0; j < SEL_JMAX; ++j) h[j] = (r[j][0] == INT_MAX || r[j][0] < 0) ? NEG_INF : s[j][0];
+    float hk = NEG_INF;
+#pragma unroll
+    for (int round = 0; round < K; ++round) {
+        float m = h[0];
+#pragma unroll
+        for (int j = 1; j < SEL_JMAX; ++j) m = fmaxf(m, h[j]);
+        hk = sel_wave_max(m);
+        const unsigned long long owners = __builtin_amdgcn_ballot_w64(m == hk);
+        if (owners != 0ull && lane == (int)__builtin_ctzll(owners)) {
+            bool done = false;
+#pragma unroll
+            for (int j = 0; j < SEL_JMAX; ++j) {
+                const bool hit = !done && h[j] == hk;
+                h[j] = hit ? NEG_INF : h[j];
+                done = done || hit;
+            }
+        }
+    }
+    TopList<K> l;
+    l.init();
+#pragma unroll
+    for (int j = 0; j < SEL_JMAX; ++j) {
+#pragma unroll
+        for (int i = 0; i < K; ++i) {
+            const bool pass = s[j][i] >= hk && r[j][i] != INT_MAX && r[j][i] >= 0;
+            if (__builtin_amdgcn_ballot_w64(pass) != 0ull) {
+                if (pass) l.insert_ordered(s[j][i], r[j][i]);
+            }
+        }
+    }
+    float ov = NEG_INF;
+    int orr = INT_MAX;
+#pragma unroll
+    for (int round = 0; round < K; ++round) {
+        const float bs = sel_wave_max(l.v[0]);
+        const int br = sel_wave_min(l.v[0] == bs ? l.r[0] : INT_MAX);
+        const bool mine = l.v[0] == bs && l.r[0] == br;
+        const unsigned long long owners = __builtin_amdgcn_ballot_w64(mine);
+        const int from = owners != 0ull ? (int)__builtin_ctzll(owners) : 0;
+        const float ws = __builtin_bit_cast(float, __builtin_amdgcn_readlane(__builtin_bit_cast(int, l.v[0]), from));
+        if (lane == round) {
+            ov = ws;
+            orr = br;
+        }
+        if (mine) {
+#pragma unroll
+            for (int i = 0; i + 1 < K; ++i) {
+                l.v[i] = l.v[i + 1];
+                l.r[i] = l.r[i + 1];
+            }
+            l.v[K - 1] = NEG_INF;
+            l.r[K - 1] = INT_MAX;
+        }
+    }
+    if (lane < k_out && lane < K) {
+        const bool valid = orr != INT_MAX && ov > NEG_INF;
+        out_s[(size_t)q * k_out + lane] = valid ? ov : NEG_INF;
+        out_r[(size_t)q * k_out + lane] = valid ? (long long)orr + row_offset : -1;
+    }
+#endif
 }
 
 struct Plan {
@@ -304,9 +430,9 @@
     return ws_layout(make_plan(B, n, k)).total + 256;
 }
 
-int mmrag_internal_cosine_topk_lists_ex(const void *q, const void *corpus, int B, int64_t n, int d, int64_t ld,
-                                        int dtype, int k, const uint32_t *alive_bits, void *workspace,
-                                        size_t workspace_bytes, void *stream, unsigned dbg) {
+static int cosine_topk_lists_impl(const void *q, const void *corpus, int B, int64_t n, int d, int64_t ld, int dtype,
+                                  int k, const uint32_t *alive_bits, void *workspace, size_t workspace_bytes,
+                                  void *stream, unsigned dbg, bool armed) {
     if (int st = check_search_args("cosine_topk", MMRAG_MAX_K, q, corpus, B, n, d, ld, dtype, k)) return st;
     if (n == 0) return MMRAG_OK;
     const Plan pl = make_plan(B, n, k, dbg);
@@ -353,8 +479,9 @@
         const bool seed = per >= 12 && !(dbg & DBG_NO_SEED);
         const bool dyn = pl.grid_y == 1 && per >= 24 && !(dbg & DBG_NO_DYN);
         if (seed || dyn) {
-            MMRAG_CHECK_HIP(hipMemsetD32Async((hipDeviceptr_t)((char *)workspace + wl.off_pub), (int)TICKET0,
-                                              (wl.xch_end - wl.off_pub) / 4, s));
+            if (!armed || dbg != 0u)
+                MMRAG_CHECK_HIP(hipMemsetD32Async((hipDeviceptr_t)((char *)workspace + wl.off_pub), (int)TICKET0,
+                                                  (wl.xch_end - wl.off_pub) / 4, s));
             if (seed) {
                 p.pub_best = (float *)((char *)workspace + wl.off_pub);
                 p.pub_thr = (float *)((char *)workspace + wl.off_pthr);
@@ -430,15 +557,42 @@
     return qs_supported(dtype, rb, pl.K) ? 1 : 0;
 }
 
+int mmrag_internal_cosine_topk_lists_ex(const void *q, const void *corpus, int B, int64_t n, int d, int64_t ld,
+                                        int dtype, int k, const uint32_t *alive_bits, void *workspace,
+                                        size_t workspace_bytes, void *stream, unsigned dbg) {
+    return cosine_topk_lists_impl(q, corpus, B, n, d, ld, dtype, k, alive_bits, workspace, workspace_bytes, stream, dbg,
+                                  false);
+}
+
 int mmrag_cosine_topk_lists(const void *q, const void *corpus, int B, int64_t n, int d, int64_t ld, int dtype,
                             int k, const uint32_t *alive_bits, void *workspace, size_t workspace_bytes,
                             void *stream) {
-    return mmrag_internal_cosine_topk_lists_ex(q, corpus, B, n, d, ld, dtype, k, alive_bits, workspace,
-                                               workspace_bytes, stream, 0u);
-}
-
-int mmrag_cosine_topk_select(int B, int64_t n, int k, int64_t row_offset, const void *workspace,
-                             float *out_scores, int64_t *out_rows, void *stream) {
+    return cosine_topk_lists_impl(q, corpus, B, n, d, ld, dtype, k, alive_bits, workspace, workspace_bytes, stream, 0u,
+                                  false);
+}
+
+int mmrag_cosine_topk_lists_armed(const void *q, const void *corpus, int B, int64_t n, int d, int64_t ld, int dtype,
+                                  int k, const uint32_t *alive_bits, void *workspace, size_t workspace_bytes,
+                                  void *stream) {
+    return cosine_topk_lists_impl(q, corpus, B, n, d, ld, dtype, k, alive_bits, workspace, workspace_bytes, stream, 0u,
+                                  true);
+}
+
+int mmrag_internal_select_layout(int B, int64_t n, int k, int *n_lists, int *b_pad, size_t *off_r, size_t *off_pub,
+                                 size_t *xch_bytes) {
+    MMRAG_CHECK_ARG(B > 0 && n > 0 && k >= 1 && k <= MMRAG_MAX_K, "select_layout: bad shape");
+    const Plan pl = make_plan(B, n, k);
+    const WsLayout wl = ws_layout(pl);
+    *n_lists = pl.n_lists;
+    *b_pad = pl.b_pad;
+    *off_r = wl.off_r;
+    *off_pub = wl.off_pub;
+    *xch_bytes = wl.xch_end - wl.off_pub;
+    return MMRAG_OK;
+}
+
+static int cosine_topk_select_impl(int B, int64_t n, int k, int64_t row_offset, void *workspace, float *out_scores,
+                                   int64_t *out_rows, void *stream, bool rearm) {
     MMRAG_CHECK_ARG(B > 0 && n >= 0 && k >= 1 && k <= MMRAG_MAX_K, "cosine_topk_select: bad shape");
     MMRAG_CHECK_ARG(out_scores && out_rows, "cosine_topk_select: null output");
     hipStream_t s = (hipStream_t)stream;
@@ -453,11 +607,32 @@
     const WsLayout wl = ws_layout(pl);
     const float *cand_s = (const float *)workspace;
     const int *cand_r = (const int *)((const char *)workspace + wl.off_r);
+    const size_t xch_bytes = rearm ? wl.xch_end - wl.off_pub : 0;
+    if (xch_bytes) MMRAG_CHECK_ARG(((uintptr_t)workspace % 16) == 0, "cosine_topk_select_rearm: workspace must be 16-byte aligned");
+    if (pl.K == 5 && pl.n_lists <= 64 * SEL_JMAX) {
+        select_sorted_lists_kernel<5><<<(B + SEL_WAVES - 1) / SEL_WAVES, 64 * SEL_WAVES, 0, s>>>(
+            cand_s, cand_r, pl.n_lists, B, k, row_offset, out_scores, (long long *)out_rows,
+            xch_bytes ? (uint4 *)((char *)workspace + wl.off_pub) : nullptr, (unsigned)(xch_bytes / 16));
+        MMRAG_CHECK_HIP(hipGetLastError());
+        return MMRAG_OK;
+    }
     const long long n_cand = (long long)pl.n_lists * pl.K;
     launch_merge<int>(pl.K, cand_s, cand_r, n_cand, n_cand, 0, n_cand, B, k, row_offset, out_scores,
                       (long long *)out_rows, s);
     MMRAG_CHECK_HIP(hipGetLastError());
-    return MMRAG_OK;
+    if (xch_bytes)
+        MMRAG_CHECK_HIP(hipMemsetD32Async((hipDeviceptr_t)((char *)workspace + wl.off_pub), (int)TICKET0, xch_bytes / 4, s));
+    return MMRAG_OK;
+}
+
+int mmrag_cosine_topk_select(int B, int64_t n, int k, int64_t row_offset, const void *workspace,
+                             float *out_scores, int64_t *out_rows, void *stream) {
+    return cosine_topk_select_impl(B, n, k, row_offset, const_cast<void *>(workspace), out_scores, out_rows, stream, false);
+}
+
+int mmrag_cosine_topk_select_rearm(int B, int64_t n, int k, int64_t row_offset, void *workspace, float *out_scores,
+                                   int64_t *out_rows, void *stream) {
+    return cosine_topk_select_impl(B, n, k, row_offset, workspace, out_scores, out_rows, stream, true);
 }
 
 int mmrag_cosine_topk(const void *q, const void *corpus, int B, int64_t n, int d, int64_t ld, int dtype,
```

Result: no change. 684,500 (median of 2 runs) (+0.4%).
